# tan9zj/xnrs

Measured on AMD Instinct MI355X. Metric: impressions/sec (encode+score) on MIND-shaped batches, higher is better.
Workload: dtype f32; 1 GPU; NRMS full user+news encode + 5-candidate dot scoring (BASELINE configs[2]; token shape of config/mind_small_NRMS.yml); batch_impressions_per_gpu=512, history=50, candidates=5, d_backbone=768, n_heads=16, emb_dim=256, parallelism=impressions sharded by user over 1 GPU(s), no data-path collective

## Files before the change

### include/xnrs_hip.h

```cpp
#ifndef XNRS_HIP_H
#define XNRS_HIP_H

#include <stddef.h>
#include <stdint.h>

#ifdef __cplusplus
extern "C" {
#endif

#define XNRS_ABI_VERSION 6

#define XNRS_OK 0
#define XNRS_EINVAL (-1)
#define XNRS_EHEADS (-2)
#define XNRS_EWORKSPACE (-3)
#define XNRS_EUNSUPPORTED (-4)

#define XNRS_ACT_NONE 0
#define XNRS_ACT_RELU 1
#define XNRS_ACT_TANH 2

#define XNRS_POOL_ADDITIVE 0
#define XNRS_POOL_MEAN 1

typedef struct {
  const float *wq, *bq, *wk, *bk, *wv, *bv, *wo, *bo;
  int32_t n_heads;
  int32_t scaled;
  float dropout_p;
  uint64_t seed;
  const uint64_t *seed_dev;
} xnrs_mha_params;

typedef struct {
  const float *w1, *b1, *w2, *b2;
  int32_t hidden;
  const float *w1_folded, *b1_folded;
} xnrs_additive_params;

typedef struct {
  const float *w0, *b0, *w2, *b2;
  int32_t out_features;
  int32_t activation;
  const float *w0_folded, *b0_rowvec;
} xnrs_head_params;

int32_t xnrs_abi_version(void);
const char *xnrs_build_id(void);
const char *xnrs_error_string(int32_t code);

int32_t xnrs_linear_fwd(const float *x, const int32_t *gather_ids, int32_t gather_S, const float *w,
                        const float *bias, float *y, int64_t M, int32_t N, int32_t K, int32_t act,
                        void *stream);

size_t xnrs_mha_workspace_bytes(int64_t B, int32_t S, int32_t D);
int32_t xnrs_mha_fwd(const float *x, const float *m, const xnrs_mha_params *p, float *y, int64_t B,
                     int32_t S, int32_t D, void *ws, size_t ws_bytes, void *stream);

size_t xnrs_additive_workspace_bytes(int64_t B, int32_t N, int32_t D, int32_t A);
int32_t xnrs_additive_attention_fwd(const float *x, const float *m, const xnrs_additive_params *p,
                                    float *y, float *a_out, int64_t B, int32_t N, int32_t D, void *ws,
                                    size_t ws_bytes, void *stream);

int32_t xnrs_masked_mean_fwd(const float *x, const float *m, float *y, int64_t B, int32_t N, int32_t D,
                             void *stream);

int32_t xnrs_collapse_mask(const float *m, float *hm, int64_t n_rows, int32_t S, void *stream);

size_t xnrs_text_encoder_workspace_bytes(int64_t n_news, int32_t S, int32_t D, int32_t A, int32_t E,
                                         int32_t has_att, int32_t pool_kind, int32_t has_head,
                                         int64_t chunk);
int32_t xnrs_text_encoder_fwd(const float *x, const float *m, const int32_t *ids, int64_t n_news,
                              int32_t S, int32_t D, const xnrs_mha_params *att, int32_t pool_kind,
                              const xnrs_additive_params *pool, const xnrs_head_params *head, float *y,
                              float *hm, int64_t chunk, void *ws, size_t ws_bytes, void *stream);

size_t xnrs_fold_weights_workspace_bytes(int32_t D, int32_t A);
int32_t xnrs_fold_weights(const xnrs_mha_params *att, const xnrs_additive_params *pool, int32_t D, float *w1f, float *b1f,
                          void *ws, size_t ws_bytes, void *stream);

size_t xnrs_fold_head_weights_workspace_bytes(int32_t D, int32_t E);
int32_t xnrs_fold_head_weights(const xnrs_mha_params *att, const xnrs_head_params *head, int32_t D, float *w0f, float *b0v,
                               void *ws, size_t ws_bytes, void *stream);

size_t xnrs_text_encoder_unpadded_workspace_bytes(int64_t n_news, int64_t n_valid, int32_t S, int32_t D, int32_t A,
                                                  int32_t E, int32_t has_att, int32_t has_head);
int32_t xnrs_text_encoder_fwd_unpadded(const float *x, const int32_t *ids, int64_t n_news, int32_t S, int32_t D,
                                       const int32_t *rows, const int64_t *row_off, int64_t n_valid,
                                       const xnrs_mha_params *att, const xnrs_additive_params *pool,
                                       const xnrs_head_params *head, float *y, float *hm, void *ws, size_t ws_bytes,
                                       void *stream);

size_t xnrs_text_encoder_compact_workspace_bytes(int64_t n_news, int32_t S, int32_t D, int32_t A, int32_t E,
                                                 int32_t has_att, int32_t has_head, int64_t chunk);
int32_t xnrs_text_encoder_fwd_compact(const float *x, const float *m, const int32_t *ids, int64_t n_news, int32_t S,
                                      int32_t D, const xnrs_mha_params *att, const xnrs_additive_params *pool,
                                      const xnrs_head_params *head, float *y, float *hm, int64_t chunk, void *ws,
                                      size_t ws_bytes, void *stream);

size_t xnrs_user_encoder_workspace_bytes(int64_t B, int32_t H, int32_t E, int32_t A, int32_t has_att,
                                         int32_t pool_kind, int32_t has_head);
int32_t xnrs_user_encoder_fwd(const float *x, const float *m, int64_t B, int32_t H, int32_t E,
                              const xnrs_mha_params *att, int32_t pool_kind,
                              const xnrs_additive_params *pool, const xnrs_head_params *head, float *y,
                              float *a_out, void *ws, size_t ws_bytes, void *stream);

int32_t xnrs_dot_scoring_fwd(const float *u, const float *c, float *r, int64_t B, int32_t C, int32_t E,
                             int32_t normalize, void *stream);

#define XNRS_POOL_NONE (-1)
typedef struct {
  float *wq, *bq, *wk, *bk, *wv, *bv, *wo, *bo;
} xnrs_mha_grads;
typedef struct {
  float *w1, *b1, *w2, *b2;
} xnrs_additive_grads;
typedef struct {
  float *w0, *b0, *w2, *b2;
} xnrs_head_grads;

size_t xnrs_seq_encoder_saved_bytes(int64_t n_seq, int32_t L, int32_t D, int32_t A, int32_t E, int32_t n_heads,
                                    int32_t pool_kind, int32_t has_head);
int32_t xnrs_seq_encoder_fwd_train(const float *x, const float *m, const int32_t *ids, int64_t n_seq, int32_t L,
                                   int32_t D, const xnrs_mha_params *att, int32_t pool_kind,
                                   const xnrs_additive_params *pool, const xnrs_head_params *head, float *y,
                                   float *a_out, float *hm, void *saved, size_t saved_bytes, void *stream);
int32_t xnrs_seq_encoder_fwd_train_live(const float *x, const float *m, const int32_t *ids, int64_t n_seq, int32_t L,
                                        int32_t D, const xnrs_mha_params *att, int32_t pool_kind,
                                        const xnrs_additive_params *pool, const xnrs_head_params *head, float *y,
                                        float *a_out, float *hm, void *saved, size_t saved_bytes,
                                        const int32_t *live_rows, const int32_t *live_src_rows, int64_t n_live,
                                        void *stream);
size_t xnrs_seq_encoder_bwd_workspace_bytes(int64_t n_seq, int32_t L, int32_t D, int32_t A, int32_t E,
                                            int32_t n_heads, int32_t pool_kind, int32_t has_head);
int32_t xnrs_seq_encoder_bwd(const float *x, const float *m, const int32_t *ids, int64_t n_seq, int32_t L, int32_t D,
                             const xnrs_mha_params *att, int32_t pool_kind, const xnrs_additive_params *pool,
                             const xnrs_head_params *head, const void *saved, size_t saved_bytes, const float *dy,
                             float *dx, const xnrs_mha_grads *g_att, const xnrs_additive_grads *g_pool,
                             const xnrs_head_grads *g_head, void *ws, size_t ws_bytes, void *stream);
int32_t xnrs_seq_encoder_bwd_live(const float *x, const float *m, const int32_t *ids, int64_t n_seq, int32_t L, int32_t D,
                                  const xnrs_mha_params *att, int32_t pool_kind, const xnrs_additive_params *pool,
                                  const xnrs_head_params *head, const void *saved, size_t saved_bytes, const float *dy,
                                  float *dx, const xnrs_mha_grads *g_att, const xnrs_additive_grads *g_pool,
                                  const xnrs_head_grads *g_head, const int32_t *live_rows,
                                  const int32_t *live_src_rows, int64_t n_live, void *ws, size_t ws_bytes, void *stream);

typedef struct {
  const int32_t *live_rows, *live_src_rows;
  int64_t n_live;
  const int32_t *kv_rows, *kv_src_rows;
  int64_t n_kv;
  const float *qkv_shared;
  const int64_t *counts_dev;
  float *dqkv_image;
  int32_t dqkv_mode;
} xnrs_row_lists;
#define XNRS_DQKV_OWN 0
#define XNRS_DQKV_DEFER 1
#define XNRS_DQKV_MERGE 2

size_t xnrs_row_lists_workspace_bytes(int64_t n_seq);
int32_t xnrs_build_row_lists(const float *m, const int32_t *ids, int64_t n_seq, int32_t L, int32_t *live_rows,
                             int32_t *live_src_rows, int32_t *kv_rows, int32_t *kv_src_rows, int64_t *counts, void *ws,
                             size_t ws_bytes, void *stream);
size_t xnrs_seq_encoder_saved_qkv_offset(int64_t n_seq, int32_t L, int32_t D, int32_t A, int32_t E, int32_t n_heads,
                                         int32_t pool_kind, int32_t has_head);
int32_t xnrs_seq_encoder_fwd_train_rows(const float *x, const float *m, const int32_t *ids, int64_t n_seq, int32_t L,
                                        int32_t D, const xnrs_mha_params *att, int32_t pool_kind,
                                        const xnrs_additive_params *pool, const xnrs_head_params *head, float *y,
                                        float *a_out, float *hm, void *saved, size_t saved_bytes,
                                        const xnrs_row_lists *rows, void *stream);
int32_t xnrs_seq_encoder_bwd_rows(const float *x, const float *m, const int32_t *ids, int64_t n_seq, int32_t L, int32_t D,
                                  const xnrs_mha_params *att, int32_t pool_kind, const xnrs_additive_params *pool,
                                  const xnrs_head_params *head, const void *saved, size_t saved_bytes, const float *dy,
                                  float *dx, const xnrs_mha_grads *g_att, const xnrs_additive_grads *g_pool,
                                  const xnrs_head_grads *g_head, const xnrs_row_lists *rows, void *ws, size_t ws_bytes,
                                  void *stream);

size_t xnrs_linear_bwd_workspace_bytes(int64_t M, int32_t N, int32_t K);
int32_t xnrs_linear_bwd(const float *x, const int32_t *gather_ids, int32_t gather_S, const float *w, const float *dy,
                        float *dx, float *dw, float *db, int64_t M, int32_t N, int32_t K, void *ws, size_t ws_bytes,
                        void *stream);

size_t xnrs_embedding_linear_bwd_workspace_bytes(int64_t M, int32_t N, int32_t K);
int32_t xnrs_embedding_linear_bwd(const float *table, const int32_t *ids, const float *w, const float *dy, float *d_table,
                                  float *dw, float *db, int64_t M, int32_t N, int32_t K, int32_t n_rows, void *ws,
                                  size_t ws_bytes, void *stream);

int32_t xnrs_dot_scoring_bwd(const float *u, const float *c, const float *dr, float *du, float *dc, int64_t B,
                             int32_t C, int32_t E, void *stream);
int32_t xnrs_dot_scoring_norm_bwd(const float *u, const float *c, const float *dr, float *du, float *dc, int64_t B,
                                  int32_t C, int32_t E, void *stream);

int32_t xnrs_gather_rows(const float *table, const int32_t *ids, float *out, int64_t n, int64_t row_floats,
                         void *stream);

int32_t xnrs_dropout_rows(const float *x, const int32_t *ids, float *out, int64_t n, int64_t row_floats, float p,
                          uint64_t seed, const uint64_t *seed_dev, void *stream);

int32_t xnrs_assemble_train_batch(const int64_t *sess, int64_t B, const int64_t *hist_off, const int32_t *hist_val,
                                  const int64_t *pos_off, const int32_t *pos_val, const int64_t *neg_off,
                                  const int32_t *neg_val, int32_t l_hist, int32_t n_neg, int32_t pad_row, uint64_t seed,
                                  int32_t *hist_rows, int32_t *cand_rows, void *stream);
int32_t xnrs_assemble_eval_batch(const int64_t *sess, int64_t B, const int64_t *hist_off, const int32_t *hist_val,
                                 const int64_t *pos_off, const int32_t *pos_val, const int64_t *neg_off,
                                 const int32_t *neg_val, int32_t l_hist, int32_t pad_row, const int64_t *cand_off,
                                 int32_t *hist_rows, int32_t *cand_rows, int32_t *cand_sess, float *targets, void *stream);
int32_t xnrs_score_csr(const float *vecs, const int32_t *cand_rows, const int32_t *cand_sess, const float *u, float *r,
                       int64_t n_cand, int32_t E, int32_t relu, void *stream);
int32_t xnrs_rank_metrics(const float *scores, const float *targets, const int64_t *cand_off, float *out, int64_t B,
                          void *stream);

size_t xnrs_infonce_saved_bytes(int64_t B, int32_t E);
int32_t xnrs_infonce_fwd(const float *emb, const int64_t *labels, int64_t B, int32_t E, float temperature, float *loss,
                         void *saved, size_t saved_bytes, void *stream);
int32_t xnrs_infonce_bwd(const int64_t *labels, int64_t B, int32_t E, float temperature, const void *saved,
                         size_t saved_bytes, const float *gout, float *demb, void *stream);

#define XNRS_PROFILE_STAGES 10
int32_t xnrs_profile_enable(uint32_t stage_mask);
int32_t xnrs_profile_read(double *ms, int64_t *launches, double *flops);

int32_t xnrs_train_fold_enabled(void);

#define XNRS_STATUS_NONBINARY_MASK 1
#define XNRS_STATUS_ROW_RANGE 2
#define XNRS_STATUS_QUERY_RANGE 4
int32_t xnrs_set_status_word(int32_t *device_word);
const char *xnrs_status_string(int32_t word);

#define XNRS_GEMM_F32 0
#define XNRS_GEMM_BF16X3 1
#define XNRS_GEMM_BF16X2 2
int32_t xnrs_set_gemm_mode(int32_t mode);
int32_t xnrs_get_gemm_mode(void);

int32_t xnrs_reload_knobs(void);

size_t xnrs_bilinear_scoring_saved_bytes(int64_t B, int32_t E, int32_t normalize);
int32_t xnrs_bilinear_scoring_fwd(const float *u, const float *c, const float *w, const float *bias, float *s, int64_t B,
                                  int32_t N, int32_t E, int32_t normalize, void *saved, size_t saved_bytes, void *stream);
size_t xnrs_bilinear_scoring_bwd_workspace_bytes(int64_t B, int32_t E, int32_t normalize);
int32_t xnrs_bilinear_scoring_bwd(const float *u, const float *c, const float *w, const void *saved, size_t saved_bytes,
                                  const float *ds, float *du, float *dc, float *dw, float *dbias, int64_t B, int32_t N,
                                  int32_t E, int32_t normalize, void *ws, size_t ws_bytes, void *stream);
size_t xnrs_mlp_scoring_saved_bytes(int64_t B, int32_t N, int32_t H);
int32_t xnrs_mlp_scoring_fwd(const float *u, const float *c, const float *w1, const float *b1, const float *w2,
                             const float *b2, float *s, int64_t B, int32_t N, int32_t E, int32_t H, void *saved,
                             size_t saved_bytes, void *stream);
size_t xnrs_mlp_scoring_bwd_workspace_bytes(int64_t B, int32_t N, int32_t H);
int32_t xnrs_mlp_scoring_bwd(const float *u, const float *c, const float *w1, const float *w2, const void *saved,
                             size_t saved_bytes, const float *ds, float *du, float *dc, float *dw1, float *db1, float *dw2,
                             float *db2, int64_t B, int32_t N, int32_t E, int32_t H, void *ws, size_t ws_bytes,
                             void *stream);
int32_t xnrs_mlp_scoring_news_proj(const float *c, int64_t rows, int32_t E, const float *w1, int32_t H, float *p,
                                   void *stream);
size_t xnrs_score_csr_scorer_workspace_bytes(int64_t n_sess, int32_t width);
int32_t xnrs_score_csr_bilinear(const float *vecs, const int32_t *cand_rows, const int32_t *cand_sess, const float *u,
                                int64_t n_sess, const float *w, const float *bias, float *r, int64_t n_cand, int32_t E,
                                int32_t relu, void *ws, size_t ws_bytes, void *stream);
int32_t xnrs_score_csr_mlp(const float *P, const int32_t *cand_rows, const int32_t *cand_sess, const float *u,
                           int64_t n_sess, const float *w1, const float *b1, const float *w2, const float *b2, float *r,
                           int64_t n_cand, int32_t E, int32_t H, int32_t relu, void *ws, size_t ws_bytes, void *stream);
int32_t xnrs_l2_normalize_rows(const float *x, float *y, int64_t rows, int32_t E, void *stream);

typedef struct {
  const float *wx, *bx;
  const float *q;
  const int32_t *q_idx;
  int32_t hidden;
  int32_t q_ld;
  int32_t n_q;
} xnrs_personalized_params;

size_t xnrs_personalized_saved_bytes(int64_t n_seq, int32_t L, int32_t D, int32_t A, int32_t E, int32_t has_head);
int32_t xnrs_personalized_fwd(const float *x, const float *m, const int32_t *ids, int64_t n_seq, int32_t L, int32_t D,
                              const xnrs_personalized_params *p, const xnrs_head_params *head, float *y, float *a_out,
                              float *hm, void *ws, size_t ws_bytes, void *stream);
int32_t xnrs_personalized_fwd_train(const float *x, const float *m, const int32_t *ids, int64_t n_seq, int32_t L, int32_t D,
                                    const xnrs_personalized_params *p, const xnrs_head_params *head, float *y, float *a_out,
                                    float *hm, void *saved, size_t saved_bytes, void *stream);
size_t xnrs_personalized_bwd_workspace_bytes(int64_t n_seq, int32_t L, int32_t D, int32_t A, int32_t E, int32_t has_head);
int32_t xnrs_personalized_bwd(const float *x, const int32_t *ids, int64_t n_seq, int32_t L, int32_t D,
                              const xnrs_personalized_params *p, const xnrs_head_params *head, const void *saved,
                              size_t saved_bytes, const float *dy, float *dx, float *dwx, float *dbx, float *dq, int64_t n_q,
                              const xnrs_head_grads *g_head, void *ws, size_t ws_bytes, void *stream);

int32_t xnrs_embedding_grad_sparse(const float *d_rows, const int32_t *ids, int64_t M, int32_t K, float *d_table,
                                   int32_t n_rows, void *stream);
size_t xnrs_embedding_linear_bwd_sparse_workspace_bytes(int64_t M, int32_t N, int32_t K);
int32_t xnrs_embedding_linear_bwd_sparse(const float *table, const int32_t *ids, const float *w, const float *dy,
                                         float *d_table, float *dw, float *db, int64_t M, int32_t N, int32_t K, int32_t n_rows,
                                         void *ws, size_t ws_bytes, void *stream);

typedef struct {
  const float *w_ih, *w_hh, *b_ih, *b_hh;
  int32_t hidden;
} xnrs_gru_params;
typedef struct {
  float *w_ih, *w_hh, *b_ih, *b_hh;
} xnrs_gru_grads;
size_t xnrs_gru_workspace_bytes(int64_t B, int32_t T, int32_t E, int32_t Hd);
size_t xnrs_gru_saved_bytes(int64_t B, int32_t T, int32_t E, int32_t Hd);
int32_t xnrs_gru_fwd(const float *x, const float *m, int32_t ldm, const float *h0, const xnrs_gru_params *p, float *y,
                     int64_t B, int32_t T, int32_t E, void *ws, size_t ws_bytes, void *stream);
int32_t xnrs_gru_fwd_train(const float *x, const float *m, int32_t ldm, const float *h0, const xnrs_gru_params *p, float *y,
                           int64_t B, int32_t T, int32_t E, void *saved, size_t saved_bytes, void *stream);
size_t xnrs_gru_bwd_workspace_bytes(int64_t B, int32_t T, int32_t E, int32_t Hd);
int32_t xnrs_gru_bwd(const float *x, const xnrs_gru_params *p, const void *saved, size_t saved_bytes, const float *dy,
                     float *dx, float *dh0, const xnrs_gru_grads *g, int64_t B, int32_t T, int32_t E, void *ws,
                     size_t ws_bytes, void *stream);

size_t xnrs_attn_long_saved_bytes(int64_t L, int64_t Nb, int32_t E, int32_t n_heads);
size_t xnrs_attn_long_workspace_bytes(int64_t L, int64_t Nb, int32_t E, int32_t n_heads);
int32_t xnrs_attn_long_fwd(const float *qkv, int64_t seq_stride, int64_t batch_stride, float *o, int64_t o_seq_stride,
                           int64_t o_batch_stride, int64_t L, int64_t Nb, int32_t E, int32_t n_heads, void *stream);
int32_t xnrs_attn_long_fwd_train(const float *qkv, int64_t seq_stride, int64_t batch_stride, float *o, int64_t o_seq_stride,
                                 int64_t o_batch_stride, int64_t L, int64_t Nb, int32_t E, int32_t n_heads, void *saved,
                                 size_t saved_bytes, void *stream);
int32_t xnrs_attn_long_bwd(const float *qkv, int64_t seq_stride, int64_t batch_stride, const float *o, const float *d_o,
                           int64_t o_seq_stride, int64_t o_batch_stride, const void *saved, size_t saved_bytes, float *dqkv,
                           int64_t L, int64_t Nb, int32_t E, int32_t n_heads, void *ws, size_t ws_bytes, void *stream);

int32_t xnrs_caum_pair_fwd(const float *hp, const float *cp, int64_t ld_cp, float *h_cnn, float *z, int64_t B, int32_t C,
                           int32_t H, int32_t E, void *stream);
int32_t xnrs_caum_pair_bwd(const float *d_hcnn, const float *d_z, float *d_hp, float *d_cp, int64_t ld_dcp, int64_t B,
                           int32_t C, int32_t H, int32_t E, void *stream);

int32_t xnrs_caum_bias_tanh_fwd(const float *pre, const float *cb, int64_t ld_cb, float *t, int64_t P, int32_t H, int32_t E,
                                void *stream);
int32_t xnrs_caum_bias_tanh_bwd(const float *t, const float *dt, float *dpre, float *dcb, int64_t P, int32_t H, int32_t E,
                                void *stream);
int32_t xnrs_act_bwd(const float *y, const float *dy, float *dpre, int64_t n, int32_t act, void *stream);

int32_t xnrs_caum_pool_fwd(const float *t2, const float *w3, const float *b3, const float *h_all, float *u, float *a_out,
                           int64_t P, int32_t H, int32_t A, int32_t E, void *stream);
size_t xnrs_caum_pool_bwd_workspace_bytes(int64_t P, int32_t H, int32_t A);
int32_t xnrs_caum_pool_bwd(const float *t2, const float *w3, const float *h_all, const float *a, const float *du, float *d_t2,
                           float *d_w3, float *d_b3, float *d_hall, int64_t P, int32_t H, int32_t A, int32_t E, void *ws,
                           size_t ws_bytes, void *stream);

#ifdef __cplusplus
}
#endif
#endif
```

### xnrs_amd/csrc/api.hip

```cpp
#include <mutex>
#include <vector>

#include "host.h"

using namespace xnrs;

namespace xnrs {
uint32_t g_prof_mask = 0;
}
namespace {
std::vector<ProfRec> g_prof;
std::mutex g_prof_mu;
constexpr size_t PROF_MAX = 1 << 16;
}

bool xnrs::prof_begin(ProfRec* r, hipStream_t stream) {
  if (hipEventCreate(&r->beg) != hipSuccess || hipEventCreate(&r->end) != hipSuccess) return false;
  (void)hipEventRecord(r->beg, stream);
  return true;
}

void xnrs::prof_end(const ProfRec& r, hipStream_t stream) {
  (void)hipEventRecord(r.end, stream);
  std::lock_guard<std::mutex> lk(g_prof_mu);
  if (g_prof.size() < PROF_MAX) g_prof.push_back(r);
  else {
    (void)hipEventDestroy(r.beg);
    (void)hipEventDestroy(r.end);
  }
}

int64_t xnrs::prof_count(int stage, const int64_t* cnt, int which, int64_t host_value, hipStream_t stream) {
  if (!cnt || !prof_on(stage)) return host_value;
  int64_t v = host_value;
  if (hipStreamSynchronize(stream) != hipSuccess) return host_value;
  if (hipMemcpy(&v, cnt + which, sizeof(v), hipMemcpyDeviceToHost) != hipSuccess) return host_value;
  return v;
}

extern "C" {

int32_t xnrs_abi_version(void) { return XNRS_ABI_VERSION; }

#ifndef XNRS_BUILD_ID
#define XNRS_BUILD_ID "unknown"
#endif
const char* xnrs_build_id(void) { return XNRS_BUILD_ID; }

int32_t xnrs_set_status_word(int32_t* device_word) {
  set_status_word(device_word);
  return XNRS_OK;
}

const char* xnrs_status_string(int32_t word) {
  if (word == XNRS_STATUS_QUERY_RANGE)
    return "a query row index or user id outside its table (personalized attention: NaN outputs / clamped user ids)";
  if (word & XNRS_STATUS_QUERY_RANGE)
    return "several status bits: a query row index or user id out of range, and a bad mask value or table row id";
  switch (word & 3) {
    case 0: return "ok";
    case XNRS_STATUS_NONBINARY_MASK: return "a mask value other than 0 / 1 reached the device-compacted encoder (its outputs are NaN)";
    case XNRS_STATUS_ROW_RANGE: return "a news-table row id outside the table (clamped; the gathered rows are wrong)";
    default: return "a mask value other than 0 / 1 reached the device-compacted encoder AND a table row id was out of range";
  }
}

const char* xnrs_error_string(int32_t code) {
  switch (code) {
    case XNRS_OK: return "ok";
    case XNRS_EINVAL: return "invalid argument (shape or NULL pointer)";
    case XNRS_EHEADS: return "d_model is not divisible by n_heads";
    case XNRS_EWORKSPACE: return "workspace too small";
    case XNRS_EUNSUPPORTED:
      return "shape outside the supported range (attention S <= 128, pooling N <= 512, head width d_k <= 128, "
             "personalized attention L <= 4096, CAUM pooling H <= 8192)";
    default: return code > 0 ? hipGetErrorString((hipError_t)code) : "unknown error";
  }
}

int32_t xnrs_set_gemm_mode(int32_t mode) {
  const int prev = xnrs::gemm_mode();
  xnrs::set_gemm_mode(mode);
  return prev;
}

int32_t xnrs_get_gemm_mode(void) { return xnrs::gemm_mode(); }

int32_t xnrs_train_fold_enabled(void) { return fold_wanted(knobs().fold_train) ? 1 : 0; }

int32_t xnrs_reload_knobs(void) {
  xnrs::reload_knobs();
  return XNRS_OK;
}

int32_t xnrs_profile_enable(uint32_t stage_mask) {
  std::lock_guard<std::mutex> lk(g_prof_mu);
  for (auto& r : g_prof) {
    (void)hipEventDestroy(r.beg);
    (void)hipEventDestroy(r.end);
  }
  g_prof.clear();
  g_prof_mask = stage_mask;
  return XNRS_OK;
}

int32_t xnrs_profile_read(double* ms, int64_t* launches, double* flops) {
  if (!ms || !launches || !flops) return XNRS_EINVAL;
  for (int i = 0; i < XNRS_PROFILE_STAGES; ++i) {
    ms[i] = 0.0;
    launches[i] = 0;
    flops[i] = 0.0;
  }
  int32_t rc = XNRS_OK;
  std::lock_guard<std::mutex> lk(g_prof_mu);
  for (auto& r : g_prof) {
    float t = 0.f;
    hipError_t e = hipEventSynchronize(r.end);
    if (e == hipSuccess) e = hipEventElapsedTime(&t, r.beg, r.end);
    if (e != hipSuccess) rc = (int32_t)e;
    else {
      ms[r.stage] += t;
      launches[r.stage] += 1;
      flops[r.stage] += r.flops;
    }
    (void)hipEventDestroy(r.beg);
    (void)hipEventDestroy(r.end);
  }
  g_prof.clear();
  return rc;
}

}
```

### xnrs_amd/csrc/encoder_fwd.hip

```cpp
#include <vector>

#include "host.h"

using namespace xnrs;

namespace xnrs {

Plan make_plan(int64_t n_seq, int L, int D, int A, int E, bool att, bool additive, bool head, bool pooled, int64_t chunk,
               bool train, int n_heads) {
  Plan p{};
  if (train) chunk = n_seq > 0 ? n_seq : 1;
  if (chunk <= 0) chunk = 65536 / L;
  if (chunk > n_seq) chunk = n_seq;
  if (chunk < 1) chunk = 1;
  p.chunk = chunk;
  const size_t rows = (size_t)chunk * L;
  Carver c;
  p.off_qkv = c.take_if(att, rows * 3 * (size_t)D * F32);
  p.off_o = c.take_if(att, rows * (size_t)D * F32);
  p.off_y = c.take_if(att && pooled, rows * (size_t)D * F32);
  p.off_t = c.take_if(pooled && additive, rows * (size_t)A * F32);
  p.off_p = c.take_if(pooled && head, (size_t)n_seq * D * F32);
  p.off_h = c.take_if(pooled && head, (size_t)n_seq * E * F32);
  p.off_stats = c.take_if(train && att, (size_t)chunk * n_heads * L * 2 * F32);
  p.off_a = c.take_if(train && additive, rows * F32);
  size_t pl = 0;
  if (att) pl += 4 * align_up(split_planes_bytes(D, D));
  if (pooled && additive) pl += align_up(split_planes_bytes(A, D));
  p.off_planes = c.take(pl);
  NewsFusedPlan nf{};
  size_t nfb = 0;
  if (att && additive && !train) {
    if (n_heads <= 0) nfb = news_fused_img_bound_bytes(L, D, A);
    else if (news_fused_plan(L, D, n_heads, A, &nf)) nfb = nf.img_bytes;
  }
  p.off_nf = c.take_if(nfb != 0, nfb);
  p.off_nfo = c.take_if(nfb != 0, news_fused_scratch_bytes(L, D));
  const bool lt = att && pooled && !train;
  const size_t passes = (size_t)(((n_seq > 0 ? n_seq : 1) + chunk - 1) / chunk);
  p.off_lt_alive = c.take_if(lt, (size_t)(n_seq > 0 ? n_seq : 1));
  p.off_lt_n = c.take_if(lt, passes * sizeof(int64_t));
  p.off_lt_tiles = c.take_if(lt, passes * (size_t)live_tiles_cap(chunk, L, LIVE_TILE_BM) * sizeof(int32_t));
  const bool lr = lt && L <= 64;
  p.off_lr_loc = c.take_if(lr, passes * rows * sizeof(int32_t));
  p.off_lr_src = c.take_if(lr, passes * rows * sizeof(int32_t));
  p.off_lr_cnt = c.take_if(lr, passes * 3 * sizeof(int64_t));
  p.fold = carve_fold(c, att && additive, n_seq, D, A);
  p.total = c.total();
  return p;
}

bool device_counts_ok(const float* x, int D, int A, const xnrs_mha_params* att, const xnrs_additive_params* pool) {
  auto al16 = [](const void* p) { return p == nullptr || (reinterpret_cast<uintptr_t>(p) & 15) == 0; };
  if (!knobs().gemm_buf || gemm_mode() != 0 || D % 4 != 0 || D < 4 || (A > 0 && A % 4 != 0)) return false;
  if (!al16(x) || (pool && !al16(pool->w1))) return false;
  if (att && !(al16(att->wq) && al16(att->wk) && al16(att->wv) && al16(att->wo))) return false;
  return (int64_t)D * D * 4 <= (1ll << 30) && (int64_t)A * D * 4 <= (1ll << 30);
}

}

namespace {


hipError_t fold_product(const float* X, int M, const float* wo, int D, float* C, float* slabs, hipStream_t stream) {
  GemmArgs g = gemm_kmajor_b(X, D, wo, D, C, D, M, D, D);
  if (D >= 64 * FOLD_SPLITS) {
    g.slabs = slabs;
    g.nsplit = FOLD_SPLITS;
  }
  return launch_gemm_f32(g, stream);
}

const float* fold_out_projection(const xnrs_mha_params* att, const xnrs_additive_params* pool, int D, int A, float* wf,
                                 float* bf, float* slabs, hipStream_t stream, hipError_t* err) {
  *err = fold_product(pool->w1, A, att->wo, D, wf, slabs, stream);
  if (*err != hipSuccess || !att->bo) return pool->b1;
  *err = launch_fold_bias(pool->w1, att->bo, pool->b1, bf, A, D, stream);
  return bf;
}

struct Fc1 {
  const float* w;
  const float* b;
};
int32_t fc1_pair(bool fold, const xnrs_mha_params* att, const xnrs_additive_params* pool, int D, void* ws, const FoldRegions& fr,
                 hipStream_t stream, Fc1* fc1) {
  *fc1 = Fc1{pool ? pool->w1 : nullptr, pool ? pool->b1 : nullptr};
  if (!fold) return XNRS_OK;
  if (pool->w1_folded) {
    if (att->bo && !pool->b1_folded) return XNRS_EINVAL;
    *fc1 = Fc1{pool->w1_folded, att->bo ? pool->b1_folded : pool->b1};
    return XNRS_OK;
  }
  hipError_t fe = hipSuccess;
  fc1->w = at(ws, fr.fw);
  fc1->b = fold_out_projection(att, pool, D, pool->hidden, at(ws, fr.fw), at(ws, fr.fb), at(ws, fr.fsl), stream, &fe);
  return hip_rc(fe);
}

bool fc1_rowdot_ok(const float* x, bool att, const xnrs_additive_params* pool, int D) {
  auto al16 = [](const void* p) { return (reinterpret_cast<uintptr_t>(p) & 15) == 0; };
  return knobs().fc1_rowdot && knobs().gemm_buf && gemm_mode() == 0 && pool && pool->w2 && D % 4 == 0 && D >= 4 &&
         al16(pool->w1) && (att || al16(x)) && (int64_t)pool->hidden * D * 4 <= (1ll << 30);
}
inline int n_epart(int A) { return (A + 31) / 32; }

int32_t compact_attention_rc(const xnrs_mha_params* att, int S, int D) {
  if (att->n_heads <= 0 || D % att->n_heads != 0) return XNRS_EHEADS;
  if (S > 64 || D / att->n_heads > 64 || (D / att->n_heads) % 4 != 0 || D % 4 != 0) return XNRS_EUNSUPPORTED;
  return XNRS_OK;
}

GemmArgs qkv_projection(const float* x, RowIds rows, const xnrs_mha_params* att, int first, float* C, int64_t ldc, int64_t M,
                        int D, const unsigned short* const* planes = nullptr) {
  const float* W[3] = {att->wq, att->wk, att->wv};
  const float* b[3] = {att->bq, att->bk, att->bv};
  GemmArgs g = gemm_base(x, D, nullptr, D, C, ldc, M, D, D);
  g.gather_ids = rows.ids;
  g.gather_S = rows.S;
  for (int s = first; s < 3; ++s) {
    g.W[s - first] = W[s];
    g.bias[s - first] = b[s];
    g.Wp[s - first] = planes ? planes[s] : nullptr;
  }
  g.ldp = split_plane_ld(D);
  g.nseg = 3 - first;
  return g;
}

MhaCoreArgs mha_core_args(const float* k, int64_t ld, const xnrs_mha_params* att, float* out, int64_t n_seq, int S, int D) {
  MhaCoreArgs ma{};
  ma.k = k;
  ma.v = k + D;
  ma.ld = ld;
  ma.seq_stride = (int64_t)S * ld;
  ma.head_stride = D / att->n_heads;
  ma.out = out;
  ma.ldo = D;
  ma.n_seq = n_seq;
  ma.S = S;
  ma.n_heads = att->n_heads;
  ma.d_k = D / att->n_heads;
  ma.scaled = att->scaled;
  return ma;
}

GemmArgs fc1_product(const float* seq, RowIds rows, Fc1 fc1, float* t, int64_t M, int D, int A, bool rowdot,
                     const xnrs_additive_params* pool, const unsigned short* planes = nullptr) {
  GemmArgs g = gemm_linear(seq, rows, D, fc1.w, fc1.b, t, A, M, A, D, XNRS_ACT_TANH, planes);
  if (rowdot) {
    g.rowdot_w = pool->w2;
    g.rowdot_out = t;
    g.ldrd = n_epart(A);
  }
  return g;
}

AdditivePoolArgs additive_pool_args(const float* t, bool rowdot, const xnrs_additive_params* pool, const float* x, int64_t n_seq,
                                    int N, int D, int A) {
  AdditivePoolArgs pa{};
  pa.t = rowdot ? nullptr : t;
  pa.epart = rowdot ? t : nullptr;
  pa.n_epart = n_epart(A);
  pa.w2 = pool->w2;
  pa.b2 = pool->b2;
  pa.x = x;
  pa.ldx = D;
  pa.n_seq = n_seq;
  pa.N = N;
  pa.D = D;
  pa.A = A;
  return pa;
}

hipError_t pooled_out_projection(const float* po, const float* s, const xnrs_mha_params* att, float* dst, int64_t n, int D,
                                 const unsigned short* planes, hipStream_t stream) {
  GemmArgs g = gemm_linear(po, {}, D, att->wo, nullptr, dst, D, n, D, D, XNRS_ACT_NONE, planes);
  const bool in_epilogue = att->bo && gemm_mode() == 0;
  if (in_epilogue) {
    g.rowscale = s;
    g.rowscale_vec = att->bo;
  }
  hipError_t e = launch_gemm_f32(g, stream);
  if (e != hipSuccess || !att->bo || in_epilogue) return e;
  return launch_add_rowscaled_bias(dst, D, s, att->bo, n, D, stream);
}

int32_t pooled_tail(bool fold, const float* pob, const float* asum, const xnrs_mha_params* att, const xnrs_head_params* head,
                    float* pb, float* hb, float* y, int64_t n, int D, int E, const unsigned short* wo_planes, bool train,
                    hipStream_t stream) {
  const bool fold_head = fold && head && !train && head->w0_folded && gemm_mode() == 0 && (!att->bo || head->b0_rowvec);
  if (fold && !fold_head) {
    ProfScope ps(2, 2.0 * n * (double)D * D, stream);
    XNRS_TRY(pooled_out_projection(pob, asum, att, head ? pb : y, n, D, wo_planes, stream));
  }
  if (head) {
    ProfScope ps(5, 2.0 * n * ((double)D * E + (double)E * E), stream);
    GemmArgs g1 = gemm_linear(fold_head ? pob : pb, {}, D, fold_head ? head->w0_folded : head->w0, head->b0, hb, E, n, E, D,
                              head->activation);
    if (fold_head && att->bo) {
      g1.rowscale = asum;
      g1.rowscale_vec = head->b0_rowvec;
    }
    XNRS_TRY(launch_gemm_f32(g1, stream));
    XNRS_TRY(launch_gemm_f32(gemm_linear(hb, {}, E, head->w2, head->b2, y, E, n, E, E), stream));
  }
  return XNRS_OK;
}

}

int32_t xnrs::seq_encode(const SeqEncode& r, hipStream_t stream) {
  const float *x = r.x, *m = r.m;
  const int32_t* ids = r.ids;
  const int64_t n_seq = r.n_seq;
  const int L = r.L, D = r.D, pool_kind = r.pool_kind;
  const xnrs_mha_params* att = r.att;
  const xnrs_additive_params* pool = r.pool;
  const xnrs_head_params* head = r.head;
  const bool pooled = r.pooled, train = r.train;
  float *y = r.y, *a_out = r.a_out, *hm = r.hm;
  const xnrs_row_lists no_lists{};
  const xnrs_row_lists* rl = r.rl ? r.rl : &no_lists;
  const int32_t *live_rows = rl->live_rows, *live_src_rows = rl->live_src_rows, *kv_rows = rl->kv_rows,
                *kv_src_rows = rl->kv_src_rows;
  const float* qkv_shared = rl->qkv_shared;
  const int64_t* cnt = rl->counts_dev;
  const int64_t n_live = cnt ? n_seq * L : rl->n_live, n_kv = cnt ? n_seq * L : rl->n_kv;
  if (n_seq == 0) return XNRS_OK;
  if (n_seq < 0 || L <= 0 || D <= 0 || !x || !y) return XNRS_EINVAL;
  if (att) {
    if (att->n_heads <= 0 || !att->wq || !att->wk || !att->wv || !att->wo) return XNRS_EINVAL;
    if (D % att->n_heads != 0) return XNRS_EHEADS;
    if (L > 128) return XNRS_EUNSUPPORTED;
    if (train && D / att->n_heads > 128) return XNRS_EUNSUPPORTED;
  }
  const bool additive = pooled && pool_kind == XNRS_POOL_ADDITIVE;
  if (pooled) {
    if (pool_kind != XNRS_POOL_ADDITIVE && pool_kind != XNRS_POOL_MEAN) return XNRS_EINVAL;
    if (additive && (!pool || !pool->w1 || !pool->w2 || pool->hidden <= 0)) return XNRS_EINVAL;
    if (pool_kind == XNRS_POOL_MEAN && !m) return XNRS_EINVAL;
    if (L > 512) return XNRS_EUNSUPPORTED;
    if (head && (!head->w0 || !head->w2 || head->out_features <= 0 || head->activation < 0 || head->activation > 2))
      return XNRS_EINVAL;
  }
  if (ids && !m && pooled && pool_kind == XNRS_POOL_MEAN) return XNRS_EINVAL;
  const int A = additive ? pool->hidden : 0;
  const int E = (pooled && head) ? head->out_features : D;
  const Plan p = make_plan(n_seq, L, D, A, E, att != nullptr, additive, pooled && head, pooled, r.chunk, train,
                           att ? att->n_heads : 0);
  if (p.total > r.ws_bytes || (p.total > 0 && !r.ws)) return XNRS_EWORKSPACE;
  void* w = r.ws;
  float* stats = (train && att) ? at(w, p.off_stats) : nullptr;
  float* a_save = (train && additive) ? at(w, p.off_a) : nullptr;
  const bool qkv_given = train && att && qkv_shared;
  float* qkv = qkv_given ? const_cast<float*>(qkv_shared) : at(w, p.off_qkv);
  float *o = at(w, p.off_o), *yb = at(w, p.off_y), *t = at(w, p.off_t), *pb = at(w, p.off_p), *hb = at(w, p.off_h);

  const bool live = train && additive && m && live_rows && (cnt || (n_live >= 0 && n_live < n_seq * L)) &&
                    !(ids && !live_src_rows);
  if (cnt && live && !device_counts_ok(x, D, A, att, pool)) return XNRS_EUNSUPPORTED;
  const int32_t* lvx = live ? (ids ? live_src_rows : live_rows) : nullptr;
  const bool kvl = live && kv_rows && (cnt || (n_kv >= 0 && n_kv < n_seq * L)) && !(ids && !kv_src_rows);
  const int32_t* kvx = kvl ? (ids ? kv_src_rows : kv_rows) : nullptr;

  NewsFusedArgs f{};
  bool fused = att && additive && !train && !a_out && att->dropout_p == 0.f && gemm_mode() == 0 &&
               knobs().news_fused && news_fused_plan(L, D, att->n_heads, A, nullptr) &&
               (D / att->n_heads) * att->n_heads == D &&
               (knobs().news_fused == 2 || (L >= 26 && n_seq >= 192));
  if (fused) {
    f.x = x; f.ids = ids; f.mask = m;
    f.wq = att->wq; f.bq = att->bq; f.wk = att->wk; f.bk = att->bk; f.wv = att->wv; f.bv = att->bv;
    f.wo = att->wo; f.bo = att->bo;
    f.w1 = pool->w1; f.b1 = pool->b1; f.w2 = pool->w2; f.b2 = pool->b2;
    f.img = at(w, p.off_nf);
    f.p = head ? pb : y;
    f.ldp = D;
    f.hm = m ? hm : nullptr;
    f.n_seq = n_seq;
    f.S = L; f.D = D; f.n_heads = att->n_heads; f.d_k = D / att->n_heads; f.A = A; f.scaled = att->scaled;
    f.npw = knobs().news_fused_npw ? knobs().news_fused_npw : (n_seq < 512 ? 1 : 2);
    if (fold_wanted(knobs().fold_out)) {
      f.fold = 1;
      f.o_scratch = at(w, p.off_nfo);
      f.asum = at(w, p.fold.as);
      f.p = at(w, p.fold.po);
    }
    fused = p.off_nf != 0 && news_fused_ready(f);
  }
  const bool fold = att && additive && fold_wanted(train ? knobs().fold_train : knobs().fold_out);
  float *pob = at(w, p.fold.po), *asum = at(w, p.fold.as);
  const bool rowdot = additive && !train && !fused && fc1_rowdot_ok(x, att != nullptr, pool, D);
  Fc1 fc1{};
  XNRS_TRY_RC(fc1_pair(fold, att, additive ? pool : nullptr, D, w, p.fold, stream, &fc1));
  if (fold && fused) {
    f.w1 = fc1.w;
    f.b1 = fc1.b;
  }

  bool afused = !att && additive && !train && !a_out && gemm_mode() == 0 && knobs().additive_fused &&
                additive_fused_plan(L, D, A, nullptr, nullptr) && rowdot &&
                (knobs().additive_fused == 2 || additive_fused_tiles(n_seq, L) >= 512);
  if (afused) {
    AdditiveFusedArgs af{};
    af.x = x; af.ids = ids; af.mask = m;
    af.w1 = pool->w1; af.b1 = pool->b1; af.w2 = pool->w2; af.b2 = pool->b2;
    af.y = head ? pb : y;
    af.ldy = D;
    af.hm = m ? hm : nullptr;
    af.n_seq = n_seq;
    af.S = L; af.D = D; af.A = A;
    afused = additive_fused_ready(af);
    if (afused) {
      const double fl = (double)n_seq * (2.0 * L * D * A + 2.0 * L * (A + D));
      ProfScope ps(3, fl, stream);
      XNRS_TRY(launch_additive_fused(af, stream));
    }
  }

  const unsigned short* pqkv[3] = {nullptr, nullptr, nullptr};
  const unsigned short *po = nullptr, *p1 = nullptr;
  if (gemm_mode() != 0) {
    char* pw = at<char>(w, p.off_planes);
    auto prep = [&](const float* W, int N, int K) -> const unsigned short* {
      unsigned short* dst = reinterpret_cast<unsigned short*>(pw);
      pw += align_up(split_planes_bytes(N, K));
      return launch_split_weights(W, N, K, dst, stream) == hipSuccess ? dst : nullptr;
    };
    if (att) {
      pqkv[0] = prep(att->wq, D, D);
      pqkv[1] = prep(att->wk, D, D);
      pqkv[2] = prep(att->wv, D, D);
      po = prep(att->wo, D, D);
    }
    if (pooled && additive) p1 = prep(fc1.w, A, D);
  }

  if (fused) {
    const double fl = (double)n_seq * ((f.fold ? 6.0 : 8.0) * L * D * D + 4.0 * L * L * D + 2.0 * L * D * A + 2.0 * L * (A + D));
    ProfScope ps(6, fl, stream);
    XNRS_TRY(launch_news_fused(f, stream));
  }
  const bool lt = r.live_tiles && knobs().gemm_live_tiles && !train && pooled && m && att && !fused && !afused &&
                  n_seq * (int64_t)L >= knobs().gemm_live_tiles_min_rows &&
                  device_counts_ok(x, D, A, att, additive ? pool : nullptr);
  bool lt_qkv = false;
  if (lt && knobs().mha_skip_masked) {
    MhaCoreArgs probe = mha_core_args(qkv + D, 3 * (int64_t)D, att, o, p.chunk, L, D);
    probe.q = qkv;
    probe.mask = m;
    probe.skip_dead = 1;
    lt_qkv = mha_core_skips_dead(probe);
  }
  const bool lt_fc1 = lt && additive && rowdot;
  const int64_t lt_cap = live_tiles_cap(p.chunk, L, LIVE_TILE_BM);
  const int64_t* lt_n = at<int64_t>(w, p.off_lt_n);
  const int32_t* lt_tiles = at<int32_t>(w, p.off_lt_tiles);
  const bool lr = lt && knobs().gemm_live_rows && p.off_lr_cnt != 0 && L <= 64 && n_seq * (int64_t)L <= 0x7fffffffLL &&
                  n_seq * (int64_t)L >= knobs().gemm_live_rows_min_rows;
  const bool lr_qkv = lr && lt_qkv, lr_fc1 = lr && lt_fc1;
  const int32_t *lr_loc = at<int32_t>(w, p.off_lr_loc), *lr_src = at<int32_t>(w, p.off_lr_src);
  const int64_t* lr_cnt = at<int64_t>(w, p.off_lr_cnt);
  constexpr float LR_FILL = 0.3f;
  if (lr_qkv || lr_fc1)
    XNRS_TRY(launch_dense_row_lists(m, ids, n_seq, p.chunk, L, LIVE_TILE_BM, at<int32_t>(w, p.off_lr_loc), at<int32_t>(w, p.off_lr_src),
                                    at<int64_t>(w, p.off_lr_cnt), at<uint8_t>(w, p.off_lt_alive), at<int64_t>(w, p.off_lt_n),
                                    at<int32_t>(w, p.off_lt_tiles), stream));
  else if (lt_qkv || lt_fc1)
    XNRS_TRY(launch_live_tiles(m, ids, n_seq, p.chunk, L, LIVE_TILE_BM, at<uint8_t>(w, p.off_lt_alive), at<int64_t>(w, p.off_lt_n),
                               at<int32_t>(w, p.off_lt_tiles), stream));
  std::vector<int64_t> lt_host, lr_host;
  if ((lt_qkv && prof_on(0)) || (lt_fc1 && prof_on(3))) {
    lt_host.resize((size_t)((n_seq + p.chunk - 1) / p.chunk));
    if (hipStreamSynchronize(stream) != hipSuccess ||
        hipMemcpy(lt_host.data(), lt_n, lt_host.size() * sizeof(int64_t), hipMemcpyDeviceToHost) != hipSuccess)
      lt_host.clear();
    if (lr_qkv || lr_fc1) {
      lr_host.resize(3 * lt_host.size());
      if (lt_host.empty() || hipMemcpy(lr_host.data(), lr_cnt, lr_host.size() * sizeof(int64_t), hipMemcpyDeviceToHost) != hipSuccess)
        lr_host.clear();
    }
  }
  for (int64_t c0 = 0; !fused && !afused && c0 < n_seq; c0 += p.chunk) {
    const int64_t nc = (n_seq - c0 < p.chunk) ? (n_seq - c0) : p.chunk;
    const int64_t rows = nc * L;
    const int64_t* ltn = lt_n + c0 / p.chunk;
    const int32_t* ltl = lt_tiles + (c0 / p.chunk) * lt_cap;
    const double lt_rows = (double)LIVE_TILE_BM *
                           (double)(lt_host.empty() ? (rows + LIVE_TILE_BM - 1) / LIVE_TILE_BM : lt_host[(size_t)(c0 / p.chunk)]);
    const int32_t* lrl = lr_loc + (c0 / p.chunk) * p.chunk * L;
    const int32_t* lrs = lr_src + (c0 / p.chunk) * p.chunk * L;
    const int64_t* lrn = lr_cnt + 3 * (c0 / p.chunk);
    const double lr_rows = lr_host.empty() ? (double)rows : (double)lr_host[(size_t)(3 * (c0 / p.chunk))];
    const int32_t* cids = ids ? ids + c0 : nullptr;
    const float* cx = ids ? x : x + c0 * (int64_t)L * D;
    const float* cm = m ? (ids ? m : m + c0 * (int64_t)L) : nullptr;

    const float* seq = cx;
    const int32_t* seq_ids = cids;
    if (att) {
      const int64_t ld3 = 3 * (int64_t)D;
      if (qkv_given) {
      } else if (live) {
        const double nl = (double)prof_count(0, cnt, 0, n_live, stream), nkv = (double)prof_count(0, cnt, 1, n_kv, stream);
        ProfScope ps(0, 2.0 * (kvl ? nkv : rows) * 2.0 * D * D + 2.0 * nl * (double)D * D, stream);
        GemmArgs g = qkv_projection(cx, {cids, L}, att, 1, qkv + D, ld3, rows, D, pqkv);
        if (kvl) {
          XNRS_TRY(launch_zero_dead_qkv(qkv, cm, cids, nc, L, D, stream));
          g.gather_ids = kvx;
          g.gather_S = 1;
          g.c_scatter = 1;
          g.c_scatter_ids = kv_rows;
          g.M = n_kv;
          g.m_dev = cnt ? cnt + 1 : nullptr;
          g.m_fill_hint = 0.6f;
          if (n_kv > 0) XNRS_TRY(launch_gemm_f32(g, stream));
        } else {
          XNRS_TRY(launch_gemm_f32(g, stream));
          XNRS_TRY(launch_zero_cols(qkv, ld3, D, rows, stream));
        }
        if (n_live > 0) {
          GemmArgs q = gemm_linear(cx, {lvx, 1}, D, att->wq, att->bq, qkv, ld3, n_live, D, D, XNRS_ACT_NONE, pqkv[0]);
          q.c_scatter = 1;
          q.c_scatter_ids = live_rows;
          q.m_dev = cnt;
          q.m_fill_hint = 0.4f;
          XNRS_TRY(launch_gemm_f32(q, stream));
        }
      } else if (lr_qkv) {
        ProfScope ps(0, 2.0 * lt_rows * 2.0 * D * D + 2.0 * lr_rows * (double)D * D, stream);
        GemmArgs g = qkv_projection(cx, {cids, L}, att, 1, qkv + D, ld3, rows, D, pqkv);
        g.live_n = ltn;
        g.live_tiles = ltl;
        XNRS_TRY(launch_gemm_f32(g, stream));
        GemmArgs q = gemm_linear(cx, {ids ? lrs : lrl, 1}, D, att->wq, att->bq, qkv, ld3, rows, D, D);
        q.c_scatter = 1;
        q.c_scatter_ids = lrl;
        q.m_dev = lrn;
        q.m_fill_hint = LR_FILL;
        XNRS_TRY(launch_gemm_f32(q, stream));
      } else {
        GemmArgs g = qkv_projection(cx, {cids, L}, att, 0, qkv, ld3, rows, D, pqkv);
        if (lt_qkv) {
          g.live_n = ltn;
          g.live_tiles = ltl;
        }
        ProfScope ps(0, 2.0 * (lt_qkv ? lt_rows : (double)rows) * 3.0 * D * D, stream);
        XNRS_TRY(launch_gemm_f32(g, stream));
      }

      MhaCoreArgs ma = mha_core_args(qkv + D, ld3, att, o, nc, L, D);
      ma.q = qkv;
      ma.mask = cm;
      ma.mask_gather_ids = cids;
      ma.dropout_p = att->dropout_p;
      ma.seed = att->seed + (uint64_t)c0 * (uint64_t)att->n_heads * 0x9E3779B97F4A7C15ull;
      ma.seed_dev = att->seed_dev;
      ma.stats = stats;
      ma.skip_dead = (live || (pooled && cm && knobs().mha_skip_masked)) ? 1 : 0;
      if (lt_qkv && !mha_core_skips_dead(ma)) return XNRS_EUNSUPPORTED;
      {
        ProfScope ps(1, 4.0 * rows * (double)L * D, stream);
        XNRS_TRY(launch_mha_core(ma, stream));
      }

      float* dst = pooled ? yb : y + c0 * (int64_t)L * D;
      if (fold) {
        dst = o;
      } else if (live) {
        ProfScope ps(2, 2.0 * (double)prof_count(2, cnt, 0, n_live, stream) * (double)D * D, stream);
        XNRS_TRY(hipMemsetAsync(dst, 0, (size_t)rows * D * sizeof(float), stream));
        if (n_live > 0) {
          GemmArgs og = gemm_linear(o, {live_rows, 1}, D, att->wo, att->bo, dst, D, n_live, D, D, XNRS_ACT_NONE, po);
          og.c_scatter = 1;
          og.m_dev = cnt;
          og.m_fill_hint = 0.4f;
          XNRS_TRY(launch_gemm_f32(og, stream));
        }
      } else {
        ProfScope ps(2, 2.0 * rows * (double)D * D, stream);
        XNRS_TRY(launch_gemm_f32(gemm_linear(o, {}, D, att->wo, att->bo, dst, D, rows, D, D, XNRS_ACT_NONE, po), stream));
      }
      seq = dst;
      seq_ids = nullptr;
    }
    if (!pooled) continue;

    float* pooled_dst = (head ? pb : y) + c0 * (int64_t)D;
    float* hm_dst = hm ? hm + c0 : nullptr;
    if (additive) {
      if (live) {
        ProfScope ps(3, 2.0 * (double)prof_count(3, cnt, 0, n_live, stream) * (double)D * A, stream);
        XNRS_TRY(hipMemsetAsync(t, 0, (size_t)rows * A * sizeof(float), stream));
        if (n_live > 0) {
          GemmArgs fg = fc1_product(seq, {att ? live_rows : lvx, 1}, fc1, t, n_live, D, A, false, pool, p1);
          fg.c_scatter = 1;
          fg.c_scatter_ids = live_rows;
          fg.m_dev = cnt;
          fg.m_fill_hint = 0.4f;
          XNRS_TRY(launch_gemm_f32(fg, stream));
        }
      } else if (lr_fc1) {
        GemmArgs fg = fc1_product(seq, {seq_ids ? lrs : lrl, 1}, fc1, t, rows, D, A, true, pool, p1);
        fg.c_scatter = 1;
        fg.c_scatter_ids = lrl;
        fg.m_dev = lrn;
        fg.m_fill_hint = LR_FILL;
        ProfScope ps(3, 2.0 * lr_rows * (double)D * A, stream);
        XNRS_TRY(launch_gemm_f32(fg, stream));
      } else {
        GemmArgs fg = fc1_product(seq, {seq_ids, L}, fc1, t, rows, D, A, rowdot, pool, p1);
        if (lt_fc1) {
          fg.live_n = ltn;
          fg.live_tiles = ltl;
        }
        ProfScope ps(3, 2.0 * (lt_fc1 ? lt_rows : (double)rows) * (double)D * A, stream);
        XNRS_TRY(launch_gemm_f32(fg, stream));
      }
      AdditivePoolArgs pa = additive_pool_args(t, rowdot, pool, seq, nc, L, D, A);
      pa.skip_dead = lt_fc1 ? 1 : 0;
      pa.skip_masked = lr_fc1 ? 1 : 0;
      pa.mask = cm;
      pa.mask_gather_ids = cids;
      pa.x_gather_ids = seq_ids;
      pa.y = fold ? pob + c0 * (int64_t)D : pooled_dst;
      pa.asum_out = fold ? asum + c0 : nullptr;
      pa.a_out = a_save ? a_save : (a_out ? a_out + c0 * (int64_t)L : nullptr);
      pa.hm_out = cm ? hm_dst : nullptr;
      {
        ProfScope ps(4, 2.0 * rows * (double)(A + D), stream);
        XNRS_TRY(launch_additive_pool(pa, stream));
      }
      if (a_save && a_out)
        XNRS_TRY(hipMemcpyAsync(a_out, a_save, (size_t)rows * sizeof(float), hipMemcpyDeviceToDevice, stream));
    } else {
      MeanPoolArgs mp{};
      mp.x = seq;
      mp.ldx = D;
      mp.mask = cm;
      mp.mask_gather_ids = cids;
      mp.x_gather_ids = seq_ids;
      mp.y = pooled_dst;
      mp.hm_out = hm_dst;
      mp.n_seq = nc;
      mp.N = L;
      mp.D = D;
      {
        ProfScope ps(4, 2.0 * rows * (double)D, stream);
        XNRS_TRY(launch_mean_pool(mp, stream));
      }
    }
  }
  return pooled_tail(fold, pob, asum, att, pooled ? head : nullptr, pb, hb, y, n_seq, D, E, po, train, stream);
}

namespace {

struct UnpadPlan {
  size_t off_kv, off_q, off_o, off_y, off_t, off_p, off_h;
  FoldRegions fold;
  size_t total;
};
UnpadPlan make_unpad_plan(int64_t n_news, int64_t n_valid, int S, int D, int A, int E, bool att, bool head) {
  UnpadPlan p{};
  Carver c;
  const size_t nv = (size_t)(n_valid > 0 ? n_valid : 1);
  p.off_kv = c.take_if(att, (size_t)n_news * S * 2 * D * F32);
  p.off_q = c.take_if(att, nv * D * F32);
  p.off_o = c.take_if(att, nv * D * F32);
  p.off_y = c.take_if(att, nv * D * F32);
  p.off_t = c.take(nv * A * F32);
  p.off_p = c.take_if(head, (size_t)n_news * D * F32);
  p.off_h = c.take_if(head, (size_t)n_news * E * F32);
  p.fold = carve_fold(c, att, n_news, D, A);
  p.total = c.total();
  return p;
}

struct CompactPlan {
  int64_t chunk;
  size_t off_kv, off_q, off_o, off_t, off_roff, off_live, off_kvs, off_kvb, off_cnt, off_p, off_h;
  FoldRegions fold;
  size_t total;
};
CompactPlan make_compact_plan(int64_t n_news, int S, int D, int A, int E, bool att, bool head, int64_t chunk) {
  CompactPlan p{};
  if (chunk <= 0) chunk = 262144 / S;
  if (chunk > n_news) chunk = n_news;
  if (chunk < 1) chunk = 1;
  p.chunk = chunk;
  Carver c;
  const size_t rows = (size_t)chunk * S;
  p.off_kv = c.take_if(att, rows * 2 * D * F32);
  p.off_q = c.take_if(att, rows * D * F32);
  p.off_o = c.take_if(att, rows * D * F32);
  p.off_t = c.take(rows * (size_t)n_epart(A) * F32);
  const size_t passes = (size_t)((n_news + chunk - 1) / chunk);
  p.off_roff = c.take(passes * ((size_t)chunk + 1) * 8);
  p.off_live = c.take(passes * rows * 4);
  p.off_kvs = c.take(passes * rows * 4);
  p.off_kvb = c.take(passes * (size_t)chunk * 4);
  p.off_cnt = c.take(passes * 3 * 8);
  p.off_p = c.take_if(head, (size_t)n_news * D * F32);
  p.off_h = c.take_if(head, (size_t)n_news * E * F32);
  p.fold = carve_fold(c, att, n_news, D, A);
  p.total = c.total();
  return p;
}

SeqEncode padded_call(const float* x, const float* m, int64_t n_seq, int L, int D, float* y, void* ws, size_t ws_bytes) {
  SeqEncode r{};
  r.x = x; r.m = m; r.n_seq = n_seq; r.L = L; r.D = D; r.y = y; r.ws = ws; r.ws_bytes = ws_bytes;
  return r;
}

}

extern "C" {

int32_t xnrs_linear_fwd(const float* x, const int32_t* gather_ids, int32_t gather_S, const float* w, const float* bias,
                        float* y, int64_t M, int32_t N, int32_t K, int32_t act, void* stream) {
  if (!x || !w || !y || M < 0 || N <= 0 || K <= 0 || act < 0 || act > 2) return XNRS_EINVAL;
  if (gather_ids && gather_S <= 0) return XNRS_EINVAL;
  return hip_rc(launch_gemm_f32(gemm_linear(x, {gather_ids, gather_S}, K, w, bias, y, N, M, N, K, act), (hipStream_t)stream));
}

size_t xnrs_mha_workspace_bytes(int64_t B, int32_t S, int32_t D) {
  return make_plan(B, S, D, 0, D, true, false, false, false, 0).total;
}

int32_t xnrs_mha_fwd(const float* x, const float* m, const xnrs_mha_params* p, float* y, int64_t B, int32_t S, int32_t D,
                     void* ws, size_t ws_bytes, void* stream) {
  if (!p) return XNRS_EINVAL;
  SeqEncode r = padded_call(x, m, B, S, D, y, ws, ws_bytes);
  r.att = p;
  return seq_encode(r, (hipStream_t)stream);
}

size_t xnrs_additive_workspace_bytes(int64_t B, int32_t N, int32_t D, int32_t A) {
  return make_plan(B, N, D, A, D, false, true, false, true, 0).total;
}

int32_t xnrs_additive_attention_fwd(const float* x, const float* m, const xnrs_additive_params* p, float* y, float* a_out,
                                    int64_t B, int32_t N, int32_t D, void* ws, size_t ws_bytes, void* stream) {
  if (!p) return XNRS_EINVAL;
  SeqEncode r = padded_call(x, m, B, N, D, y, ws, ws_bytes);
  r.pooled = true; r.pool_kind = XNRS_POOL_ADDITIVE; r.pool = p; r.a_out = a_out;
  return seq_encode(r, (hipStream_t)stream);
}

int32_t xnrs_masked_mean_fwd(const float* x, const float* m, float* y, int64_t B, int32_t N, int32_t D, void* stream) {
  SeqEncode r = padded_call(x, m, B, N, D, y, nullptr, 0);
  r.pooled = true; r.pool_kind = XNRS_POOL_MEAN;
  return seq_encode(r, (hipStream_t)stream);
}

size_t xnrs_text_encoder_workspace_bytes(int64_t n_news, int32_t S, int32_t D, int32_t A, int32_t E, int32_t has_att,
                                         int32_t pool_kind, int32_t has_head, int64_t chunk) {
  return make_plan(n_news, S, D, A, E, has_att != 0, pool_kind == XNRS_POOL_ADDITIVE, has_head != 0, true, chunk).total;
}

int32_t xnrs_text_encoder_fwd(const float* x, const float* m, const int32_t* ids, int64_t n_news, int32_t S, int32_t D,
                              const xnrs_mha_params* att, int32_t pool_kind, const xnrs_additive_params* pool,
                              const xnrs_head_params* head, float* y, float* hm, int64_t chunk, void* ws, size_t ws_bytes,
                              void* stream) {
  if (n_news == 0) return XNRS_OK;
  if (!m) return XNRS_EINVAL;
  SeqEncode r = padded_call(x, m, n_news, S, D, y, ws, ws_bytes);
  r.ids = ids; r.att = att; r.pooled = true; r.pool_kind = pool_kind; r.pool = pool; r.head = head; r.hm = hm; r.chunk = chunk;
  r.live_tiles = true;
  return seq_encode(r, (hipStream_t)stream);
}

size_t xnrs_user_encoder_workspace_bytes(int64_t B, int32_t H, int32_t E, int32_t A, int32_t has_att, int32_t pool_kind,
                                         int32_t has_head) {
  return make_plan(B, H, E, A, E, has_att != 0, pool_kind == XNRS_POOL_ADDITIVE, has_head != 0, true, 0).total;
}

int32_t xnrs_user_encoder_fwd(const float* x, const float* m, int64_t B, int32_t H, int32_t E, const xnrs_mha_params* att,
                              int32_t pool_kind, const xnrs_additive_params* pool, const xnrs_head_params* head, float* y,
                              float* a_out, void* ws, size_t ws_bytes, void* stream) {
  SeqEncode r = padded_call(x, m, B, H, E, y, ws, ws_bytes);
  r.att = att; r.pooled = true; r.pool_kind = pool_kind; r.pool = pool; r.head = head; r.a_out = a_out;
  return seq_encode(r, (hipStream_t)stream);
}

size_t xnrs_text_encoder_unpadded_workspace_bytes(int64_t n_news, int64_t n_valid, int32_t S, int32_t D, int32_t A,
                                                  int32_t E, int32_t has_att, int32_t has_head) {
  return make_unpad_plan(n_news, n_valid, S, D, A, E, has_att != 0, has_head != 0).total;
}

int32_t xnrs_text_encoder_fwd_unpadded(const float* x, const int32_t* ids, int64_t n_news, int32_t S, int32_t D,
                                       const int32_t* rows, const int64_t* row_off, int64_t n_valid,
                                       const xnrs_mha_params* att, const xnrs_additive_params* pool,
                                       const xnrs_head_params* head, float* y, float* hm, void* ws, size_t ws_bytes,
                                       void* stream_) {
  hipStream_t stream = (hipStream_t)stream_;
  if (n_news == 0) return XNRS_OK;
  if (!x || !row_off || !pool || !y || n_news < 0 || n_valid < 0 || S <= 0 || D <= 0 || (n_valid > 0 && !rows))
    return XNRS_EINVAL;
  if (S > 512) return XNRS_EUNSUPPORTED;
  const int A = pool->hidden, E = head ? head->out_features : D;
  if (att) XNRS_TRY_RC(compact_attention_rc(att, S, D));
  const UnpadPlan p = make_unpad_plan(n_news, n_valid, S, D, A, E, att != nullptr, head != nullptr);
  if (p.total > 0 && (!ws || ws_bytes < p.total)) return XNRS_EWORKSPACE;
  float *kv = at(ws, p.off_kv), *qc = at(ws, p.off_q), *oc = at(ws, p.off_o), *yc = at(ws, p.off_y), *tc = at(ws, p.off_t);
  float *pb = at(ws, p.off_p), *hb = at(ws, p.off_h), *pob = at(ws, p.fold.po), *asum = at(ws, p.fold.as);
  const int64_t rows_all = n_news * (int64_t)S;

  const float* vals = x;
  const int32_t* val_ids = rows;
  const bool fold = att && fold_wanted(knobs().fold_out);
  Fc1 fc1{};
  XNRS_TRY_RC(fc1_pair(fold, att, pool, D, ws, p.fold, stream, &fc1));
  if (att) {
    {
      ProfScope ps(0, 2.0 * rows_all * 2.0 * D * D + 2.0 * n_valid * (double)D * D, stream);
      XNRS_TRY(launch_gemm_f32(qkv_projection(x, {ids, S}, att, 1, kv, 2 * (int64_t)D, rows_all, D), stream));
      if (n_valid > 0) XNRS_TRY(launch_gemm_f32(gemm_linear(x, {rows, 1}, D, att->wq, att->bq, qc, D, n_valid, D, D), stream));
    }
    if (n_valid > 0) {
      MhaCoreArgs ma = mha_core_args(kv, 2 * (int64_t)D, att, oc, n_news, S, D);
      ma.q = qc;
      ma.q_off = row_off;
      ma.ldq = D;
      {
        ProfScope ps(1, 4.0 * n_valid * (double)S * D, stream);
        XNRS_TRY(launch_mha_core(ma, stream));
      }
      if (!fold) {
        ProfScope ps(2, 2.0 * n_valid * (double)D * D, stream);
        XNRS_TRY(launch_gemm_f32(gemm_linear(oc, {}, D, att->wo, att->bo, yc, D, n_valid, D, D), stream));
      }
    }
    vals = fold ? oc : yc;
    val_ids = nullptr;
  }
  const bool rowdot = fc1_rowdot_ok(x, att != nullptr, pool, D);
  if (n_valid > 0) {
    ProfScope ps(3, 2.0 * n_valid * (double)D * A, stream);
    XNRS_TRY(launch_gemm_f32(fc1_product(vals, {val_ids, 1}, fc1, tc, n_valid, D, A, rowdot, pool), stream));
  }
  AdditivePoolArgs pa = additive_pool_args(tc, rowdot, pool, vals, n_news, S, D, A);
  pa.row_off = row_off;
  pa.row_ids = val_ids;
  pa.y = fold ? pob : (head ? pb : y);
  pa.asum_out = fold ? asum : nullptr;
  pa.hm_out = hm;
  {
    ProfScope ps(4, 2.0 * n_valid * (double)(A + D), stream);
    XNRS_TRY(launch_additive_pool(pa, stream));
  }
  return pooled_tail(fold, pob, asum, att, head, pb, hb, y, n_news, D, E, nullptr, false, stream);
}

size_t xnrs_text_encoder_compact_workspace_bytes(int64_t n_news, int32_t S, int32_t D, int32_t A, int32_t E, int32_t has_att,
                                                 int32_t has_head, int64_t chunk) {
  return make_compact_plan(n_news, S, D, A, E, has_att != 0, has_head != 0, chunk).total;
}

int32_t xnrs_text_encoder_fwd_compact(const float* x, const float* m, const int32_t* ids, int64_t n_news, int32_t S, int32_t D,
                                      const xnrs_mha_params* att, const xnrs_additive_params* pool, const xnrs_head_params* head,
                                      float* y, float* hm, int64_t chunk, void* ws, size_t ws_bytes, void* stream_) {
  hipStream_t stream = (hipStream_t)stream_;
  if (n_news == 0) return XNRS_OK;
  if (!x || !m || !pool || !pool->w1 || !pool->w2 || !y || n_news < 0 || S <= 0 || D <= 0 || pool->hidden <= 0) return XNRS_EINVAL;
  if (S > 512) return XNRS_EUNSUPPORTED;
  const int A = pool->hidden, E = head ? head->out_features : D;
  if (att) {
    XNRS_TRY_RC(compact_attention_rc(att, S, D));
    if (att->dropout_p != 0.f) return XNRS_EUNSUPPORTED;
  }
  if (gemm_mode() != 0 || !fc1_rowdot_ok(x, att != nullptr, pool, D)) return XNRS_EUNSUPPORTED;
  const CompactPlan p = make_compact_plan(n_news, S, D, A, E, att != nullptr, head != nullptr, chunk);
  if (!ws || ws_bytes < p.total) return XNRS_EWORKSPACE;
  float *kv = at(ws, p.off_kv), *qc = at(ws, p.off_q), *oc = at(ws, p.off_o), *tc = at(ws, p.off_t);
  int64_t *roff0 = at<int64_t>(ws, p.off_roff), *cnt0 = at<int64_t>(ws, p.off_cnt);
  int32_t *live0 = at<int32_t>(ws, p.off_live), *kvs0 = at<int32_t>(ws, p.off_kvs), *kvb0 = at<int32_t>(ws, p.off_kvb);
  float *pb = at(ws, p.off_p), *hb = at(ws, p.off_h), *pob = at(ws, p.fold.po), *asum = at(ws, p.fold.as);
  const bool fold = att && fold_wanted(knobs().fold_out);
  Fc1 fc1{};
  XNRS_TRY_RC(fc1_pair(fold, att, pool, D, ws, p.fold, stream, &fc1));
  if (att && !fold) return XNRS_EUNSUPPORTED;
  XNRS_TRY(launch_compact_rows(m, ids, n_news, p.chunk, S, roff0, live0, kvs0, kvb0, cnt0, stream));
  for (int64_t c0 = 0; c0 < n_news; c0 += p.chunk) {
    const int64_t nc = (n_news - c0 < p.chunk) ? (n_news - c0) : p.chunk;
    const int64_t rows = nc * S;
    const int64_t pass = c0 / p.chunk;
    const int64_t* cnt = cnt0 + 3 * pass;
    const int64_t* roff = roff0 + pass * (p.chunk + 1);
    const int32_t* live = live0 + pass * p.chunk * S;
    const int32_t* kvs = kvs0 + pass * p.chunk * S;
    const int32_t* kvb = kvb0 + pass * p.chunk;
    const float* vals = x;
    const int32_t* val_ids = live;
    if (att) {
      {
        GemmArgs g = qkv_projection(x, {kvs, 1}, att, 1, kv, 2 * (int64_t)D, rows, D);
        g.m_dev = cnt + 1;
        ProfScope ps(0, 2.0 * rows * 3.0 * D * D, stream);
        XNRS_TRY(launch_gemm_f32(g, stream));
        GemmArgs q = gemm_linear(x, {live, 1}, D, att->wq, att->bq, qc, D, rows, D, D);
        q.m_dev = cnt;
        XNRS_TRY(launch_gemm_f32(q, stream));
      }
      MhaCoreArgs ma = mha_core_args(kv, 2 * (int64_t)D, att, oc, nc, S, D);
      ma.q = qc;
      ma.q_off = roff;
      ma.ldq = D;
      ma.kv_block = kvb;
      {
        ProfScope ps(1, 4.0 * rows * (double)S * D, stream);
        XNRS_TRY(launch_mha_core(ma, stream));
      }
      vals = oc;
      val_ids = nullptr;
    }
    {
      ProfScope ps(3, 2.0 * rows * (double)D * A, stream);
      GemmArgs fg = fc1_product(vals, {val_ids, 1}, fc1, tc, rows, D, A, true, pool);
      fg.m_dev = cnt;
      XNRS_TRY(launch_gemm_f32(fg, stream));
    }
    AdditivePoolArgs pa = additive_pool_args(tc, true, pool, vals, nc, S, D, A);
    pa.row_off = roff;
    pa.row_ids = val_ids;
    pa.poison = cnt + 2;
    pa.y = (fold ? pob : (head ? pb : y)) + c0 * (int64_t)D;
    pa.asum_out = fold ? asum + c0 : nullptr;
    pa.hm_out = hm ? hm + c0 : nullptr;
    {
      ProfScope ps(4, 2.0 * rows * (double)(A + D), stream);
      XNRS_TRY(launch_additive_pool(pa, stream));
    }
  }
  XNRS_TRY_RC(pooled_tail(fold, pob, asum, att, head, pb, hb, y, n_news, D, E, nullptr, false, stream));
  const int n_pass = (int)((n_news + p.chunk - 1) / p.chunk);
  XNRS_TRY(launch_poison(y, n_news * (int64_t)E, cnt0 + 2, n_pass, 3, stream));
  if (hm) XNRS_TRY(launch_poison(hm, n_news, cnt0 + 2, n_pass, 3, stream));
  return XNRS_OK;
}

size_t xnrs_fold_weights_workspace_bytes(int32_t D, int32_t A) {
  return D > 0 && A > 0 ? align_up((size_t)FOLD_SPLITS * A * D * sizeof(float)) : 0;
}

int32_t xnrs_fold_weights(const xnrs_mha_params* att, const xnrs_additive_params* pool, int32_t D, float* w1f, float* b1f,
                          void* ws, size_t ws_bytes, void* stream) {
  if (!att || !pool || !att->wo || !pool->w1 || pool->hidden <= 0 || D <= 0 || !w1f || !b1f) return XNRS_EINVAL;
  if (ws_bytes < xnrs_fold_weights_workspace_bytes(D, pool->hidden) || !ws) return XNRS_EWORKSPACE;
  hipError_t fe = hipSuccess;
  const float* b = fold_out_projection(att, pool, D, pool->hidden, w1f, b1f, static_cast<float*>(ws), (hipStream_t)stream, &fe);
  XNRS_TRY(fe);
  if (b != b1f) {
    if (pool->b1) XNRS_TRY(hipMemcpyAsync(b1f, pool->b1, (size_t)pool->hidden * sizeof(float), hipMemcpyDeviceToDevice, (hipStream_t)stream));
    else XNRS_TRY(hipMemsetAsync(b1f, 0, (size_t)pool->hidden * sizeof(float), (hipStream_t)stream));
  }
  return XNRS_OK;
}

size_t xnrs_fold_head_weights_workspace_bytes(int32_t D, int32_t E) {
  return (D > 0 && E > 0) ? (size_t)FOLD_SPLITS * (size_t)E * (size_t)D * sizeof(float) : 0;
}

int32_t xnrs_fold_head_weights(const xnrs_mha_params* att, const xnrs_head_params* head, int32_t D, float* w0f, float* b0v,
                               void* ws, size_t ws_bytes, void* stream_) {
  hipStream_t stream = (hipStream_t)stream_;
  if (!att || !head || !att->wo || !head->w0 || !w0f || D <= 0 || head->out_features <= 0) return XNRS_EINVAL;
  if (att->bo && !b0v) return XNRS_EINVAL;
  const int E = head->out_features;
  if (ws_bytes < xnrs_fold_head_weights_workspace_bytes(D, E) || !ws) return XNRS_EWORKSPACE;
  XNRS_TRY(fold_product(head->w0, E, att->wo, D, w0f, static_cast<float*>(ws), stream));
  if (att->bo) XNRS_TRY(launch_fold_bias(head->w0, att->bo, nullptr, b0v, E, D, stream));
  return XNRS_OK;
}

}
```

### xnrs_amd/csrc/gemm_f32.hip

```cpp
#include <atomic>
#include <cstdlib>
#include <type_traits>

#include "kernels.h"

namespace xnrs {

constexpr int KALIGN = 32;

__device__ __attribute__((aligned(16))) float g_zero_line[4] = {0.f, 0.f, 0.f, 0.f};

typedef unsigned u32x4 __attribute__((ext_vector_type(4)));
constexpr unsigned BUF_OOB = 0x40000000u;

template <int TM, int TN, bool A_COL, bool B_KN, bool VEC, int PIPE, int BK, bool BUF = false, int MINW = 2, bool GATH = false,
          int KG = 2, bool RDOT = false, bool MDEV = false, bool LIVE = false>
__global__ __launch_bounds__(256, MINW) void gemm_f32_kernel(const GemmArgs a, int m_tiles, int n_tiles_seg, int gn) {
  static_assert(!MDEV || (!A_COL && !B_KN), "device row counts: forward layout only");
  static_assert(!LIVE || (BUF && !MDEV), "live row tiles: buffer-load forward kernels, host row count");
  static_assert(!BUF || (!A_COL && !B_KN && VEC), "buffer loads are implemented for the forward layout");
  static_assert(!RDOT || PIPE == 5, "the fused row dots ride on the interleaved pipeline (its MFMA call is the swapped one)");
  static_assert(!GATH || BUF, "the gathered-A variant keeps buffer loads for B");
  constexpr int BM = 64 * TM, BN = 64 * TN;
  constexpr bool SWZ = BK == 16;
  constexpr int LDK = SWZ ? BK : BK + 4;
  constexpr int CHK = BK / 4;
  constexpr int RPP = 256 / CHK;
  constexpr int AR = BM / RPP, BR = BN / RPP;
  constexpr int LDA = A_COL ? (BM + 4) : LDK;
  constexpr int LDB = B_KN ? (BN + 4) : LDK;
  constexpr int A_SZ = A_COL ? BK * LDA : BM * LDA;
  constexpr int B_SZ = B_KN ? BK * LDB : BN * LDB;
  constexpr int NBUF = 2;
  __shared__ __attribute__((aligned(16))) float As[NBUF][A_SZ];
  __shared__ __attribute__((aligned(16))) float Bs[NBUF][B_SZ];

  int64_t Mrun = a.M;
  int nwg = gridDim.x;
  if constexpr (MDEV) {
    const int64_t md = load_dev_scalar(a.m_dev);
    Mrun = ((int64_t)__builtin_amdgcn_readfirstlane((int)(md >> 32)) << 32) | (uint32_t)__builtin_amdgcn_readfirstlane((int)md);
    if (Mrun > a.M) Mrun = a.M;
    m_tiles = (int)((Mrun + BM - 1) / BM);
    nwg = m_tiles * n_tiles_seg * a.nseg;
    if ((int)blockIdx.x >= nwg) return;
  }
  if constexpr (LIVE) {
    const int nl = __builtin_amdgcn_readfirstlane((int)load_dev_scalar(a.live_n));
    m_tiles = nl < m_tiles ? (nl > 0 ? nl : 0) : m_tiles;
    nwg = m_tiles * n_tiles_seg * a.nseg;
    if ((int)blockIdx.x >= nwg) return;
  }
  const int bid = blockIdx.x;
  const int xcd = bid & 7;
  const int q = nwg >> 3, r = nwg & 7;
  const int wgid = (xcd < r ? xcd * (q + 1) : r * (q + 1) + (xcd - r) * q) + (bid >> 3);
  const int n_tiles = n_tiles_seg * a.nseg;
  const int grp = wgid / (gn * m_tiles);
  const int rem = wgid - grp * gn * m_tiles;
  const int gw = (n_tiles - grp * gn < gn) ? n_tiles - grp * gn : gn;
  const int mt = rem / gw;
  const int nt = grp * gn + (rem - mt * gw);
  const int seg = nt / n_tiles_seg;
  const int nts = nt - seg * n_tiles_seg;
  int64_t m0 = (int64_t)mt * BM;
  if constexpr (LIVE) m0 = (int64_t)__builtin_amdgcn_readfirstlane(a.live_tiles[mt]) * BM;
  const int n0 = nts * BN;

  int64_t kps = a.k_per_split;
  int Ktot = (int)a.K;
  if constexpr (A_COL && B_KN) {
    if (a.k_dev) {
      const int kd = __builtin_amdgcn_readfirstlane((int)load_dev_scalar(a.k_dev));
      Ktot = kd < Ktot ? (kd > 0 ? kd : 0) : Ktot;
      kps = (((int64_t)Ktot + gridDim.y - 1) / gridDim.y + KALIGN - 1) / KALIGN * KALIGN;
      if (kps < KALIGN) kps = KALIGN;
    }
  }
  const int kbeg = (int)((int64_t)blockIdx.y * kps);
  const int kend = (int)((kbeg + kps < Ktot) ? kbeg + kps : Ktot);

  const float* __restrict__ W = a.W[seg];
  const float* __restrict__ bias = a.bias[seg];

  const int tid = threadIdx.x;
  const int lane = tid & 63;
  const int wave = tid >> 6;
  const int wm = wave >> 1, wn = wave & 1;

  const int lc = tid % CHK, lr = tid / CHK;
  constexpr int CHA = BM / 4, KRA = 256 / CHA;
  constexpr int CHB = BN / 4, KRB = 256 / CHB;
  const int cA = tid % CHA, kA = tid / CHA;
  const int cB = tid % CHB, kB = tid / CHB;

  const float* pa[AR];
  const float* pb[BR];
  unsigned a_ok = 0, b_ok = 0;
  unsigned offA0 = 0, offB0 = 0;
  unsigned offBv[BR];
  int dA = 0, dB = 0;
  __amdgpu_buffer_rsrc_t rsA, rsB;
  if constexpr (BUF) {
    if constexpr (!GATH) rsA = __builtin_amdgcn_make_buffer_rsrc(const_cast<float*>(a.A), 0, (int)(Mrun * a.lda * 4), 0x00020000);
    rsB = __builtin_amdgcn_make_buffer_rsrc(const_cast<float*>(W), 0, (int)((int64_t)a.Nseg * a.ldw * 4), 0x00020000);
    if constexpr (GATH) {
#pragma unroll
      for (int i = 0; i < AR; ++i) {
        const int64_t gr = m0 + lr + RPP * i;
        int64_t src = gr < Mrun ? gr : Mrun - 1;
        if (a.gather_ids) {
          const int64_t n = src / a.gather_S;
          src = (int64_t)a.gather_ids[n] * a.gather_S + (src - n * a.gather_S);
        }
        pa[i] = a.A + src * a.lda + 4 * lc;
      }
    } else {
      const int64_t gr = m0 + lr;
      offA0 = gr < Mrun ? (unsigned)((gr * a.lda + 4 * lc) * 4) : BUF_OOB;
      dA = (int)(RPP * a.lda * 4);
    }
    const int col = n0 + lr;
    offB0 = col < a.Nseg ? (unsigned)(((int64_t)col * a.ldw + 4 * lc) * 4) : BUF_OOB;
    dB = (int)(RPP * a.ldw * 4);
    if constexpr (GATH) {
#pragma unroll
      for (int i = 0; i < BR; ++i) offBv[i] = offB0 + (unsigned)(i * dB);
    }
  } else if (!A_COL) {
#pragma unroll
    for (int i = 0; i < AR; ++i) {
      int64_t gr = m0 + lr + RPP * i;
      if (gr < Mrun) a_ok |= 1u << i;
      else gr = Mrun - 1;
      int64_t src = gr;
      if (a.gather_ids) {
        const int64_t n = gr / a.gather_S;
        src = (int64_t)a.gather_ids[n] * a.gather_S + (gr - n * a.gather_S);
      }
      pa[i] = a.A + src * a.lda;
    }
  } else {
    if (m0 + 4 * cA < Mrun) a_ok = 1;
  }
  if (!B_KN) {
#pragma unroll
    for (int i = 0; i < BR; ++i) {
      int col = n0 + lr + RPP * i;
      if (col < a.Nseg) b_ok |= 1u << i;
      else col = a.Nseg - 1;
      pb[i] = W + (int64_t)col * a.ldw;
    }
  } else {
    if (n0 + 4 * cB < a.Nseg) b_ok = 1;
  }

  f32x4 ra[1][AR], rb[1][BR];
  const f32x4 zero4 = {0.f, 0.f, 0.f, 0.f};
  auto gload = [&](auto P, int k0, int only = -1) {
    constexpr int p = decltype(P)::value;
    if constexpr (BUF) {
      const unsigned sel = (k0 + 4 * lc < kend) ? 0u : BUF_OOB;
      const int soff = (int)(k0 * 4);
      int ka = k0;
      if constexpr (GATH) {
        const int klim = kend - 4 - 4 * lc;
        ka = ka < klim ? ka : klim;
      }
#pragma unroll
      for (int i = 0; i < AR; ++i)
        if (only < 0 || only == i) {
          if constexpr (GATH) ra[p][i] = *reinterpret_cast<const f32x4*>(pa[i] + ka);
          else ra[p][i] = __builtin_bit_cast(f32x4, __builtin_amdgcn_raw_buffer_load_b128(rsA, (int)(offA0 | sel), soff + i * dA, 0));
        }
#pragma unroll
      for (int i = 0; i < BR; ++i)
        if (only < 0 || only == AR + i) {
          if constexpr (GATH) rb[p][i] = __builtin_bit_cast(f32x4, __builtin_amdgcn_raw_buffer_load_b128(rsB, (int)(offBv[i] | sel), soff, 0));
          else rb[p][i] = __builtin_bit_cast(f32x4, __builtin_amdgcn_raw_buffer_load_b128(rsB, (int)(offB0 | sel), soff + i * dB, 0));
        }
      return;
    }
    if (!A_COL) {
      const int64_t k = k0 + 4 * lc;
      const bool kok = k < kend;
#pragma unroll
      for (int i = 0; i < AR; ++i) {
        if (only >= 0 && only != i) continue;
        if (VEC) {
          ra[p][i] = *reinterpret_cast<const f32x4*>((kok && ((a_ok >> i) & 1u)) ? pa[i] + k : g_zero_line);
        } else {
          f32x4 v = zero4;
          if ((a_ok >> i) & 1u) {
#pragma unroll
            for (int e = 0; e < 4; ++e)
              if (k + e < kend) v[e] = pa[i][k + e];
          }
          ra[p][i] = v;
        }
      }
    } else {
      const int64_t mi = m0 + 4 * cA;
#pragma unroll
      for (int i = 0; i < AR; ++i) {
        if (only >= 0 && only != i) continue;
        const int k = k0 + kA + KRA * i;
        const bool kok = k < kend;
        int srck = kok ? k : kbeg;
        if constexpr (KG == 1) {
          srck = a.gather_ids[srck];
        } else if constexpr (KG == 2) {
          if (a.gather_ids) {
            if (a.gather_S == 1) srck = a.gather_ids[srck];
            else {
              const int n = srck / a.gather_S;
              srck = a.gather_ids[n] * a.gather_S + (srck - n * a.gather_S);
            }
          }
        }
        const float* ptr = a.A + (int64_t)srck * a.lda;
        if (VEC) {
          ra[p][i] = *reinterpret_cast<const f32x4*>((kok && a_ok) ? ptr + mi : g_zero_line);
        } else {
          f32x4 v = zero4;
          if (kok) {
#pragma unroll
            for (int e = 0; e < 4; ++e)
              if (mi + e < Mrun) v[e] = ptr[mi + e];
          }
          ra[p][i] = v;
        }
      }
    }
    if (!B_KN) {
      const int64_t k = k0 + 4 * lc;
      const bool kok = k < kend;
#pragma unroll
      for (int i = 0; i < BR; ++i) {
        if (only >= 0 && only != AR + i) continue;
        if (VEC) {
          rb[p][i] = *reinterpret_cast<const f32x4*>((kok && ((b_ok >> i) & 1u)) ? pb[i] + k : g_zero_line);
        } else {
          f32x4 v = zero4;
          if ((b_ok >> i) & 1u) {
#pragma unroll
            for (int e = 0; e < 4; ++e)
              if (k + e < kend) v[e] = pb[i][k + e];
          }
          rb[p][i] = v;
        }
      }
    } else {
      const int ni = n0 + 4 * cB;
#pragma unroll
      for (int i = 0; i < BR; ++i) {
        if (only >= 0 && only != AR + i) continue;
        const int k = k0 + kB + KRB * i;
        const bool kok = k < kend;
        int src = kok ? k : kbeg;
        if constexpr (KG == 1) {
          src = a.b_gather_ids[src];
        } else if constexpr (KG == 2) {
          if (a.b_gather_ids) {
            if (a.b_gather_S == 1) src = a.b_gather_ids[src];
            else {
              const int n = src / a.b_gather_S;
              src = a.b_gather_ids[n] * a.b_gather_S + (src - n * a.b_gather_S);
            }
          }
        }
        const float* ptr = W + (int64_t)src * a.ldw;
        if (VEC) {
          rb[p][i] = *reinterpret_cast<const f32x4*>((kok && b_ok) ? ptr + ni : g_zero_line);
        } else {
          f32x4 v = zero4;
          if (kok) {
#pragma unroll
            for (int e = 0; e < 4; ++e)
              if (ni + e < a.Nseg) v[e] = ptr[ni + e];
          }
          rb[p][i] = v;
        }
      }
    }
  };
  auto kswz = [](int row, int c) { return SWZ ? (c ^ ((row >> 2) & 3)) : c; };
  const bool do_cs = A_COL && a.colsum != nullptr && nt == 0;
  f32x4 cs = {0.f, 0.f, 0.f, 0.f};
  auto sstore = [&](auto P, int buf, int only = -1, bool fresh = true) {
    constexpr int p = decltype(P)::value;
#pragma unroll
    for (int i = 0; i < AR; ++i) {
      if (only >= 0 && only != i) continue;
      if (!A_COL) *reinterpret_cast<f32x4*>(&As[buf][(lr + RPP * i) * LDA + 4 * kswz(lr + RPP * i, lc)]) = ra[p][i];
      else {
        *reinterpret_cast<f32x4*>(&As[buf][(kA + KRA * i) * LDA + 4 * cA]) = ra[p][i];
        if (do_cs && fresh) cs += ra[p][i];
      }
    }
#pragma unroll
    for (int i = 0; i < BR; ++i) {
      if (only >= 0 && only != AR + i) continue;
      if (!B_KN) *reinterpret_cast<f32x4*>(&Bs[buf][(lr + RPP * i) * LDB + 4 * kswz(lr + RPP * i, lc)]) = rb[p][i];
      else *reinterpret_cast<f32x4*>(&Bs[buf][(kB + KRB * i) * LDB + 4 * cB]) = rb[p][i];
    }
  };

  f32x16 acc[TM][TN];
#pragma unroll
  for (int i = 0; i < TM; ++i)
#pragma unroll
    for (int j = 0; j < TN; ++j)
#pragma unroll
      for (int e = 0; e < 16; ++e) acc[i][j][e] = 0.f;

  const int frow = lane & 31;
  const int fk = (lane >> 5) * 4;
  const int a_row0 = wm * 32 * TM + frow;
  const int b_row0 = wn * 32 * TN + frow;

  auto compute = [&](int buf, auto KQ0, auto KQ1) {
#pragma unroll
    for (int kq = decltype(KQ0)::value; kq < decltype(KQ1)::value; ++kq) {
      f32x4 fa[TM], fb[TN];
#pragma unroll
      for (int i = 0; i < TM; ++i) {
        if (!A_COL) {
          fa[i] = *reinterpret_cast<const f32x4*>(&As[buf][(a_row0 + 32 * i) * LDA + 4 * kswz(a_row0 + 32 * i, kq * 2 + (fk >> 2))]);
        } else {
#pragma unroll
          for (int e = 0; e < 4; ++e) fa[i][e] = As[buf][(kq * 8 + fk + e) * LDA + a_row0 + 32 * i];
        }
      }
#pragma unroll
      for (int j = 0; j < TN; ++j) {
        if (!B_KN) {
          fb[j] = *reinterpret_cast<const f32x4*>(&Bs[buf][(b_row0 + 32 * j) * LDB + 4 * kswz(b_row0 + 32 * j, kq * 2 + (fk >> 2))]);
        } else {
#pragma unroll
          for (int e = 0; e < 4; ++e) fb[j][e] = Bs[buf][(kq * 8 + fk + e) * LDB + b_row0 + 32 * j];
        }
      }
#pragma unroll
      for (int e = 0; e < 4; ++e)
#pragma unroll
        for (int i = 0; i < TM; ++i)
#pragma unroll
          for (int j = 0; j < TN; ++j)
            acc[i][j] = __builtin_amdgcn_mfma_f32_32x32x2f32(fa[i][e], fb[j][e], acc[i][j], 0, 0, 0);
    }
  };
  using I0 = std::integral_constant<int, 0>;
  using I4 = std::integral_constant<int, BK / 8>;

  const int nk = (kend - kbeg + BK - 1) / BK;
  auto ktile = [&](int t) { return kbeg + t * BK; };
  if constexpr (PIPE == 1) {
    if (nk > 0) {
      gload(I0{}, ktile(0));
      sstore(I0{}, 0);
    }
    __syncthreads();
    for (int t = 0; t < nk; ++t) {
      const int buf = t & 1;
      if (t + 1 < nk) gload(I0{}, ktile(t + 1));
      compute(buf, I0{}, I4{});
      if (t + 1 < nk) sstore(I0{}, buf ^ 1);
      __syncthreads();
    }
  } else if constexpr (PIPE == 5) {
    constexpr int NKQ = BK / 8;
    constexpr int NSLOT = NKQ * 4;
    constexpr int NCH = AR + BR;
    static_assert(NCH + 2 <= NSLOT, "not enough slots for the tile stores/loads");
    f32x4 fa[2][TM], fb[2][TN];
    auto ldfrag = [&](int st, int buf, int kq) {
#pragma unroll
      for (int i = 0; i < TM; ++i) {
        if (!A_COL) {
          fa[st][i] = *reinterpret_cast<const f32x4*>(&As[buf][(a_row0 + 32 * i) * LDA + 4 * kswz(a_row0 + 32 * i, kq * 2 + (fk >> 2))]);
        } else {
#pragma unroll
          for (int e = 0; e < 4; ++e) fa[st][i][e] = As[buf][(kq * 8 + fk + e) * LDA + a_row0 + 32 * i];
        }
      }
#pragma unroll
      for (int j = 0; j < TN; ++j) {
        if (!B_KN) {
          fb[st][j] = *reinterpret_cast<const f32x4*>(&Bs[buf][(b_row0 + 32 * j) * LDB + 4 * kswz(b_row0 + 32 * j, kq * 2 + (fk >> 2))]);
        } else {
#pragma unroll
          for (int e = 0; e < 4; ++e) fb[st][j][e] = Bs[buf][(kq * 8 + fk + e) * LDB + b_row0 + 32 * j];
        }
      }
    };
    const int last = nk - 1;
    if (nk > 0) {
      gload(I0{}, ktile(0));
      sstore(I0{}, 0);
      gload(I0{}, ktile(1 < last ? 1 : last));
    }
    __syncthreads();
    for (int t = 0; t < nk; ++t) {
      const int buf = t & 1;
      const int kn = ktile(t + 2 < last ? t + 2 : last);
      ldfrag(0, buf, 0);
#pragma unroll
      for (int kq = 0; kq < NKQ; ++kq) {
#pragma unroll
        for (int e = 0; e < 4; ++e) {
          const int slot = kq * 4 + e;
#pragma unroll
          for (int i = 0; i < TM; ++i)
#pragma unroll
            for (int j = 0; j < TN; ++j)
              if constexpr (RDOT)
                acc[i][j] = __builtin_amdgcn_mfma_f32_32x32x2f32(fb[kq & 1][j][e], fa[kq & 1][i][e], acc[i][j], 0, 0, 0);
              else
                acc[i][j] = __builtin_amdgcn_mfma_f32_32x32x2f32(fa[kq & 1][i][e], fb[kq & 1][j][e], acc[i][j], 0, 0, 0);
          if (e == 1 && kq + 1 < NKQ) ldfrag((kq + 1) & 1, buf, kq + 1);
          if (slot >= 1 && slot < 1 + NCH) sstore(I0{}, buf ^ 1, slot - 1, t < last);
          if (slot >= 2 && slot < 2 + NCH) gload(I0{}, kn, slot - 2);
          __builtin_amdgcn_sched_barrier(0);
        }
      }
      __syncthreads();
    }
  }

  if constexpr (A_COL) {
    if (a.colsum != nullptr && nt == 0) {
      f32x4* red = reinterpret_cast<f32x4*>(&As[0][0]);
      red[kA * CHA + cA] = cs;
      __syncthreads();
      if (kA == 0) {
        f32x4 v = red[cA];
#pragma unroll
        for (int r = 1; r < KRA; ++r) v += red[r * CHA + cA];
        float* dst = a.colsum + (int64_t)blockIdx.y * Mrun + m0 + 4 * cA;
#pragma unroll
        for (int e = 0; e < 4; ++e)
          if (m0 + 4 * cA + e < Mrun) dst[e] = v[e];
      }
    }
  }

  const int ccol = lane & 31;
  const int crow = 4 * (lane >> 5);
  const bool split = gridDim.y > 1;
  float* Cout = split ? a.slabs + (int64_t)blockIdx.y * a.slab_stride : a.C;
  if constexpr (RDOT) {
    float2* s_bw = reinterpret_cast<float2*>(&As[0][0]);
    static_assert(sizeof(float2) * BN <= sizeof(float) * A_SZ * NBUF, "bias / weight staging fits the A tile buffers");
    for (int c = tid; c < BN; c += 256) {
      const int col = n0 + c;
      const bool cok = col < a.Nseg;
      s_bw[c] = make_float2((bias && cok) ? bias[col] : 0.f, cok ? a.rowdot_w[col] : 0.f);
    }
    __syncthreads();
    const int half = lane >> 5;
    auto dots = [&](auto FAST) {
#pragma unroll
      for (int j = 0; j < TN; ++j) {
        const int cb = wn * 32 * TN + 32 * j;
#pragma unroll
        for (int i = 0; i < TM; ++i) {
          const float sc = rowdot_block_t_lds<decltype(FAST)::value>(acc[i][j], s_bw + cb, half);
          int64_t row = m0 + wm * 32 * TM + 32 * i + (lane & 31);
          if (lane < 32 && row < Mrun && n0 + cb < a.Nseg) {
            if constexpr (GATH && MDEV) {
              if (a.c_scatter) row = (a.c_scatter_ids ? a.c_scatter_ids : a.gather_ids)[row];
            }
            a.rowdot_out[row * a.ldrd + ((n0 + cb) >> 5)] = sc;
          }
        }
      }
    };
    if (a.act == ACT_TANH_FAST) dots(std::true_type{});
    else dots(std::false_type{});
    return;
  }
  if constexpr (!A_COL) {
    if (a.c_scatter) {
      const int32_t* __restrict__ sids = a.c_scatter_ids ? a.c_scatter_ids : a.gather_ids;
      const bool one = a.gather_S == 1;
      float bvj[TN];
      int colj[TN];
#pragma unroll
      for (int j = 0; j < TN; ++j) {
        colj[j] = n0 + wn * 32 * TN + 32 * j + ccol;
        bvj[j] = (bias && !split && colj[j] < a.Nseg) ? bias[colj[j]] : 0.f;
      }
#pragma unroll
      for (int i = 0; i < TM; ++i) {
#pragma unroll
        for (int e = 0; e < 16; ++e) {
          int64_t row = m0 + wm * 32 * TM + 32 * i + (e & 3) + 8 * (e >> 2) + crow;
          if (row >= Mrun) continue;
          if (one) row = sids[row];
          else {
            const int64_t n = row / a.gather_S;
            row = (int64_t)sids[n] * a.gather_S + (row - n * a.gather_S);
          }
#pragma unroll
          for (int j = 0; j < TN; ++j) {
            if (colj[j] >= a.Nseg) continue;
            const int64_t coff = (int64_t)seg * a.Nseg + colj[j];
            float v = acc[i][j][e];
            if (!split) {
              if (a.rowscale) v = fmaf(a.rowscale[row], a.rowscale_vec[colj[j]], v);
              v = apply_act(v + bvj[j], a.act);
              if (a.aux_mode) {
                const float x = a.aux[row * a.ldaux + coff];
                v *= (a.aux_mode == 1) ? (1.f - x * x) : (x > 0.f ? 1.f : 0.f);
              }
              if (a.accumulate) v += Cout[row * a.ldc + coff];
            }
            Cout[row * a.ldc + coff] = v;
          }
        }
      }
      return;
    }
  }
#pragma unroll
  for (int j = 0; j < TN; ++j) {
    const int col = n0 + wn * 32 * TN + 32 * j + ccol;
    if (col >= a.Nseg) continue;
    const float bv = (bias && !split) ? bias[col] : 0.f;
    const int64_t coff = (int64_t)seg * a.Nseg + col;
#pragma unroll
    for (int i = 0; i < TM; ++i) {
#pragma unroll
      for (int e = 0; e < 16; ++e) {
        int64_t row = m0 + wm * 32 * TM + 32 * i + (e & 3) + 8 * (e >> 2) + crow;
        if (row < Mrun) {
          float v = acc[i][j][e];
          if (!split) {
            if (a.rowscale) v = fmaf(a.rowscale[row], a.rowscale_vec[col], v);
            v = apply_act(v + bv, a.act);
            if (a.aux_mode) {
              const float x = a.aux[row * a.ldaux + coff];
              v *= (a.aux_mode == 1) ? (1.f - x * x) : (x > 0.f ? 1.f : 0.f);
            }
            if (a.accumulate) v += Cout[row * a.ldc + coff];
          }
          if (BUF && a.nt_store) __builtin_nontemporal_store(v, &Cout[row * a.ldc + coff]);
          else Cout[row * a.ldc + coff] = v;
        }
      }
    }
  }
}

__global__ __launch_bounds__(256) void transpose_kernel(const float* W, float* Wt, int rows, int cols) {
  __shared__ float tile[32][33];
  const int tx = threadIdx.x & 31, ty = threadIdx.x >> 5;
  const int c0 = blockIdx.x * 32, r0 = blockIdx.y * 32;
#pragma unroll
  for (int i = 0; i < 4; ++i) {
    const int r = r0 + ty + 8 * i, c = c0 + tx;
    if (r < rows && c < cols) tile[ty + 8 * i][tx] = W[(int64_t)r * cols + c];
  }
  __syncthreads();
#pragma unroll
  for (int i = 0; i < 4; ++i) {
    const int c = c0 + ty + 8 * i, r = r0 + tx;
    if (r < rows && c < cols) Wt[(int64_t)c * rows + r] = tile[tx][ty + 8 * i];
  }
}

__global__ __launch_bounds__(256) void zero_cols_kernel(float* p, int64_t ld, int w4, int64_t n4) {
  const int64_t i = (int64_t)blockIdx.x * 256 + threadIdx.x;
  if (i >= n4) return;
  const int64_t r = i / w4;
  const int c = (int)(i - r * w4);
  __builtin_nontemporal_store(f32x4{0.f, 0.f, 0.f, 0.f}, reinterpret_cast<f32x4*>(p + r * ld) + c);
}

hipError_t launch_zero_cols(float* p, int64_t ld, int width, int64_t rows, hipStream_t stream) {
  if (rows <= 0 || width <= 0) return hipSuccess;
  if (width % 4 != 0 || ld % 4 != 0 || (reinterpret_cast<uintptr_t>(p) & 15) != 0)
    return hipMemset2DAsync(p, (size_t)ld * sizeof(float), 0, (size_t)width * sizeof(float), (size_t)rows, stream);
  const int64_t n4 = rows * (width / 4);
  hipLaunchKernelGGL(zero_cols_kernel, dim3((unsigned)((n4 + 255) / 256)), dim3(256), 0, stream, p, ld, width / 4, n4);
  return hipGetLastError();
}

__global__ __launch_bounds__(256) void zero_dead_qkv_kernel(float* qkv, const float* __restrict__ mask,
                                                            const int32_t* __restrict__ ids, int L, int D4) {
  const int64_t seq = blockIdx.x;
  const float* mp = mask + (ids ? (int64_t)ids[seq] : seq) * L;
  int any = 0;
  for (int s = threadIdx.x; s < L; s += 256) any |= mp[s] != 0.f ? 1 : 0;
  const bool empty = !__syncthreads_or(any);
  const int w4 = empty ? 3 * D4 : D4;
  f32x4* base = reinterpret_cast<f32x4*>(qkv) + seq * L * (int64_t)(3 * D4);
  for (int s = 0; s < L; ++s) {
    if (!empty && mp[s] != 0.f) continue;
    f32x4* row = base + (int64_t)s * (3 * D4);
    for (int c = threadIdx.x; c < w4; c += 256) __builtin_nontemporal_store(f32x4{0.f, 0.f, 0.f, 0.f}, row + c);
  }
}

hipError_t launch_zero_dead_qkv(float* qkv, const float* mask, const int32_t* ids, int64_t n_seq, int L, int D, hipStream_t stream) {
  if (n_seq <= 0) return hipSuccess;
  if (D % 4 != 0 || (reinterpret_cast<uintptr_t>(qkv) & 15) != 0 || n_seq > 0x7fffffffLL || !mask)
    return launch_zero_cols(qkv, 3 * (int64_t)D, 3 * D, n_seq * L, stream);
  hipLaunchKernelGGL(zero_dead_qkv_kernel, dim3((unsigned)n_seq), dim3(256), 0, stream, qkv, mask, ids, L, D / 4);
  return hipGetLastError();
}

hipError_t launch_transpose(const float* W, float* Wt, int rows, int cols, hipStream_t stream) {
  if (rows <= 0 || cols <= 0) return hipSuccess;
  hipLaunchKernelGGL(transpose_kernel, dim3((unsigned)((cols + 31) / 32), (unsigned)((rows + 31) / 32)), dim3(256), 0, stream, W,
                     Wt, rows, cols);
  return hipGetLastError();
}

__global__ __launch_bounds__(256) void splitk_reduce_kernel(const float* slabs, int64_t slab_stride, int nsplit, float* C,
                                                             int64_t n, int accumulate, const float* cs_partial, float* cs_out,
                                                             int cs_n, float* C2, int64_t n1, float* cs_out2, int cs_n1) {
  const int64_t i = (int64_t)blockIdx.x * 256 + threadIdx.x;
  if (i >= n) {
    const int64_t c = i - n;
    if (c < cs_n) {
      float v = 0.f;
      for (int s = 0; s < nsplit; ++s) v += cs_partial[(int64_t)s * cs_n + c];
      if (cs_out2 && c >= cs_n1) cs_out2[c - cs_n1] = v;
      else cs_out[c] = v;
    }
    return;
  }
  float* dst = (C2 && i >= n1) ? C2 + (i - n1) : C + i;
  float v = accumulate ? *dst : 0.f;
  for (int s = 0; s < nsplit; ++s) v += slabs[(int64_t)s * slab_stride + i];
  *dst = v;
}

int gemm_group_tiles(int n_tiles, int bn, int64_t K, bool plain) {
  int64_t gn = (int64_t)(2.5 * 1024 * 1024) / ((int64_t)bn * (K > 0 ? K : 1) * 4);
  if (knobs().gemm_group >= 0) gn = knobs().gemm_group;
  if (plain || gn <= 0 || gn >= n_tiles) return n_tiles;
  const int groups = (int)((n_tiles + gn - 1) / gn);
  return (n_tiles + groups - 1) / groups;
}

template <int TM, int TN, bool A_COL, bool B_KN>
static hipError_t launch_cfg(const GemmArgs& a, bool vec, int nsplit, hipStream_t stream) {
  constexpr int BM = 64 * TM, BN = 64 * TN;
  const int64_t m_tiles = (a.M + BM - 1) / BM;
  const int n_tiles_seg = (a.Nseg + BN - 1) / BN;
  const int64_t grid = m_tiles * n_tiles_seg * a.nseg;
  if (grid <= 0 || grid > 0x7fffffffLL) return hipErrorInvalidValue;
  const dim3 g((unsigned)grid, (unsigned)nsplit);
  const int gn = gemm_group_tiles(n_tiles_seg * a.nseg, BN, a.K, A_COL || B_KN);
  const int pipe = knobs().gemm_pipe;
  const int bk = knobs().gemm_bk;
  const bool bufB = knobs().gemm_buf && vec && (int64_t)a.Nseg * a.ldw * 4 <= (int64_t)BUF_OOB;
  const bool buf = bufB && !a.gather_ids && a.M * a.lda * 4 <= (int64_t)BUF_OOB;
  const bool gath = bufB && !buf && a.K >= 4;
#define XNRS_LAUNCH(VECV, PIPEV, BKV, BUFV, MINWV)                                                                  \
  hipLaunchKernelGGL((gemm_f32_kernel<TM, TN, A_COL, B_KN, VECV, PIPEV, BKV, BUFV, MINWV>), g, dim3(256), 0, stream, a, \
                     (int)m_tiles, n_tiles_seg, gn)
#define XNRS_LAUNCH_GATH(MINWV)                                                                                       \
  hipLaunchKernelGGL((gemm_f32_kernel<TM, TN, A_COL, B_KN, true, 5, 16, true, MINWV, true>), g, dim3(256), 0, stream, a, \
                     (int)m_tiles, n_tiles_seg, gn)
  if constexpr (TM == 2 && TN == 2 && !A_COL && !B_KN) {
    if (a.live_tiles) {
      if (!vec || !(buf || gath) || a.m_dev || !a.live_n || nsplit != 1 || a.c_scatter) return hipErrorInvalidValue;
#define XNRS_LAUNCH_LIVE(GATHV, RDOTV)                                                                                            \
  hipLaunchKernelGGL((gemm_f32_kernel<2, 2, false, false, true, 5, 16, true, 4, GATHV, 2, RDOTV, false, true>), g, dim3(256), 0, \
                     stream, a, (int)m_tiles, n_tiles_seg, gn)
      if (a.rowdot_out) {
        if (buf) XNRS_LAUNCH_LIVE(false, true);
        else XNRS_LAUNCH_LIVE(true, true);
      } else if (buf) XNRS_LAUNCH_LIVE(false, false);
      else XNRS_LAUNCH_LIVE(true, false);
#undef XNRS_LAUNCH_LIVE
      return hipGetLastError();
    }
  }
  if constexpr (!A_COL && !B_KN) {
    if (a.live_tiles && !(TM == 2 && TN == 2)) return hipErrorInvalidValue;
    if (a.m_dev) {
      if (!vec || !(buf || gath)) return hipErrorInvalidValue;
      if (a.rowdot_out) {
        if (buf)
          hipLaunchKernelGGL((gemm_f32_kernel<TM, TN, false, false, true, 5, 16, true, 4, false, 2, true, true>), g, dim3(256), 0,
                             stream, a, (int)m_tiles, n_tiles_seg, gn);
        else
          hipLaunchKernelGGL((gemm_f32_kernel<TM, TN, false, false, true, 5, 16, true, 4, true, 2, true, true>), g, dim3(256), 0,
                             stream, a, (int)m_tiles, n_tiles_seg, gn);
      } else if (buf) {
        hipLaunchKernelGGL((gemm_f32_kernel<TM, TN, false, false, true, 5, 16, true, 4, false, 2, false, true>), g, dim3(256), 0,
                           stream, a, (int)m_tiles, n_tiles_seg, gn);
      } else {
        hipLaunchKernelGGL((gemm_f32_kernel<TM, TN, false, false, true, 5, 16, true, 4, true, 2, false, true>), g, dim3(256), 0,
                           stream, a, (int)m_tiles, n_tiles_seg, gn);
      }
      return hipGetLastError();
    }
    if (a.rowdot_out) {
      if (!vec || !(buf || gath)) return hipErrorInvalidValue;
      if (buf)
        hipLaunchKernelGGL((gemm_f32_kernel<TM, TN, false, false, true, 5, 16, true, 4, false, 2, true>), g, dim3(256), 0, stream,
                           a, (int)m_tiles, n_tiles_seg, gn);
      else
        hipLaunchKernelGGL((gemm_f32_kernel<TM, TN, false, false, true, 5, 16, true, 4, true, 2, true>), g, dim3(256), 0, stream,
                           a, (int)m_tiles, n_tiles_seg, gn);
      return hipGetLastError();
    }
  }
  if (!vec) XNRS_LAUNCH(false, 1, 32, false, 2);
  else if constexpr (TM == 2 && TN == 2 && !A_COL && !B_KN) {
    if (pipe == 1 && buf) XNRS_LAUNCH(true, 1, 32, true, 2);
    else if (pipe == 1) XNRS_LAUNCH(true, 1, 32, false, 2);
    else if (pipe == 5 && bk == 16 && buf) XNRS_LAUNCH(true, 5, 16, true, 2);
    else if (pipe == 5 && buf) XNRS_LAUNCH(true, 5, 32, true, 2);
    else if (pipe == 5) XNRS_LAUNCH(true, 5, 32, false, 2);
    else if (buf) XNRS_LAUNCH(true, 5, 16, true, 4);
    else if (gath) XNRS_LAUNCH_GATH(4);
    else XNRS_LAUNCH(true, 5, 16, false, 3);
  } else if constexpr (!A_COL && !B_KN) {
    if (buf) XNRS_LAUNCH(true, 5, 16, true, 4);
    else if (gath) XNRS_LAUNCH_GATH(4);
    else XNRS_LAUNCH(true, 5, 16, false, 4);
  } else if constexpr (A_COL && B_KN) {
    const bool g_none = !a.gather_ids && !a.b_gather_ids;
    const bool g_live = a.gather_ids && a.b_gather_ids && a.gather_S == 1 && a.b_gather_S == 1;
#define XNRS_LAUNCH_KG(KGV)                                                                                              \
  hipLaunchKernelGGL((gemm_f32_kernel<TM, TN, A_COL, B_KN, true, 5, 32, false, 2, false, KGV>), g, dim3(256), 0, stream, a, \
                     (int)m_tiles, n_tiles_seg, gn)
    if (g_none) XNRS_LAUNCH_KG(0);
    else if (g_live) XNRS_LAUNCH_KG(1);
    else XNRS_LAUNCH_KG(2);
#undef XNRS_LAUNCH_KG
  } else {
    XNRS_LAUNCH(true, 5, 32, false, 2);
  }
#undef XNRS_LAUNCH
#undef XNRS_LAUNCH_GATH
  return hipGetLastError();
}

template <bool A_COL, bool B_KN>
static hipError_t launch_layout(const GemmArgs& a, bool vec, int nsplit, hipStream_t stream) {
  const int cand[4][2] = {{2, 2}, {2, 1}, {1, 2}, {1, 1}};
  const double eff[4] = {1.0, 0.94, 0.94, 0.86};
  int best = 0;
  double best_t = 1e300;
  for (int c = 0; c < 4; ++c) {
    const int64_t bm = 64 * cand[c][0], bn = 64 * cand[c][1];
    const int64_t m_exp = (a.m_dev && a.m_fill_hint > 0.f && a.m_fill_hint < 1.f) ? (int64_t)(a.M * (double)a.m_fill_hint) + 1 : a.M;
    const int64_t wgs = ((m_exp + bm - 1) / bm) * ((a.Nseg + bn - 1) / bn) * a.nseg * nsplit;
    const double slots = (A_COL || B_KN) ? 512.0 : 1024.0;
    const double rounds = (double)wgs / slots > 1.0 ? (double)wgs / slots : 1.0;
    const double t = rounds * (double)(bm * bn) / eff[c];
    if (t < best_t * 0.999) {
      best_t = t;
      best = c;
    }
  }
  if (knobs().gemm_tile >= 0 && knobs().gemm_tile <= 3) best = knobs().gemm_tile;
  if (a.live_tiles) best = 0;
  switch (best) {
    case 0: return launch_cfg<2, 2, A_COL, B_KN>(a, vec, nsplit, stream);
    case 1: return launch_cfg<2, 1, A_COL, B_KN>(a, vec, nsplit, stream);
    case 2: return launch_cfg<1, 2, A_COL, B_KN>(a, vec, nsplit, stream);
    default: return launch_cfg<1, 1, A_COL, B_KN>(a, vec, nsplit, stream);
  }
}

size_t gemm_splitk_workspace_bytes(int64_t M, int64_t N, int64_t K) {
  const int ns0 = gemm_pick_splits(M, N, K, false), ns1 = gemm_pick_splits(M, N, K, true);
  const int ns = ns0 > ns1 ? ns0 : ns1;
  return ns > 1 ? (size_t)ns * (size_t)M * (size_t)N * sizeof(float) : 0;
}

int gemm_pick_splits(int64_t M, int64_t N, int64_t K, bool dw_kernel) {
  int64_t tiles = ((M + 127) / 128) * ((N + 127) / 128);
  int64_t slots = dw_kernel ? 768 : 512;
  if (dw_kernel && knobs().gemm_dw_tile != 128 && M >= 384 && N >= 384) {
    tiles = ((M + 255) / 256) * ((N + 255) / 256);
    slots = 256;
  }
  int64_t ns = slots / tiles;
  const int64_t max_by_k = K / 256;
  if (ns > max_by_k) ns = max_by_k;
  if (ns > 64) ns = 64;
  if (ns < 1) ns = 1;
  return (int)ns;
}

static Knobs read_knobs() {
  Knobs k;
  auto num = [](const char* name, long long dflt) {
    const char* e = getenv(name);
    return (e && *e) ? atoll(e) : dflt;
  };
  k.gemm_pipe = (int)num("XNRS_GEMM_PIPE", 6);
  k.gemm_bk = num("XNRS_GEMM_BK", 32) == 16 ? 16 : 32;
  k.gemm_buf = num("XNRS_GEMM_BUF", 1) != 0;
  k.gemm_group = num("XNRS_GEMM_GROUP", -1);
  k.gemm_tile = (int)num("XNRS_GEMM_TILE", -1);
  k.split_min_tiles = num("XNRS_GEMM_SPLIT_MIN_TILES", 512);
  k.mha_lds = (int)num("XNRS_MHA_LDS", -1);
  k.mha_headwave = num("XNRS_MHA_HEADWAVE", 1) != 0;
  k.mha_pair = num("XNRS_MHA_PAIR", 1) != 0;
  k.mha_bwd_fused = num("XNRS_MHA_BWD_FUSED", 1) != 0;
  k.gemm_dw = (int)num("XNRS_GEMM_DW", 2);
  k.gemm_dw_tile = (int)num("XNRS_GEMM_DW_TILE", 256);
  k.fold_out = (int)num("XNRS_FOLD_OUT", 1);
  k.fc1_rowdot = num("XNRS_FC1_ROWDOT", 1) != 0;
  k.fold_train = (int)num("XNRS_FOLD_TRAIN", 1);
  k.news_fused = (int)num("XNRS_NEWS_FUSED", 1);
  k.news_fused_npw = (int)num("XNRS_NEWS_FUSED_NPW", 0);
  k.fast_tanh = num("XNRS_FAST_TANH", 1) != 0;
  k.additive_fused = (int)num("XNRS_ADDITIVE_FUSED", 1);
  k.af_fbuf = num("XNRS_AF_FBUF", 1) == 2 ? 2 : 1;
  k.mha_skip_masked = num("XNRS_MHA_SKIP_MASKED", 1) != 0;
  k.gemm_live_tiles = num("XNRS_GEMM_LIVE_TILES", 1) != 0;
  k.gemm_live_tiles_min_rows = num("XNRS_GEMM_LIVE_TILES_MIN_ROWS", 16384);
  k.gemm_live_rows = num("XNRS_GEMM_LIVE_ROWS", 1) != 0;
  k.gemm_live_rows_min_rows = num("XNRS_GEMM_LIVE_ROWS_MIN_ROWS", 16384);
  k.bwd_side_stream = num("XNRS_BWD_SIDE_STREAM", 1) != 0;
  k.bwd_side_min_rows = num("XNRS_BWD_SIDE_MIN_ROWS", 0);
  k.gru_layout = num("XNRS_GRU_LAYOUT", 0) == 1 ? 1 : 0;
  const long long m = num("XNRS_GEMM_MODE", 0);
  k.gemm_mode_init = (m >= 0 && m <= 2) ? (int)m : 0;
  return k;
}
static Knobs g_knobs = read_knobs();
static std::atomic<int> g_gemm_mode{g_knobs.gemm_mode_init};
const Knobs& knobs() { return g_knobs; }
void reload_knobs() { g_knobs = read_knobs(); }
int gemm_mode() { return g_gemm_mode.load(std::memory_order_relaxed); }
void set_gemm_mode(int mode) { g_gemm_mode.store((mode >= 0 && mode <= 2) ? mode : 0, std::memory_order_relaxed); }

hipError_t launch_gemm_f32(const GemmArgs& a_in, hipStream_t stream, int* nsplit_used) {
  GemmArgs a = a_in;
  if (a.M <= 0 || a.Nseg <= 0) return hipSuccess;
  if (a.act == 2 && knobs().fast_tanh) a.act = ACT_TANH_FAST;
  if (a.K >= (1ll << 31)) return hipErrorInvalidValue;
  auto al16 = [](const void* p) { return (reinterpret_cast<uintptr_t>(p) & 15) == 0; };
  bool vec = (a.lda % 4 == 0) && (a.ldw % 4 == 0) && al16(a.A);
  vec = vec && (a.a_col ? (a.M % 4 == 0) : (a.K % 4 == 0));
  vec = vec && (a.b_kn ? (a.Nseg % 4 == 0) : (a.K % 4 == 0));
  for (int s = 0; s < a.nseg; ++s) vec = vec && al16(a.W[s]);

  int nsplit = 1;
  if (a.slabs && a.nsplit > 1) {
    nsplit = a.nsplit;
    const int64_t per = ((a.K + nsplit - 1) / nsplit + KALIGN - 1) / KALIGN * KALIGN;
    a.k_per_split = per;
    nsplit = (int)((a.K + per - 1) / per);
    a.slab_stride = a.M * a.ldc;
    if (a.nseg != 1 || a.ldc != a.Nseg) return hipErrorInvalidValue;
  }
  if (nsplit <= 1) {
    nsplit = 1;
    a.k_per_split = a.K > 0 ? a.K : 1;
  }
  if (nsplit_used) *nsplit_used = nsplit;
  a.nt_store = (!a.accumulate && !a.c_scatter && a.M * a.ldc * 4 >= (64ll << 20)) ? 1 : 0;
  if (a.colsum && !(a.a_col && a.b_kn)) return hipErrorInvalidValue;
  if (a.k_dev && !(a.a_col && a.b_kn)) return hipErrorInvalidValue;
  if (a.colsum_out && !a.colsum) return hipErrorInvalidValue;
  if (a.C2 && (nsplit <= 1 || !(a.a_col && a.b_kn) || a.c2_row0 <= 0 || a.c2_row0 >= a.M)) return hipErrorInvalidValue;
  bool cs_copy = false;
  if (a.colsum && a.colsum_out && nsplit == 1) {
    if (al16(a.colsum_out)) a.colsum = a.colsum_out;
    else cs_copy = true;
  }
  if (a.rowdot_out && (a.a_col || a.b_kn || a.nseg != 1 || nsplit != 1 || !a.rowdot_w || a.accumulate || a.aux_mode ||
                       (a.act != 2 && a.act != ACT_TANH_FAST)))
    return hipErrorInvalidValue;
  if (a.rowdot_out && a.c_scatter && !(a.gather_ids && a.gather_S == 1 && a.m_dev)) return hipErrorInvalidValue;
  hipError_t e;
  const int mode = gemm_mode();
  const int64_t min_tiles = knobs().split_min_tiles;
  if (a.m_dev && (a.a_col || a.b_kn || nsplit != 1 || mode != 0)) return hipErrorInvalidValue;
  if (a.live_tiles && (a.a_col || a.b_kn || nsplit != 1 || mode != 0 || a.m_dev)) return hipErrorInvalidValue;
  if (a.rowscale && (a.a_col || a.b_kn || a.nseg != 1 || nsplit != 1 || !a.rowscale_vec || a.c_scatter || a.rowdot_out))
    return hipErrorInvalidValue;
  if (mode && !a.rowdot_out && !a.rowscale && !a.a_col && !a.b_kn && vec && nsplit == 1 &&
      ((a.M + 127) / 128) * ((a.Nseg + 127) / 128) * a.nseg >= min_tiles)
    return launch_gemm_split(a, mode == 1 ? 3 : 2, stream);
  if (!a.a_col && !a.b_kn) e = launch_layout<false, false>(a, vec, nsplit, stream);
  else if (!a.a_col && a.b_kn) e = launch_layout<false, true>(a, vec, nsplit, stream);
  else if (a.a_col && a.b_kn) {
    if (knobs().gemm_dw && gemm_dw_eligible(a)) e = launch_gemm_dw(a, nsplit, stream);
    else e = launch_layout<true, true>(a, vec, nsplit, stream);
  }
  else return hipErrorInvalidValue;
  if (e != hipSuccess) return e;
  if (nsplit > 1) {
    const int64_t n = a.M * a.ldc;
    const int cs_n = (a.colsum && a.colsum_out) ? (int)a.M : 0;
    hipLaunchKernelGGL(splitk_reduce_kernel, dim3((unsigned)((n + cs_n + 255) / 256)), dim3(256), 0, stream, a.slabs,
                       a.slab_stride, nsplit, a.C, n, a.accumulate, a.colsum, a.colsum_out, cs_n, a.C2, a.c2_row0 * a.ldc,
                       a.C2 ? a.colsum_out2 : nullptr, (int)a.c2_row0);
    e = hipGetLastError();
  } else if (cs_copy) {
    e = launch_colsum_final(a.colsum, 1, (int)a.M, a.colsum_out, stream);
  }
  return e;
}

}
```

### xnrs_amd/csrc/kernels.h

```cpp
#pragma once
#include <hip/hip_runtime.h>
#include <stdint.h>

namespace xnrs {

typedef float f32x4 __attribute__((ext_vector_type(4)));
typedef float f32x16 __attribute__((ext_vector_type(16)));

struct Knobs {
  int gemm_pipe = 6;
  int gemm_bk = 32;
  int gemm_buf = 1;
  long long gemm_group = -1;
  int gemm_tile = -1;
  long long split_min_tiles = 512;
  bool fc1_rowdot = true;
  int fold_train = 1;
  int fold_out = 1;
  int gemm_dw = 2;
  int gemm_dw_tile = 256;
  int mha_lds = -1;
  bool mha_pair = true;
  int mha_headwave = 1;
  int mha_bwd_fused = 1;
  int news_fused = 1;
  int news_fused_npw = 0;
  int gemm_mode_init = 0;
  bool fast_tanh = true;
  int additive_fused = 1;
  int af_fbuf = 1;
  bool bwd_side_stream = true;
  long long bwd_side_min_rows = 0;
  bool gemm_live_tiles = true;
  long long gemm_live_tiles_min_rows = 16384;
  bool gemm_live_rows = true;
  long long gemm_live_rows_min_rows = 16384;
  bool mha_skip_masked = true;
  int gru_layout = 0;
};
const Knobs& knobs();
void reload_knobs();

__device__ __forceinline__ int64_t load_dev_scalar(const int64_t* p) { return *p; }

struct GemmArgs {
  const float* A;
  int32_t a_col;
  const int32_t* gather_ids;
  int32_t gather_S;
  int32_t c_scatter;
  const int32_t* c_scatter_ids;
  int64_t lda;
  const float* W[3];
  const float* bias[3];
  int32_t b_kn;
  const int32_t* b_gather_ids;
  int32_t b_gather_S;
  int32_t nseg;
  int32_t Nseg;
  int64_t ldw;
  float* C;
  int64_t ldc;
  int64_t M;
  int64_t K;
  int32_t act;
  const float* aux;
  int64_t ldaux;
  int32_t aux_mode;
  int32_t accumulate;
  int32_t nt_store;
  const unsigned short* Wp[3];
  int64_t ldp;
  float* colsum;
  const float* rowdot_w;
  float* rowdot_out;
  int64_t ldrd;
  const float* rowscale;
  const float* rowscale_vec;
  const int64_t* m_dev;
  const int64_t* k_dev;
  float* colsum_out;
  float* C2;
  int64_t c2_row0;
  float* colsum_out2;
  float m_fill_hint;
  const int64_t* live_n;
  const int32_t* live_tiles;
  float* slabs;
  int32_t nsplit;
  int64_t k_per_split;
  int64_t slab_stride;
};
hipError_t launch_zero_cols(float* p, int64_t ld, int width, int64_t rows, hipStream_t stream);
hipError_t launch_zero_dead_qkv(float* qkv, const float* mask, const int32_t* ids, int64_t n_seq, int L, int D, hipStream_t stream);
hipError_t launch_transpose(const float* W, float* Wt, int rows, int cols, hipStream_t stream);
int gemm_pick_splits(int64_t M, int64_t N, int64_t K, bool dw_kernel = false);
int gemm_group_tiles(int n_tiles, int bn, int64_t K, bool plain);
size_t gemm_splitk_workspace_bytes(int64_t M, int64_t N, int64_t K);
hipError_t launch_gemm_f32(const GemmArgs& a, hipStream_t stream, int* nsplit_used = nullptr);
bool gemm_dw_eligible(const GemmArgs& a);
bool gemm_dw_big_tile(const GemmArgs& a);
hipError_t launch_gemm_dw(const GemmArgs& a, int nsplit, hipStream_t stream);
hipError_t launch_gemm_split(const GemmArgs& a, int npl, hipStream_t stream);
inline int64_t split_plane_ld(int64_t K) { return (K + 15) / 16 * 16; }
inline size_t split_planes_bytes(int64_t N, int64_t K) { return (size_t)3 * (size_t)N * (size_t)split_plane_ld(K) * 2; }
hipError_t launch_split_weights(const float* W, int64_t N, int64_t K, unsigned short* planes, hipStream_t stream);
int gemm_mode();
void set_gemm_mode(int mode);

struct MhaCoreArgs {
  const float* q;
  const float* k;
  const float* v;
  int64_t ld;
  int64_t seq_stride;
  int64_t head_stride;
  const float* mask;
  const int32_t* mask_gather_ids;
  float* out;
  int64_t ldo;
  int64_t n_seq;
  int32_t S, n_heads, d_k;
  int32_t scaled;
  float dropout_p;
  uint64_t seed;
  const uint64_t* seed_dev;
  float* stats;
  const int64_t* q_off;
  int64_t ldq;
  const int32_t* kv_block;
  int32_t skip_dead;
};
hipError_t launch_mha_core(const MhaCoreArgs& a, hipStream_t stream);
bool mha_core_skips_dead(const MhaCoreArgs& a);

struct MhaBwdArgs {
  const float* q;
  const float* k;
  const float* v;
  int64_t ld;
  const float* mask;
  const int32_t* mask_gather_ids;
  const float* o;
  int64_t ldo;
  const float* d_o;
  int64_t lddo;
  const float* stats;
  float* delta;
  float* dq;
  float* dk;
  float* dv;
  int64_t ldd;
  int64_t n_seq;
  int32_t S, n_heads, d_k;
  int32_t scaled;
  float dropout_p;
  uint64_t seed;
  const uint64_t* seed_dev;
  int32_t masked_do_is_zero;
  int32_t dead_seq_mode;
  int32_t accumulate;
};
hipError_t launch_mha_bwd(const MhaBwdArgs& a, hipStream_t stream);

__device__ __forceinline__ int64_t xcd_pair(int64_t L, int64_t W, int n_heads) {
  const int64_t n_seq = W / n_heads;
  const int64_t full = (n_seq >> 3) << 3;
  const int64_t per = (full >> 3) * n_heads;
  const int64_t x = L & 7, q = L >> 3;
  if (q < per) return ((q / n_heads) * 8 + x) * n_heads + (q % n_heads);
  return full * n_heads + (q - per) * 8 + x;
}

__device__ __forceinline__ float attn_exp(float x) { return __expf(x); }

__device__ __forceinline__ float fast_tanh(float x) {
  const float e = __builtin_amdgcn_exp2f(x * 2.8853900817779268f);
  return fmaf(-2.f, __builtin_amdgcn_rcpf(e + 1.f), 1.f);
}
template <bool FAST>
__device__ __forceinline__ float rowdot_block_t(const f32x16& acc, const float2 (&bw)[16]) {
  float s = 0.f;
#pragma unroll
  for (int e = 0; e < 16; ++e) {
    const float pre = acc[e] + bw[e].x;
    s = fmaf(FAST ? fast_tanh(pre) : tanhf(pre), bw[e].y, s);
  }
  return s + __shfl_xor(s, 32);
}
template <bool FAST>
__device__ __forceinline__ float rowdot_block_t_lds(const f32x16& acc, const float2* __restrict__ src, int half) {
  float s = 0.f;
#pragma unroll
  for (int g = 0; g < 4; ++g) {
    float2 c[4];
#pragma unroll
    for (int r = 0; r < 4; ++r) c[r] = src[8 * g + 4 * half + r];
#pragma unroll
    for (int r = 0; r < 4; ++r) {
      const float pre = acc[4 * g + r] + c[r].x;
      s = fmaf(FAST ? fast_tanh(pre) : tanhf(pre), c[r].y, s);
    }
  }
  return s + __shfl_xor(s, 32);
}
__device__ __forceinline__ void rowdot_load_bw(float2 (&bw)[16], const float2* __restrict__ src, int half) {
#pragma unroll
  for (int g = 0; g < 4; ++g)
#pragma unroll
    for (int r = 0; r < 4; ++r) bw[4 * g + r] = src[8 * g + 4 * half + r];
}

constexpr int ACT_TANH_FAST = 3;
__device__ __forceinline__ float apply_act(float v, int act) {
  if (act == 1) return fmaxf(v, 0.f);
  if (act == 3) return fast_tanh(v);
  if (act == 2) return tanhf(v);
  return v;
}

template <class Args>
__device__ __forceinline__ uint64_t drop_seed(const Args& a) {
  return a.seed + (a.seed_dev ? *a.seed_dev : 0ull);
}
template <class Args>
__device__ __forceinline__ float drop_uniform(const Args& a, int64_t seq, int hd, int S, int query, int key) {
  uint64_t z = drop_seed(a) + 0x9E3779B97F4A7C15ull * ((uint64_t)(seq * a.n_heads + hd) + 1);
  z = (z ^ (z >> 30)) * 0xBF58476D1CE4E5B9ull;
  z = (z ^ (z >> 27)) * 0x94D049BB133111EBull;
  z = z ^ (z >> 31);
  uint32_t x = (uint32_t)z ^ ((uint32_t)(query * S + key) * 0x9E3779B9u);
  x ^= x >> 16;
  x *= 0x85EBCA6Bu;
  x ^= x >> 13;
  x *= 0xC2B2AE35u;
  x ^= x >> 16;
  x ^= (uint32_t)(z >> 32);
  return (float)(x >> 8) * (1.0f / 16777216.0f);
}
struct DropRowsArgs {
  uint64_t seed;
  const uint64_t* seed_dev;
  int n_heads;
};
__device__ __forceinline__ float drop_uniform(const DropRowsArgs& a, int64_t row, uint32_t j) {
  return drop_uniform(a, row, 0, 0, 0, (int)j);
}

struct NewsFusedArgs {
  const float* x;
  const int32_t* ids;
  const float* mask;
  const float *wq, *bq, *wk, *bk, *wv, *bv, *wo, *bo;
  const float *w1, *b1, *w2, *b2;
  float* img;
  float* p;
  int64_t ldp;
  float* hm;
  int64_t n_seq;
  int32_t S, D, n_heads, d_k, A, scaled;
  int32_t npw;
  int32_t tanh_act;
  int32_t fold;
  float* o_scratch;
  float* asum;
};
struct NewsFusedPlan {
  int npw, hg, lq, ly;
  int n_groups, nk, nkc;
  size_t lds_bytes;
  size_t img_bytes;
};
bool news_fused_plan(int S, int D, int n_heads, int A, NewsFusedPlan* plan, int npw = 2);
size_t news_fused_img_bound_bytes(int S, int D, int A);
size_t news_fused_scratch_bytes(int S, int D);
bool news_fused_ready(const NewsFusedArgs& a);
hipError_t launch_news_fused(const NewsFusedArgs& a, hipStream_t stream);

struct AdditiveFusedArgs {
  const float* x;
  const int32_t* ids;
  const float* mask;
  const float *w1, *b1, *w2, *b2;
  float* y;
  int64_t ldy;
  float* hm;
  int64_t n_seq;
  int32_t S, D, A;
  int32_t tanh_act;
};
bool additive_fused_plan(int S, int D, int A, int* nn_out, int* pp_out);
bool additive_fused_ready(const AdditiveFusedArgs& a);
int64_t additive_fused_tiles(int64_t n_seq, int S);
hipError_t launch_additive_fused(const AdditiveFusedArgs& a, hipStream_t stream);

struct AdditivePoolArgs {
  const float* t;
  const float* epart;
  int32_t n_epart;
  const float* w2;
  const float* b2;
  const float* mask;
  const int32_t* mask_gather_ids;
  const int32_t* x_gather_ids;
  const float* x;
  int64_t ldx;
  float* y;
  float* a_out;
  float* hm_out;
  float* asum_out;
  int64_t n_seq;
  int32_t N, D, A;
  const int64_t* row_off;
  const int32_t* row_ids;
  int32_t skip_dead;
  int32_t skip_masked;
  const int64_t* poison;
};
hipError_t launch_additive_pool(const AdditivePoolArgs& a, hipStream_t stream);
hipError_t launch_fold_bias(const float* w1, const float* bo, const float* b1, float* bf, int A, int D, hipStream_t stream);
hipError_t launch_add_rowscaled_bias(float* p, int64_t ld, const float* s, const float* b, int64_t n, int D, hipStream_t stream);

struct MeanPoolArgs {
  const float* x;
  int64_t ldx;
  const float* mask;
  const int32_t* mask_gather_ids;
  const int32_t* x_gather_ids;
  float* y;
  float* hm_out;
  int64_t n_seq;
  int32_t N, D;
};
hipError_t launch_mean_pool(const MeanPoolArgs& a, hipStream_t stream);

struct AdditivePoolBwdArgs {
  const float* dp;
  const float* x;
  int64_t ldx;
  const int32_t* x_gather_ids;
  const float* a;
  const float* t;
  const float* w2;
  float* dx;
  int64_t lddx;
  float* dpre;
  float* de;
  const float* da_shift;
  const float* shift_u;
  const float* shift_v;
  int64_t n_seq;
  int32_t N, D, A;
};
hipError_t launch_additive_pool_bwd(const AdditivePoolBwdArgs& a, hipStream_t stream);
hipError_t launch_mean_pool_bwd(const float* dy, const float* mask, const int32_t* mask_ids, float* dx, int64_t lddx,
                                int64_t n_seq, int32_t N, int32_t D, hipStream_t stream);
size_t colsum_workspace_bytes(int N);
hipError_t launch_colsum(const float* X, int64_t ldx, const float* w, int64_t M, int N, float* out, float* partial,
                         hipStream_t stream);
hipError_t launch_colsum2(const float* X, int64_t ldx, const float* w, int64_t M, const float* X2, int64_t ldx2, const float* w2,
                          int64_t M2, int N, float* out, float* partial, hipStream_t stream);
hipError_t launch_colsum_wsum(const float* X, int64_t ldx, const float* w, int64_t M, int N, float* out, float* wsum_out,
                              float* partial, hipStream_t stream);
hipError_t launch_colsum_final(const float* partial, int nsplit, int N, float* out, hipStream_t stream);
hipError_t launch_dot_scoring_bwd(const float* u, const float* c, const float* dr, float* du, float* dc, int64_t B, int32_t C,
                                  int32_t E, hipStream_t stream);
hipError_t launch_dot_scoring_norm_bwd(const float* u, const float* c, const float* dr, float* du, float* dc, int64_t B,
                                       int32_t C, int32_t E, hipStream_t stream);

hipError_t launch_embedding_grad(const float* d_rows, const int32_t* ids, int64_t M, int K, float* d_table, int n_rows,
                                 hipStream_t stream);

hipError_t launch_collapse_mask(const float* m, const int32_t* gather_ids, float* hm, int64_t n_rows, int32_t S,
                                hipStream_t stream);
hipError_t launch_dot_scoring(const float* u, const float* c, float* r, int64_t B, int32_t C, int32_t E,
                              int32_t normalize, hipStream_t stream);

struct BatchArgs {
  const int64_t* sess;
  const int64_t* hist_off;
  const int32_t* hist_val;
  const int64_t* pos_off;
  const int32_t* pos_val;
  const int64_t* neg_off;
  const int32_t* neg_val;
  int64_t B;
  int32_t l_hist, n_neg;
  int32_t pad_row;
  uint64_t seed;
  int32_t* hist_out;
  int32_t* cand_out;
  const int64_t* cand_off_out;
  int32_t* cand_sess_out;
  float* targets_out;
};
hipError_t launch_gather_rows(const float* table, const int32_t* ids, float* out, int64_t n, int64_t row_floats,
                              hipStream_t stream);
hipError_t launch_poison(float* y, int64_t n, const int64_t* flags, int n_flags, int flag_stride, hipStream_t stream);
int32_t* status_word();
void set_status_word(int32_t* w);
hipError_t launch_compact_rows(const float* mask, const int32_t* ids, int64_t n_news, int64_t chunk, int S, int64_t* row_off,
                               int32_t* live_src, int32_t* kv_src, int32_t* kv_block, int64_t* counts, hipStream_t stream);
hipError_t launch_build_row_lists(const float* mask, const int32_t* ids, int64_t n_seq, int L, int32_t* live, int32_t* live_src,
                                  int32_t* kv, int32_t* kv_src, int64_t* counts, int32_t* cnt_scratch, hipStream_t stream);
constexpr int LIVE_TILE_BM = 128;
inline int64_t live_tiles_cap(int64_t chunk, int L, int BM) { return (chunk * L + BM - 1) / BM; }
hipError_t launch_live_tiles(const float* mask, const int32_t* ids, int64_t n_seq, int64_t chunk, int L, int BM, uint8_t* alive,
                             int64_t* n_tiles, int32_t* tiles, hipStream_t stream);
hipError_t launch_dense_row_lists(const float* mask, const int32_t* ids, int64_t n_seq, int64_t chunk, int L, int BM,
                                  int32_t* live_loc, int32_t* live_src, int64_t* counts, uint8_t* alive, int64_t* n_tiles,
                                  int32_t* tiles, hipStream_t stream);
hipError_t launch_assemble_train(const BatchArgs& a, hipStream_t stream);
hipError_t launch_assemble_eval(const BatchArgs& a, hipStream_t stream);
hipError_t launch_score_csr(const float* vecs, const int32_t* rows, const int32_t* sess, const float* u, float* r, int64_t n,
                            int E, int relu, hipStream_t stream);
hipError_t launch_rank_metrics(const float* score, const float* target, const int64_t* off, float* out, int64_t B,
                               hipStream_t stream);

struct ColSumSeg {
  const float* X;
  int64_t ld;
  int64_t rows;
  int ncol;
  float* out;
};
hipError_t launch_colsum_segments(const ColSumSeg* segs, int n_segs, hipStream_t stream);
hipError_t launch_l2_normalize_rows(const float* x, float* y, int64_t rows, int E, hipStream_t stream);
hipError_t launch_l2_normalize_bwd(const float* u, const float* uh, const float* duh, float* du, int64_t rows, int E,
                                   hipStream_t stream);
hipError_t launch_bilinear_pair_fwd(const float* v, const float* c, const float* bias, float* s, int64_t B, int N, int E,
                                    int normalize, hipStream_t stream);
hipError_t launch_bilinear_pair_bwd(const float* v, const float* c, const float* g, float* dc, float* G, int64_t B, int N, int E,
                                    int normalize, hipStream_t stream);
hipError_t launch_mlp_pair_fwd(const float* q, const float* p, const float* w2, const float* b2, float* s, int64_t B, int N, int H,
                               hipStream_t stream);
hipError_t launch_mlp_pair_bwd(const float* q, const float* p, const float* w2, const float* g, float* delta, float* Delta,
                               float* dw2_part, int64_t B, int N, int H, hipStream_t stream);
hipError_t launch_score_csr_bilinear(const float* vecs, const int32_t* rows, const int32_t* sess, const float* v, const float* bias,
                                     float* r, int64_t n, int E, int relu, hipStream_t stream);
hipError_t launch_score_csr_mlp(const float* P, const int32_t* rows, const int32_t* sess, const float* q, const float* w2,
                                const float* b2, float* r, int64_t n, int H, int relu, hipStream_t stream);

hipError_t launch_infonce_fwd(const float* x, const int64_t* lab, int64_t B, int E, float temperature, float* loss, float* ws,
                              hipStream_t stream);
hipError_t launch_infonce_bwd(const int64_t* lab, int64_t B, int E, float temperature, const float* ws, const float* gout,
                              float* dx, hipStream_t stream);

struct GruFwdArgs {
  float* g;
  const float* whh;
  const float* bhh;
  const float* h0;
  const int32_t* len;
  float* y;
  float* hs;
  float* q;
  int32_t B, T, Hd;
  int32_t vec;
};
hipError_t launch_gru_lengths(const float* m, int64_t ldm, int32_t* len, int64_t B, int T, hipStream_t stream);
hipError_t launch_gru_fwd(const GruFwdArgs& a, hipStream_t stream);
struct GruBwdArgs {
  const float* g;
  const float* q;
  const float* hs;
  const float* whh_t;
  const float* dy;
  float* dh;
  float* dgi;
  float* dgh;
  int32_t B, T, Hd;
  int32_t vec;
};
hipError_t launch_gru_bwd(const GruBwdArgs& a, hipStream_t stream);

}
```

Before: 20620 impressions/s.

## Fuse K/V and query projection GEMMs into a single launch

Merges the live-tile K/V projection GEMM and the scattered query-row projection GEMM into one kernel launch. Blocks are split into two sections by a map function, with the K/V section padded to a multiple of eight for XCD alignment. Device-side counts decide which blocks do work. It also adds a launch counter and an ABI query for testing. The aim is to cut one launch plus the tail idle time between the two dependent-free GEMMs, at the cost of a more complex kernel and possible idle padded blocks.

```diff
diff --git a/include/xnrs_hip.h b/include/xnrs_hip.h
--- a/include/xnrs_hip.h
+++ b/include/xnrs_hip.h
@@ -220,6 +220,11 @@
 #define XNRS_PROFILE_STAGES 10
 int32_t xnrs_profile_enable(uint32_t stage_mask);
 int32_t xnrs_profile_read(double *ms, int64_t *launches, double *flops);
+
+int32_t xnrs_qkv_launch_count(int32_t reset);
+int32_t xnrs_qkv_one_launch_map(int64_t block, int64_t live_tiles, int64_t live_rows, int32_t kv_row_tiles,
+                                int32_t kv_col_tiles, int64_t q_rows, int32_t q_tile_rows, int32_t q_col_tiles,
+                                int32_t *section, int32_t *index);
 
 int32_t xnrs_train_fold_enabled(void);
 
diff --git a/xnrs_amd/csrc/api.hip b/xnrs_amd/csrc/api.hip
--- a/xnrs_amd/csrc/api.hip
+++ b/xnrs_amd/csrc/api.hip
@@ -93,6 +93,25 @@
   return XNRS_OK;
 }
 
+int32_t xnrs_qkv_launch_count(int32_t reset) {
+  const int64_t n = xnrs::qkv_launches_read(reset != 0);
+  return n > 0x7fffffffLL ? 0x7fffffff : (int32_t)n;
+}
+
+int32_t xnrs_qkv_one_launch_map(int64_t block, int64_t live_tiles, int64_t live_rows, int32_t kv_row_tiles, int32_t kv_col_tiles,
+                                int64_t q_rows, int32_t q_tile_rows, int32_t q_col_tiles, int32_t* section, int32_t* index) {
+  if (kv_row_tiles < 0 || kv_col_tiles < 1 || q_rows < 0 || q_tile_rows < 1 || q_col_tiles < 1) return XNRS_EINVAL;
+  const int64_t grid = xnrs::qkv_one_launch_grid(kv_row_tiles, kv_col_tiles, q_rows, q_tile_rows, q_col_tiles);
+  if (grid > 0x7fffffffLL) return XNRS_EINVAL;
+  if (section && index) {
+    const xnrs::QkvOneLaunchWork w =
+        xnrs::qkv_one_launch_map(block, live_tiles, live_rows, kv_row_tiles, kv_col_tiles, q_rows, q_tile_rows, q_col_tiles);
+    *section = w.section;
+    *index = w.index;
+  }
+  return (int32_t)grid;
+}
+
 int32_t xnrs_profile_enable(uint32_t stage_mask) {
   std::lock_guard<std::mutex> lk(g_prof_mu);
   for (auto& r : g_prof) {
diff --git a/xnrs_amd/csrc/encoder_fwd.hip b/xnrs_amd/csrc/encoder_fwd.hip
--- a/xnrs_amd/csrc/encoder_fwd.hip
+++ b/xnrs_amd/csrc/encoder_fwd.hip
@@ -434,13 +434,19 @@
         GemmArgs g = qkv_projection(cx, {cids, L}, att, 1, qkv + D, ld3, rows, D, pqkv);
         g.live_n = ltn;
         g.live_tiles = ltl;
-        XNRS_TRY(launch_gemm_f32(g, stream));
         GemmArgs q = gemm_linear(cx, {ids ? lrs : lrl, 1}, D, att->wq, att->bq, qkv, ld3, rows, D, D);
         q.c_scatter = 1;
         q.c_scatter_ids = lrl;
         q.m_dev = lrn;
         q.m_fill_hint = LR_FILL;
-        XNRS_TRY(launch_gemm_f32(q, stream));
+        if (gemm_qkv_one_launch_ok(g, q)) {
+          XNRS_TRY(launch_gemm_qkv_one(g, q, stream));
+          qkv_launches_add(1);
+        } else {
+          XNRS_TRY(launch_gemm_f32(g, stream));
+          XNRS_TRY(launch_gemm_f32(q, stream));
+          qkv_launches_add(2);
+        }
       } else {
         GemmArgs g = qkv_projection(cx, {cids, L}, att, 0, qkv, ld3, rows, D, pqkv);
         if (lt_qkv) {
diff --git a/xnrs_amd/csrc/gemm_f32.hip b/xnrs_amd/csrc/gemm_f32.hip
--- a/xnrs_amd/csrc/gemm_f32.hip
+++ b/xnrs_amd/csrc/gemm_f32.hip
@@ -16,541 +16,55 @@
 template <int TM, int TN, bool A_COL, bool B_KN, bool VEC, int PIPE, int BK, bool BUF = false, int MINW = 2, bool GATH = false,
           int KG = 2, bool RDOT = false, bool MDEV = false, bool LIVE = false>
 __global__ __launch_bounds__(256, MINW) void gemm_f32_kernel(const GemmArgs a, int m_tiles, int n_tiles_seg, int gn) {
-  static_assert(!MDEV || (!A_COL && !B_KN), "device row counts: forward layout only");
-  static_assert(!LIVE || (BUF && !MDEV), "live row tiles: buffer-load forward kernels, host row count");
-  static_assert(!BUF || (!A_COL && !B_KN && VEC), "buffer loads are implemented for the forward layout");
-  static_assert(!RDOT || PIPE == 5, "the fused row dots ride on the interleaved pipeline (its MFMA call is the swapped one)");
-  static_assert(!GATH || BUF, "the gathered-A variant keeps buffer loads for B");
-  constexpr int BM = 64 * TM, BN = 64 * TN;
-  constexpr bool SWZ = BK == 16;
-  constexpr int LDK = SWZ ? BK : BK + 4;
-  constexpr int CHK = BK / 4;
-  constexpr int RPP = 256 / CHK;
-  constexpr int AR = BM / RPP, BR = BN / RPP;
-  constexpr int LDA = A_COL ? (BM + 4) : LDK;
-  constexpr int LDB = B_KN ? (BN + 4) : LDK;
-  constexpr int A_SZ = A_COL ? BK * LDA : BM * LDA;
-  constexpr int B_SZ = B_KN ? BK * LDB : BN * LDB;
-  constexpr int NBUF = 2;
-  __shared__ __attribute__((aligned(16))) float As[NBUF][A_SZ];
-  __shared__ __attribute__((aligned(16))) float Bs[NBUF][B_SZ];
-
-  int64_t Mrun = a.M;
-  int nwg = gridDim.x;
-  if constexpr (MDEV) {
-    const int64_t md = load_dev_scalar(a.m_dev);
-    Mrun = ((int64_t)__builtin_amdgcn_readfirstlane((int)(md >> 32)) << 32) | (uint32_t)__builtin_amdgcn_readfirstlane((int)md);
-    if (Mrun > a.M) Mrun = a.M;
-    m_tiles = (int)((Mrun + BM - 1) / BM);
-    nwg = m_tiles * n_tiles_seg * a.nseg;
-    if ((int)blockIdx.x >= nwg) return;
-  }
-  if constexpr (LIVE) {
-    const int nl = __builtin_amdgcn_readfirstlane((int)load_dev_scalar(a.live_n));
-    m_tiles = nl < m_tiles ? (nl > 0 ? nl : 0) : m_tiles;
-    nwg = m_tiles * n_tiles_seg * a.nseg;
-    if ((int)blockIdx.x >= nwg) return;
-  }
-  const int bid = blockIdx.x;
-  const int xcd = bid & 7;
-  const int q = nwg >> 3, r = nwg & 7;
-  const int wgid = (xcd < r ? xcd * (q + 1) : r * (q + 1) + (xcd - r) * q) + (bid >> 3);
-  const int n_tiles = n_tiles_seg * a.nseg;
-  const int grp = wgid / (gn * m_tiles);
-  const int rem = wgid - grp * gn * m_tiles;
-  const int gw = (n_tiles - grp * gn < gn) ? n_tiles - grp * gn : gn;
-  const int mt = rem / gw;
-  const int nt = grp * gn + (rem - mt * gw);
-  const int seg = nt / n_tiles_seg;
-  const int nts = nt - seg * n_tiles_seg;
-  int64_t m0 = (int64_t)mt * BM;
-  if constexpr (LIVE) m0 = (int64_t)__builtin_amdgcn_readfirstlane(a.live_tiles[mt]) * BM;
-  const int n0 = nts * BN;
-
-  int64_t kps = a.k_per_split;
-  int Ktot = (int)a.K;
-  if constexpr (A_COL && B_KN) {
-    if (a.k_dev) {
-      const int kd = __builtin_amdgcn_readfirstlane((int)load_dev_scalar(a.k_dev));
-      Ktot = kd < Ktot ? (kd > 0 ? kd : 0) : Ktot;
-      kps = (((int64_t)Ktot + gridDim.y - 1) / gridDim.y + KALIGN - 1) / KALIGN * KALIGN;
-      if (kps < KALIGN) kps = KALIGN;
-    }
-  }
-  const int kbeg = (int)((int64_t)blockIdx.y * kps);
-  const int kend = (int)((kbeg + kps < Ktot) ? kbeg + kps : Ktot);
-
-  const float* __restrict__ W = a.W[seg];
-  const float* __restrict__ bias = a.bias[seg];
-
-  const int tid = threadIdx.x;
-  const int lane = tid & 63;
-  const int wave = tid >> 6;
-  const int wm = wave >> 1, wn = wave & 1;
-
-  const int lc = tid % CHK, lr = tid / CHK;
-  constexpr int CHA = BM / 4, KRA = 256 / CHA;
-  constexpr int CHB = BN / 4, KRB = 256 / CHB;
-  const int cA = tid % CHA, kA = tid / CHA;
-  const int cB = tid % CHB, kB = tid / CHB;
-
-  const float* pa[AR];
-  const float* pb[BR];
-  unsigned a_ok = 0, b_ok = 0;
-  unsigned offA0 = 0, offB0 = 0;
-  unsigned offBv[BR];
-  int dA = 0, dB = 0;
-  __amdgpu_buffer_rsrc_t rsA, rsB;
-  if constexpr (BUF) {
-    if constexpr (!GATH) rsA = __builtin_amdgcn_make_buffer_rsrc(const_cast<float*>(a.A), 0, (int)(Mrun * a.lda * 4), 0x00020000);
-    rsB = __builtin_amdgcn_make_buffer_rsrc(const_cast<float*>(W), 0, (int)((int64_t)a.Nseg * a.ldw * 4), 0x00020000);
-    if constexpr (GATH) {
-#pragma unroll
-      for (int i = 0; i < AR; ++i) {
-        const int64_t gr = m0 + lr + RPP * i;
-        int64_t src = gr < Mrun ? gr : Mrun - 1;
-        if (a.gather_ids) {
-          const int64_t n = src / a.gather_S;
-          src = (int64_t)a.gather_ids[n] * a.gather_S + (src - n * a.gather_S);
-        }
-        pa[i] = a.A + src * a.lda + 4 * lc;
-      }
-    } else {
-      const int64_t gr = m0 + lr;
-      offA0 = gr < Mrun ? (unsigned)((gr * a.lda + 4 * lc) * 4) : BUF_OOB;
-      dA = (int)(RPP * a.lda * 4);
-    }
-    const int col = n0 + lr;
-    offB0 = col < a.Nseg ? (unsigned)(((int64_t)col * a.ldw + 4 * lc) * 4) : BUF_OOB;
-    dB = (int)(RPP * a.ldw * 4);
-    if constexpr (GATH) {
-#pragma unroll
-      for (int i = 0; i < BR; ++i) offBv[i] = offB0 + (unsigned)(i * dB);
-    }
-  } else if (!A_COL) {
-#pragma unroll
-    for (int i = 0; i < AR; ++i) {
-      int64_t gr = m0 + lr + RPP * i;
-      if (gr < Mrun) a_ok |= 1u << i;
-      else gr = Mrun - 1;
-      int64_t src = gr;
-      if (a.gather_ids) {
-        const int64_t n = gr / a.gather_S;
-        src = (int64_t)a.gather_ids[n] * a.gather_S + (gr - n * a.gather_S);
-      }
-      pa[i] = a.A + src * a.lda;
-    }
-  } else {
-    if (m0 + 4 * cA < Mrun) a_ok = 1;
-  }
-  if (!B_KN) {
-#pragma unroll
-    for (int i = 0; i < BR; ++i) {
-      int col = n0 + lr + RPP * i;
-      if (col < a.Nseg) b_ok |= 1u << i;
-      else col = a.Nseg - 1;
-      pb[i] = W + (int64_t)col * a.ldw;
-    }
-  } else {
-    if (n0 + 4 * cB < a.Nseg) b_ok = 1;
-  }
-
-  f32x4 ra[1][AR], rb[1][BR];
-  const f32x4 zero4 = {0.f, 0.f, 0.f, 0.f};
-  auto gload = [&](auto P, int k0, int only = -1) {
-    constexpr int p = decltype(P)::value;
-    if constexpr (BUF) {
-      const unsigned sel = (k0 + 4 * lc < kend) ? 0u : BUF_OOB;
-      const int soff = (int)(k0 * 4);
-      int ka = k0;
-      if constexpr (GATH) {
-        const int klim = kend - 4 - 4 * lc;
-        ka = ka < klim ? ka : klim;
-      }
-#pragma unroll
-      for (int i = 0; i < AR; ++i)
-        if (only < 0 || only == i) {
-          if constexpr (GATH) ra[p][i] = *reinterpret_cast<const f32x4*>(pa[i] + ka);
-          else ra[p][i] = __builtin_bit_cast(f32x4, __builtin_amdgcn_raw_buffer_load_b128(rsA, (int)(offA0 | sel), soff + i * dA, 0));
-        }
-#pragma unroll
-      for (int i = 0; i < BR; ++i)
-        if (only < 0 || only == AR + i) {
-          if constexpr (GATH) rb[p][i] = __builtin_bit_cast(f32x4, __builtin_amdgcn_raw_buffer_load_b128(rsB, (int)(offBv[i] | sel), soff, 0));
-          else rb[p][i] = __builtin_bit_cast(f32x4, __builtin_amdgcn_raw_buffer_load_b128(rsB, (int)(offB0 | sel), soff + i * dB, 0));
-        }
-      return;
-    }
-    if (!A_COL) {
-      const int64_t k = k0 + 4 * lc;
-      const bool kok = k < kend;
-#pragma unroll
-      for (int i = 0; i < AR; ++i) {
-        if (only >= 0 && only != i) continue;
-        if (VEC) {
-          ra[p][i] = *reinterpret_cast<const f32x4*>((kok && ((a_ok >> i) & 1u)) ? pa[i] + k : g_zero_line);
-        } else {
-          f32x4 v = zero4;
-          if ((a_ok >> i) & 1u) {
-#pragma unroll
-            for (int e = 0; e < 4; ++e)
-              if (k + e < kend) v[e] = pa[i][k + e];
-          }
-          ra[p][i] = v;
-        }
-      }
-    } else {
-      const int64_t mi = m0 + 4 * cA;
-#pragma unroll
-      for (int i = 0; i < AR; ++i) {
-        if (only >= 0 && only != i) continue;
-        const int k = k0 + kA + KRA * i;
-        const bool kok = k < kend;
-        int srck = kok ? k : kbeg;
-        if constexpr (KG == 1) {
-          srck = a.gather_ids[srck];
-        } else if constexpr (KG == 2) {
-          if (a.gather_ids) {
-            if (a.gather_S == 1) srck = a.gather_ids[srck];
-            else {
-              const int n = srck / a.gather_S;
-              srck = a.gather_ids[n] * a.gather_S + (srck - n * a.gather_S);
-            }
-          }
-        }
-        const float* ptr = a.A + (int64_t)srck * a.lda;
-        if (VEC) {
-          ra[p][i] = *reinterpret_cast<const f32x4*>((kok && a_ok) ? ptr + mi : g_zero_line);
-        } else {
-          f32x4 v = zero4;
-          if (kok) {
-#pragma unroll
-            for (int e = 0; e < 4; ++e)
-              if (mi + e < Mrun) v[e] = ptr[mi + e];
-          }
-          ra[p][i] = v;
-        }
-      }
-    }
-    if (!B_KN) {
-      const int64_t k = k0 + 4 * lc;
-      const bool kok = k < kend;
-#pragma unroll
-      for (int i = 0; i < BR; ++i) {
-        if (only >= 0 && only != AR + i) continue;
-        if (VEC) {
-          rb[p][i] = *reinterpret_cast<const f32x4*>((kok && ((b_ok >> i) & 1u)) ? pb[i] + k : g_zero_line);
-        } else {
-          f32x4 v = zero4;
-          if ((b_ok >> i) & 1u) {
-#pragma unroll
-            for (int e = 0; e < 4; ++e)
-              if (k + e < kend) v[e] = pb[i][k + e];
-          }
-          rb[p][i] = v;
-        }
-      }
-    } else {
-      const int ni = n0 + 4 * cB;
-#pragma unroll
-      for (int i = 0; i < BR; ++i) {
-        if (only >= 0 && only != AR + i) continue;
-        const int k = k0 + kB + KRB * i;
-        const bool kok = k < kend;
-        int src = kok ? k : kbeg;
-        if constexpr (KG == 1) {
-          src = a.b_gather_ids[src];
-        } else if constexpr (KG == 2) {
-          if (a.b_gather_ids) {
-            if (a.b_gather_S == 1) src = a.b_gather_ids[src];
-            else {
-              const int n = src / a.b_gather_S;
-              src = a.b_gather_ids[n] * a.b_gather_S + (src - n * a.b_gather_S);
-            }
-          }
-        }
-        const float* ptr = W + (int64_t)src * a.ldw;
-        if (VEC) {
-          rb[p][i] = *reinterpret_cast<const f32x4*>((kok && b_ok) ? ptr + ni : g_zero_line);
-        } else {
-          f32x4 v = zero4;
-          if (kok) {
-#pragma unroll
-            for (int e = 0; e < 4; ++e)
-              if (ni + e < a.Nseg) v[e] = ptr[ni + e];
-          }
-          rb[p][i] = v;
-        }
-      }
-    }
-  };
-  auto kswz = [](int row, int c) { return SWZ ? (c ^ ((row >> 2) & 3)) : c; };
-  const bool do_cs = A_COL && a.colsum != nullptr && nt == 0;
-  f32x4 cs = {0.f, 0.f, 0.f, 0.f};
-  auto sstore = [&](auto P, int buf, int only = -1, bool fresh = true) {
-    constexpr int p = decltype(P)::value;
-#pragma unroll
-    for (int i = 0; i < AR; ++i) {
-      if (only >= 0 && only != i) continue;
-      if (!A_COL) *reinterpret_cast<f32x4*>(&As[buf][(lr + RPP * i) * LDA + 4 * kswz(lr + RPP * i, lc)]) = ra[p][i];
-      else {
-        *reinterpret_cast<f32x4*>(&As[buf][(kA + KRA * i) * LDA + 4 * cA]) = ra[p][i];
-        if (do_cs && fresh) cs += ra[p][i];
-      }
-    }
-#pragma unroll
-    for (int i = 0; i < BR; ++i) {
-      if (only >= 0 && only != AR + i) continue;
-      if (!B_KN) *reinterpret_cast<f32x4*>(&Bs[buf][(lr + RPP * i) * LDB + 4 * kswz(lr + RPP * i, lc)]) = rb[p][i];
-      else *reinterpret_cast<f32x4*>(&Bs[buf][(kB + KRB * i) * LDB + 4 * cB]) = rb[p][i];
-    }
-  };
-
-  f32x16 acc[TM][TN];
-#pragma unroll
-  for (int i = 0; i < TM; ++i)
-#pragma unroll
-    for (int j = 0; j < TN; ++j)
-#pragma unroll
-      for (int e = 0; e < 16; ++e) acc[i][j][e] = 0.f;
-
-  const int frow = lane & 31;
-  const int fk = (lane >> 5) * 4;
-  const int a_row0 = wm * 32 * TM + frow;
-  const int b_row0 = wn * 32 * TN + frow;
-
-  auto compute = [&](int buf, auto KQ0, auto KQ1) {
-#pragma unroll
-    for (int kq = decltype(KQ0)::value; kq < decltype(KQ1)::value; ++kq) {
-      f32x4 fa[TM], fb[TN];
-#pragma unroll
-      for (int i = 0; i < TM; ++i) {
-        if (!A_COL) {
-          fa[i] = *reinterpret_cast<const f32x4*>(&As[buf][(a_row0 + 32 * i) * LDA + 4 * kswz(a_row0 + 32 * i, kq * 2 + (fk >> 2))]);
-        } else {
-#pragma unroll
-          for (int e = 0; e < 4; ++e) fa[i][e] = As[buf][(kq * 8 + fk + e) * LDA + a_row0 + 32 * i];
-        }
-      }
-#pragma unroll
-      for (int j = 0; j < TN; ++j) {
-        if (!B_KN) {
-          fb[j] = *reinterpret_cast<const f32x4*>(&Bs[buf][(b_row0 + 32 * j) * LDB + 4 * kswz(b_row0 + 32 * j, kq * 2 + (fk >> 2))]);
-        } else {
-#pragma unroll
-          for (int e = 0; e < 4; ++e) fb[j][e] = Bs[buf][(kq * 8 + fk + e) * LDB + b_row0 + 32 * j];
-        }
-      }
-#pragma unroll
-      for (int e = 0; e < 4; ++e)
-#pragma unroll
-        for (int i = 0; i < TM; ++i)
-#pragma unroll
-          for (int j = 0; j < TN; ++j)
-            acc[i][j] = __builtin_amdgcn_mfma_f32_32x32x2f32(fa[i][e], fb[j][e], acc[i][j], 0, 0, 0);
-    }
-  };
-  using I0 = std::integral_constant<int, 0>;
-  using I4 = std::integral_constant<int, BK / 8>;
-
-  const int nk = (kend - kbeg + BK - 1) / BK;
-  auto ktile = [&](int t) { return kbeg + t * BK; };
-  if constexpr (PIPE == 1) {
-    if (nk > 0) {
-      gload(I0{}, ktile(0));
-      sstore(I0{}, 0);
-    }
-    __syncthreads();
-    for (int t = 0; t < nk; ++t) {
-      const int buf = t & 1;
-      if (t + 1 < nk) gload(I0{}, ktile(t + 1));
-      compute(buf, I0{}, I4{});
-      if (t + 1 < nk) sstore(I0{}, buf ^ 1);
-      __syncthreads();
-    }
-  } else if constexpr (PIPE == 5) {
-    constexpr int NKQ = BK / 8;
-    constexpr int NSLOT = NKQ * 4;
-    constexpr int NCH = AR + BR;
-    static_assert(NCH + 2 <= NSLOT, "not enough slots for the tile stores/loads");
-    f32x4 fa[2][TM], fb[2][TN];
-    auto ldfrag = [&](int st, int buf, int kq) {
-#pragma unroll
-      for (int i = 0; i < TM; ++i) {
-        if (!A_COL) {
-          fa[st][i] = *reinterpret_cast<const f32x4*>(&As[buf][(a_row0 + 32 * i) * LDA + 4 * kswz(a_row0 + 32 * i, kq * 2 + (fk >> 2))]);
-        } else {
-#pragma unroll
-          for (int e = 0; e < 4; ++e) fa[st][i][e] = As[buf][(kq * 8 + fk + e) * LDA + a_row0 + 32 * i];
-        }
-      }
-#pragma unroll
-      for (int j = 0; j < TN; ++j) {
-        if (!B_KN) {
-          fb[st][j] = *reinterpret_cast<const f32x4*>(&Bs[buf][(b_row0 + 32 * j) * LDB + 4 * kswz(b_row0 + 32 * j, kq * 2 + (fk >> 2))]);
-        } else {
-#pragma unroll
-          for (int e = 0; e < 4; ++e) fb[st][j][e] = Bs[buf][(kq * 8 + fk + e) * LDB + b_row0 + 32 * j];
-        }
-      }
-    };
-    const int last = nk - 1;
-    if (nk > 0) {
-      gload(I0{}, ktile(0));
-      sstore(I0{}, 0);
-      gload(I0{}, ktile(1 < last ? 1 : last));
-    }
-    __syncthreads();
-    for (int t = 0; t < nk; ++t) {
-      const int buf = t & 1;
-      const int kn = ktile(t + 2 < last ? t + 2 : last);
-      ldfrag(0, buf, 0);
-#pragma unroll
-      for (int kq = 0; kq < NKQ; ++kq) {
-#pragma unroll
-        for (int e = 0; e < 4; ++e) {
-          const int slot = kq * 4 + e;
-#pragma unroll
-          for (int i = 0; i < TM; ++i)
-#pragma unroll
-            for (int j = 0; j < TN; ++j)
-              if constexpr (RDOT)
-                acc[i][j] = __builtin_amdgcn_mfma_f32_32x32x2f32(fb[kq & 1][j][e], fa[kq & 1][i][e], acc[i][j], 0, 0, 0);
-              else
-                acc[i][j] = __builtin_amdgcn_mfma_f32_32x32x2f32(fa[kq & 1][i][e], fb[kq & 1][j][e], acc[i][j], 0, 0, 0);
-          if (e == 1 && kq + 1 < NKQ) ldfrag((kq + 1) & 1, buf, kq + 1);
-          if (slot >= 1 && slot < 1 + NCH) sstore(I0{}, buf ^ 1, slot - 1, t < last);
-          if (slot >= 2 && slot < 2 + NCH) gload(I0{}, kn, slot - 2);
-          __builtin_amdgcn_sched_barrier(0);
-        }
-      }
-      __syncthreads();
-    }
-  }
-
-  if constexpr (A_COL) {
-    if (a.colsum != nullptr && nt == 0) {
-      f32x4* red = reinterpret_cast<f32x4*>(&As[0][0]);
-      red[kA * CHA + cA] = cs;
-      __syncthreads();
-      if (kA == 0) {
-        f32x4 v = red[cA];
-#pragma unroll
-        for (int r = 1; r < KRA; ++r) v += red[r * CHA + cA];
-        float* dst = a.colsum + (int64_t)blockIdx.y * Mrun + m0 + 4 * cA;
-#pragma unroll
-        for (int e = 0; e < 4; ++e)
-          if (m0 + 4 * cA + e < Mrun) dst[e] = v[e];
-      }
-    }
-  }
-
-  const int ccol = lane & 31;
-  const int crow = 4 * (lane >> 5);
-  const bool split = gridDim.y > 1;
-  float* Cout = split ? a.slabs + (int64_t)blockIdx.y * a.slab_stride : a.C;
-  if constexpr (RDOT) {
-    float2* s_bw = reinterpret_cast<float2*>(&As[0][0]);
-    static_assert(sizeof(float2) * BN <= sizeof(float) * A_SZ * NBUF, "bias / weight staging fits the A tile buffers");
-    for (int c = tid; c < BN; c += 256) {
-      const int col = n0 + c;
-      const bool cok = col < a.Nseg;
-      s_bw[c] = make_float2((bias && cok) ? bias[col] : 0.f, cok ? a.rowdot_w[col] : 0.f);
-    }
-    __syncthreads();
-    const int half = lane >> 5;
-    auto dots = [&](auto FAST) {
-#pragma unroll
-      for (int j = 0; j < TN; ++j) {
-        const int cb = wn * 32 * TN + 32 * j;
-#pragma unroll
-        for (int i = 0; i < TM; ++i) {
-          const float sc = rowdot_block_t_lds<decltype(FAST)::value>(acc[i][j], s_bw + cb, half);
-          int64_t row = m0 + wm * 32 * TM + 32 * i + (lane & 31);
-          if (lane < 32 && row < Mrun && n0 + cb < a.Nseg) {
-            if constexpr (GATH && MDEV) {
-              if (a.c_scatter) row = (a.c_scatter_ids ? a.c_scatter_ids : a.gather_ids)[row];
-            }
-            a.rowdot_out[row * a.ldrd + ((n0 + cb) >> 5)] = sc;
-          }
-        }
-      }
-    };
-    if (a.act == ACT_TANH_FAST) dots(std::true_type{});
-    else dots(std::false_type{});
-    return;
-  }
-  if constexpr (!A_COL) {
-    if (a.c_scatter) {
-      const int32_t* __restrict__ sids = a.c_scatter_ids ? a.c_scatter_ids : a.gather_ids;
-      const bool one = a.gather_S == 1;
-      float bvj[TN];
-      int colj[TN];
-#pragma unroll
-      for (int j = 0; j < TN; ++j) {
-        colj[j] = n0 + wn * 32 * TN + 32 * j + ccol;
-        bvj[j] = (bias && !split && colj[j] < a.Nseg) ? bias[colj[j]] : 0.f;
-      }
-#pragma unroll
-      for (int i = 0; i < TM; ++i) {
-#pragma unroll
-        for (int e = 0; e < 16; ++e) {
-          int64_t row = m0 + wm * 32 * TM + 32 * i + (e & 3) + 8 * (e >> 2) + crow;
-          if (row >= Mrun) continue;
-          if (one) row = sids[row];
-          else {
-            const int64_t n = row / a.gather_S;
-            row = (int64_t)sids[n] * a.gather_S + (row - n * a.gather_S);
-          }
-#pragma unroll
-          for (int j = 0; j < TN; ++j) {
-            if (colj[j] >= a.Nseg) continue;
-            const int64_t coff = (int64_t)seg * a.Nseg + colj[j];
-            float v = acc[i][j][e];
-            if (!split) {
-              if (a.rowscale) v = fmaf(a.rowscale[row], a.rowscale_vec[colj[j]], v);
-              v = apply_act(v + bvj[j], a.act);
-              if (a.aux_mode) {
-                const float x = a.aux[row * a.ldaux + coff];
-                v *= (a.aux_mode == 1) ? (1.f - x * x) : (x > 0.f ? 1.f : 0.f);
-              }
-              if (a.accumulate) v += Cout[row * a.ldc + coff];
-            }
-            Cout[row * a.ldc + coff] = v;
-          }
-        }
-      }
-      return;
-    }
-  }
-#pragma unroll
-  for (int j = 0; j < TN; ++j) {
-    const int col = n0 + wn * 32 * TN + 32 * j + ccol;
-    if (col >= a.Nseg) continue;
-    const float bv = (bias && !split) ? bias[col] : 0.f;
-    const int64_t coff = (int64_t)seg * a.Nseg + col;
-#pragma unroll
-    for (int i = 0; i < TM; ++i) {
-#pragma unroll
-      for (int e = 0; e < 16; ++e) {
-        int64_t row = m0 + wm * 32 * TM + 32 * i + (e & 3) + 8 * (e >> 2) + crow;
-        if (row < Mrun) {
-          float v = acc[i][j][e];
-          if (!split) {
-            if (a.rowscale) v = fmaf(a.rowscale[row], a.rowscale_vec[col], v);
-            v = apply_act(v + bv, a.act);
-            if (a.aux_mode) {
-              const float x = a.aux[row * a.ldaux + coff];
-              v *= (a.aux_mode == 1) ? (1.f - x * x) : (x > 0.f ? 1.f : 0.f);
-            }
-            if (a.accumulate) v += Cout[row * a.ldc + coff];
-          }
-          if (BUF && a.nt_store) __builtin_nontemporal_store(v, &Cout[row * a.ldc + coff]);
-          else Cout[row * a.ldc + coff] = v;
-        }
-      }
-    }
-  }
+#define XNRS_GEMM_BID blockIdx.x
+#define XNRS_GEMM_NWG gridDim.x
+#define XNRS_GEMM_LDS_TILES(A, B)                            \
+  __shared__ __attribute__((aligned(16))) float A[NBUF][A_SZ]; \
+  __shared__ __attribute__((aligned(16))) float B[NBUF][B_SZ];
+#include "gemm_f32_body.h"
+#undef XNRS_GEMM_BID
+#undef XNRS_GEMM_NWG
+#undef XNRS_GEMM_LDS_TILES
+}
+
+template <int T, int BK>
+constexpr int gemm_f32_lds_floats() {
+  return 2 * 64 * T * (BK == 16 ? BK : BK + 4);
+}
+
+template <int TM, int TN, bool A_COL, bool B_KN, bool VEC, int PIPE, int BK, bool BUF = false, int MINW = 2, bool GATH = false,
+          int KG = 2, bool RDOT = false, bool MDEV = false, bool LIVE = false>
+__device__ __forceinline__ void gemm_f32_body(const GemmArgs& a, int m_tiles, const int n_tiles_seg, const int gn, const int bid_in,
+                                              const int nwg_in, float* As0, float* Bs0) {
+  static_assert(!A_COL && !B_KN, "forward layout (the LDS tile sizes of gemm_f32_lds_floats)");
+#define XNRS_GEMM_BID bid_in
+#define XNRS_GEMM_NWG nwg_in
+#define XNRS_GEMM_LDS_TILES(A, B)                                                                                   \
+  static_assert(NBUF * A_SZ == gemm_f32_lds_floats<TM, BK>() && NBUF * B_SZ == gemm_f32_lds_floats<TN, BK>(), "LDS"); \
+  float(*const A)[A_SZ] = reinterpret_cast<float(*)[A_SZ]>(As0);                                                    \
+  float(*const B)[B_SZ] = reinterpret_cast<float(*)[B_SZ]>(Bs0);
+#include "gemm_f32_body.h"
+#undef XNRS_GEMM_BID
+#undef XNRS_GEMM_NWG
+#undef XNRS_GEMM_LDS_TILES
+}
+
+__global__ __launch_bounds__(256, 4) void gemm_qkv_one_launch_kernel(const GemmArgs kv, const GemmArgs q, int kv_m_tiles,
+                                                                     int kv_n_tiles_seg, int kv_gn, int q_m_tiles, int q_n_tiles,
+                                                                     int q_gn) {
+  __shared__ __attribute__((aligned(16))) float As[gemm_f32_lds_floats<2, 16>()];
+  __shared__ __attribute__((aligned(16))) float Bs[gemm_f32_lds_floats<2, 16>()];
+  static_assert(sizeof(As) + sizeof(Bs) <= 32768, "four workgroups per CU");
+  const int64_t ln = __builtin_amdgcn_readfirstlane((int)load_dev_scalar(kv.live_n));
+  const int64_t md0 = load_dev_scalar(q.m_dev);
+  const int64_t md = ((int64_t)__builtin_amdgcn_readfirstlane((int)(md0 >> 32)) << 32) | (uint32_t)__builtin_amdgcn_readfirstlane((int)md0);
+  const QkvOneLaunchWork w = qkv_one_launch_map((int64_t)blockIdx.x, ln, md, kv_m_tiles, kv_n_tiles_seg * kv.nseg, q.M, 128, q_n_tiles);
+  if (w.section < 0) return;
+  if (w.section == 0)
+    gemm_f32_body<2, 2, false, false, true, 5, 16, true, 4, false, 2, false, false, true>(kv, kv_m_tiles, kv_n_tiles_seg, kv_gn, w.index, 0,
+                                                                                        As, Bs);
+  else
+    gemm_f32_body<2, 1, false, false, true, 5, 16, true, 4, true, 2, false, true, false>(q, q_m_tiles, q_n_tiles, q_gn, w.index, 0, As, Bs);
 }
 
 __global__ __launch_bounds__(256) void transpose_kernel(const float* W, float* Wt, int rows, int cols) {
@@ -820,6 +334,9 @@
   k.additive_fused = (int)num("XNRS_ADDITIVE_FUSED", 1);
   k.af_fbuf = num("XNRS_AF_FBUF", 1) == 2 ? 2 : 1;
   k.mha_skip_masked = num("XNRS_MHA_SKIP_MASKED", 1) != 0;
+  {
+    k.gemm_qkv_one_launch = num("XNRS_GEMM_QKV_ONE_LAUNCH", 1) != 0;
+  }
   k.gemm_live_tiles = num("XNRS_GEMM_LIVE_TILES", 1) != 0;
   k.gemm_live_tiles_min_rows = num("XNRS_GEMM_LIVE_TILES_MIN_ROWS", 16384);
   k.gemm_live_rows = num("XNRS_GEMM_LIVE_ROWS", 1) != 0;
@@ -908,4 +425,50 @@
   return e;
 }
 
-}
+static std::atomic<int64_t> g_qkv_launches{0};
+void qkv_launches_add(int n) { g_qkv_launches.fetch_add(n, std::memory_order_relaxed); }
+int64_t qkv_launches_read(bool reset) {
+  return reset ? g_qkv_launches.exchange(0, std::memory_order_relaxed) : g_qkv_launches.load(std::memory_order_relaxed);
+}
+
+static bool qkv_section_ok(const GemmArgs& a, bool* gath) {
+  auto al16 = [](const void* p) { return (reinterpret_cast<uintptr_t>(p) & 15) == 0; };
+  if (a.a_col || a.b_kn || a.M <= 0 || a.Nseg <= 0 || a.nseg < 1 || a.K < 4 || a.K >= (1ll << 31) || a.K % 4 != 0) return false;
+  if (a.lda % 4 != 0 || a.ldw % 4 != 0 || !al16(a.A)) return false;
+  for (int s = 0; s < a.nseg; ++s)
+    if (!al16(a.W[s])) return false;
+  if ((a.slabs && a.nsplit > 1) || a.rowdot_out || a.rowscale || a.colsum || a.k_dev || a.C2) return false;
+  if (!knobs().gemm_buf || (int64_t)a.Nseg * a.ldw * 4 > (int64_t)BUF_OOB) return false;
+  *gath = a.gather_ids || a.M * a.lda * 4 > (int64_t)BUF_OOB;
+  return true;
+}
+
+bool gemm_qkv_one_launch_ok(const GemmArgs& kv, const GemmArgs& q) {
+  if (!knobs().gemm_qkv_one_launch || gemm_mode() != 0 || knobs().gemm_tile >= 0) return false;
+  bool kv_gath = false, q_gath = false;
+  if (!qkv_section_ok(kv, &kv_gath) || !qkv_section_ok(q, &q_gath)) return false;
+  if (kv_gath || !kv.live_tiles || !kv.live_n || kv.m_dev || kv.c_scatter) return false;
+  if (!q_gath || !q.gather_ids || q.gather_S != 1 || !q.c_scatter || !q.m_dev || q.live_tiles || q.nseg != 1) return false;
+  const int64_t grid = qkv_one_launch_grid((int)((kv.M + 127) / 128), (kv.Nseg + 127) / 128 * kv.nseg, q.M, 128, (q.Nseg + 63) / 64);
+  return (kv.M + 127) / 128 <= 0x7fffffffLL && grid <= 0x7fffffffLL;
+}
+
+hipError_t launch_gemm_qkv_one(const GemmArgs& kv_in, const GemmArgs& q_in, hipStream_t stream) {
+  if (!gemm_qkv_one_launch_ok(kv_in, q_in)) return hipErrorInvalidValue;
+  GemmArgs kv = kv_in, q = q_in;
+  for (GemmArgs* a : {&kv, &q}) {
+    if (a->act == 2 && knobs().fast_tanh) a->act = ACT_TANH_FAST;
+    a->k_per_split = a->K;
+    a->nt_store = (!a->accumulate && !a->c_scatter && a->M * a->ldc * 4 >= (64ll << 20)) ? 1 : 0;
+  }
+  const int kv_m_tiles = (int)((kv.M + 127) / 128), kv_n_tiles_seg = (kv.Nseg + 127) / 128;
+  const int q_m_tiles = (int)((q.M + 127) / 128), q_n_tiles = (q.Nseg + 63) / 64;
+  const int kv_gn = gemm_group_tiles(kv_n_tiles_seg * kv.nseg, 128, kv.K, false);
+  const int q_gn = gemm_group_tiles(q_n_tiles, 64, q.K, false);
+  const dim3 g((unsigned)qkv_one_launch_grid(kv_m_tiles, kv_n_tiles_seg * kv.nseg, q.M, 128, q_n_tiles));
+  hipLaunchKernelGGL(gemm_qkv_one_launch_kernel, g, dim3(256), 0, stream, kv, q, kv_m_tiles, kv_n_tiles_seg, kv_gn, q_m_tiles, q_n_tiles,
+                     q_gn);
+  return hipGetLastError();
+}
+
+}
diff --git a/xnrs_amd/csrc/gemm_f32_body.h b/xnrs_amd/csrc/gemm_f32_body.h
--- /dev/null
+++ b/xnrs_amd/csrc/gemm_f32_body.h
@@ -0,0 +1,534 @@
+  static_assert(!MDEV || (!A_COL && !B_KN), "device row counts: forward layout only");
+  static_assert(!LIVE || (BUF && !MDEV), "live row tiles: buffer-load forward kernels, host row count");
+  static_assert(!BUF || (!A_COL && !B_KN && VEC), "buffer loads are implemented for the forward layout");
+  static_assert(!RDOT || PIPE == 5, "the fused row dots ride on the interleaved pipeline (its MFMA call is the swapped one)");
+  static_assert(!GATH || BUF, "the gathered-A variant keeps buffer loads for B");
+  constexpr int BM = 64 * TM, BN = 64 * TN;
+  constexpr bool SWZ = BK == 16;
+  constexpr int LDK = SWZ ? BK : BK + 4;
+  constexpr int CHK = BK / 4;
+  constexpr int RPP = 256 / CHK;
+  constexpr int AR = BM / RPP, BR = BN / RPP;
+  constexpr int LDA = A_COL ? (BM + 4) : LDK;
+  constexpr int LDB = B_KN ? (BN + 4) : LDK;
+  constexpr int A_SZ = A_COL ? BK * LDA : BM * LDA;
+  constexpr int B_SZ = B_KN ? BK * LDB : BN * LDB;
+  constexpr int NBUF = 2;
+  XNRS_GEMM_LDS_TILES(As, Bs)
+
+  int64_t Mrun = a.M;
+  int nwg = XNRS_GEMM_NWG;
+  if constexpr (MDEV) {
+    const int64_t md = load_dev_scalar(a.m_dev);
+    Mrun = ((int64_t)__builtin_amdgcn_readfirstlane((int)(md >> 32)) << 32) | (uint32_t)__builtin_amdgcn_readfirstlane((int)md);
+    if (Mrun > a.M) Mrun = a.M;
+    m_tiles = (int)((Mrun + BM - 1) / BM);
+    nwg = m_tiles * n_tiles_seg * a.nseg;
+    if ((int)XNRS_GEMM_BID >= nwg) return;
+  }
+  if constexpr (LIVE) {
+    const int nl = __builtin_amdgcn_readfirstlane((int)load_dev_scalar(a.live_n));
+    m_tiles = nl < m_tiles ? (nl > 0 ? nl : 0) : m_tiles;
+    nwg = m_tiles * n_tiles_seg * a.nseg;
+    if ((int)XNRS_GEMM_BID >= nwg) return;
+  }
+  const int bid = XNRS_GEMM_BID;
+  const int xcd = bid & 7;
+  const int q = nwg >> 3, r = nwg & 7;
+  const int wgid = (xcd < r ? xcd * (q + 1) : r * (q + 1) + (xcd - r) * q) + (bid >> 3);
+  const int n_tiles = n_tiles_seg * a.nseg;
+  const int grp = wgid / (gn * m_tiles);
+  const int rem = wgid - grp * gn * m_tiles;
+  const int gw = (n_tiles - grp * gn < gn) ? n_tiles - grp * gn : gn;
+  const int mt = rem / gw;
+  const int nt = grp * gn + (rem - mt * gw);
+  const int seg = nt / n_tiles_seg;
+  const int nts = nt - seg * n_tiles_seg;
+  int64_t m0 = (int64_t)mt * BM;
+  if constexpr (LIVE) m0 = (int64_t)__builtin_amdgcn_readfirstlane(a.live_tiles[mt]) * BM;
+  const int n0 = nts * BN;
+
+  int64_t kps = a.k_per_split;
+  int Ktot = (int)a.K;
+  if constexpr (A_COL && B_KN) {
+    if (a.k_dev) {
+      const int kd = __builtin_amdgcn_readfirstlane((int)load_dev_scalar(a.k_dev));
+      Ktot = kd < Ktot ? (kd > 0 ? kd : 0) : Ktot;
+      kps = (((int64_t)Ktot + gridDim.y - 1) / gridDim.y + KALIGN - 1) / KALIGN * KALIGN;
+      if (kps < KALIGN) kps = KALIGN;
+    }
+  }
+  const int kbeg = (int)((int64_t)blockIdx.y * kps);
+  const int kend = (int)((kbeg + kps < Ktot) ? kbeg + kps : Ktot);
+
+  const float* __restrict__ W = a.W[seg];
+  const float* __restrict__ bias = a.bias[seg];
+
+  const int tid = threadIdx.x;
+  const int lane = tid & 63;
+  const int wave = tid >> 6;
+  const int wm = wave >> 1, wn = wave & 1;
+
+  const int lc = tid % CHK, lr = tid / CHK;
+  constexpr int CHA = BM / 4, KRA = 256 / CHA;
+  constexpr int CHB = BN / 4, KRB = 256 / CHB;
+  const int cA = tid % CHA, kA = tid / CHA;
+  const int cB = tid % CHB, kB = tid / CHB;
+
+  const float* pa[AR];
+  const float* pb[BR];
+  unsigned a_ok = 0, b_ok = 0;
+  unsigned offA0 = 0, offB0 = 0;
+  unsigned offBv[BR];
+  int dA = 0, dB = 0;
+  __amdgpu_buffer_rsrc_t rsA, rsB;
+  if constexpr (BUF) {
+    if constexpr (!GATH) rsA = __builtin_amdgcn_make_buffer_rsrc(const_cast<float*>(a.A), 0, (int)(Mrun * a.lda * 4), 0x00020000);
+    rsB = __builtin_amdgcn_make_buffer_rsrc(const_cast<float*>(W), 0, (int)((int64_t)a.Nseg * a.ldw * 4), 0x00020000);
+    if constexpr (GATH) {
+#pragma unroll
+      for (int i = 0; i < AR; ++i) {
+        const int64_t gr = m0 + lr + RPP * i;
+        int64_t src = gr < Mrun ? gr : Mrun - 1;
+        if (a.gather_ids) {
+          const int64_t n = src / a.gather_S;
+          src = (int64_t)a.gather_ids[n] * a.gather_S + (src - n * a.gather_S);
+        }
+        pa[i] = a.A + src * a.lda + 4 * lc;
+      }
+    } else {
+      const int64_t gr = m0 + lr;
+      offA0 = gr < Mrun ? (unsigned)((gr * a.lda + 4 * lc) * 4) : BUF_OOB;
+      dA = (int)(RPP * a.lda * 4);
+    }
+    const int col = n0 + lr;
+    offB0 = col < a.Nseg ? (unsigned)(((int64_t)col * a.ldw + 4 * lc) * 4) : BUF_OOB;
+    dB = (int)(RPP * a.ldw * 4);
+    if constexpr (GATH) {
+#pragma unroll
+      for (int i = 0; i < BR; ++i) offBv[i] = offB0 + (unsigned)(i * dB);
+    }
+  } else if (!A_COL) {
+#pragma unroll
+    for (int i = 0; i < AR; ++i) {
+      int64_t gr = m0 + lr + RPP * i;
+      if (gr < Mrun) a_ok |= 1u << i;
+      else gr = Mrun - 1;
+      int64_t src = gr;
+      if (a.gather_ids) {
+        const int64_t n = gr / a.gather_S;
+        src = (int64_t)a.gather_ids[n] * a.gather_S + (gr - n * a.gather_S);
+      }
+      pa[i] = a.A + src * a.lda;
+    }
+  } else {
+    if (m0 + 4 * cA < Mrun) a_ok = 1;
+  }
+  if (!B_KN) {
+#pragma unroll
+    for (int i = 0; i < BR; ++i) {
+      int col = n0 + lr + RPP * i;
+      if (col < a.Nseg) b_ok |= 1u << i;
+      else col = a.Nseg - 1;
+      pb[i] = W + (int64_t)col * a.ldw;
+    }
+  } else {
+    if (n0 + 4 * cB < a.Nseg) b_ok = 1;
+  }
+
+  f32x4 ra[1][AR], rb[1][BR];
+  const f32x4 zero4 = {0.f, 0.f, 0.f, 0.f};
+  auto gload = [&](auto P, int k0, int only = -1) {
+    constexpr int p = decltype(P)::value;
+    if constexpr (BUF) {
+      const unsigned sel = (k0 + 4 * lc < kend) ? 0u : BUF_OOB;
+      const int soff = (int)(k0 * 4);
+      int ka = k0;
+      if constexpr (GATH) {
+        const int klim = kend - 4 - 4 * lc;
+        ka = ka < klim ? ka : klim;
+      }
+#pragma unroll
+      for (int i = 0; i < AR; ++i)
+        if (only < 0 || only == i) {
+          if constexpr (GATH) ra[p][i] = *reinterpret_cast<const f32x4*>(pa[i] + ka);
+          else ra[p][i] = __builtin_bit_cast(f32x4, __builtin_amdgcn_raw_buffer_load_b128(rsA, (int)(offA0 | sel), soff + i * dA, 0));
+        }
+#pragma unroll
+      for (int i = 0; i < BR; ++i)
+        if (only < 0 || only == AR + i) {
+          if constexpr (GATH) rb[p][i] = __builtin_bit_cast(f32x4, __builtin_amdgcn_raw_buffer_load_b128(rsB, (int)(offBv[i] | sel), soff, 0));
+          else rb[p][i] = __builtin_bit_cast(f32x4, __builtin_amdgcn_raw_buffer_load_b128(rsB, (int)(offB0 | sel), soff + i * dB, 0));
+        }
+      return;
+    }
+    if (!A_COL) {
+      const int64_t k = k0 + 4 * lc;
+      const bool kok = k < kend;
+#pragma unroll
+      for (int i = 0; i < AR; ++i) {
+        if (only >= 0 && only != i) continue;
+        if (VEC) {
+          ra[p][i] = *reinterpret_cast<const f32x4*>((kok && ((a_ok >> i) & 1u)) ? pa[i] + k : g_zero_line);
+        } else {
+          f32x4 v = zero4;
+          if ((a_ok >> i) & 1u) {
+#pragma unroll
+            for (int e = 0; e < 4; ++e)
+              if (k + e < kend) v[e] = pa[i][k + e];
+          }
+          ra[p][i] = v;
+        }
+      }
+    } else {
+      const int64_t mi = m0 + 4 * cA;
+#pragma unroll
+      for (int i = 0; i < AR; ++i) {
+        if (only >= 0 && only != i) continue;
+        const int k = k0 + kA + KRA * i;
+        const bool kok = k < kend;
+        int srck = kok ? k : kbeg;
+        if constexpr (KG == 1) {
+          srck = a.gather_ids[srck];
+        } else if constexpr (KG == 2) {
+          if (a.gather_ids) {
+            if (a.gather_S == 1) srck = a.gather_ids[srck];
+            else {
+              const int n = srck / a.gather_S;
+              srck = a.gather_ids[n] * a.gather_S + (srck - n * a.gather_S);
+            }
+          }
+        }
+        const float* ptr = a.A + (int64_t)srck * a.lda;
+        if (VEC) {
+          ra[p][i] = *reinterpret_cast<const f32x4*>((kok && a_ok) ? ptr + mi : g_zero_line);
+        } else {
+          f32x4 v = zero4;
+          if (kok) {
+#pragma unroll
+            for (int e = 0; e < 4; ++e)
+              if (mi + e < Mrun) v[e] = ptr[mi + e];
+          }
+          ra[p][i] = v;
+        }
+      }
+    }
+    if (!B_KN) {
+      const int64_t k = k0 + 4 * lc;
+      const bool kok = k < kend;
+#pragma unroll
+      for (int i = 0; i < BR; ++i) {
+        if (only >= 0 && only != AR + i) continue;
+        if (VEC) {
+          rb[p][i] = *reinterpret_cast<const f32x4*>((kok && ((b_ok >> i) & 1u)) ? pb[i] + k : g_zero_line);
+        } else {
+          f32x4 v = zero4;
+          if ((b_ok >> i) & 1u) {
+#pragma unroll
+            for (int e = 0; e < 4; ++e)
+              if (k + e < kend) v[e] = pb[i][k + e];
+          }
+          rb[p][i] = v;
+        }
+      }
+    } else {
+      const int ni = n0 + 4 * cB;
+#pragma unroll
+      for (int i = 0; i < BR; ++i) {
+        if (only >= 0 && only != AR + i) continue;
+        const int k = k0 + kB + KRB * i;
+        const bool kok = k < kend;
+        int src = kok ? k : kbeg;
+        if constexpr (KG == 1) {
+          src = a.b_gather_ids[src];
+        } else if constexpr (KG == 2) {
+          if (a.b_gather_ids) {
+            if (a.b_gather_S == 1) src = a.b_gather_ids[src];
+            else {
+              const int n = src / a.b_gather_S;
+              src = a.b_gather_ids[n] * a.b_gather_S + (src - n * a.b_gather_S);
+            }
+          }
+        }
+        const float* ptr = W + (int64_t)src * a.ldw;
+        if (VEC) {
+          rb[p][i] = *reinterpret_cast<const f32x4*>((kok && b_ok) ? ptr + ni : g_zero_line);
+        } else {
+          f32x4 v = zero4;
+          if (kok) {
+#pragma unroll
+            for (int e = 0; e < 4; ++e)
+              if (ni + e < a.Nseg) v[e] = ptr[ni + e];
+          }
+          rb[p][i] = v;
+        }
+      }
+    }
+  };
+  auto kswz = [](int row, int c) { return SWZ ? (c ^ ((row >> 2) & 3)) : c; };
+  const bool do_cs = A_COL && a.colsum != nullptr && nt == 0;
+  f32x4 cs = {0.f, 0.f, 0.f, 0.f};
+  auto sstore = [&](auto P, int buf, int only = -1, bool fresh = true) {
+    constexpr int p = decltype(P)::value;
+#pragma unroll
+    for (int i = 0; i < AR; ++i) {
+      if (only >= 0 && only != i) continue;
+      if (!A_COL) *reinterpret_cast<f32x4*>(&As[buf][(lr + RPP * i) * LDA + 4 * kswz(lr + RPP * i, lc)]) = ra[p][i];
+      else {
+        *reinterpret_cast<f32x4*>(&As[buf][(kA + KRA * i) * LDA + 4 * cA]) = ra[p][i];
+        if (do_cs && fresh) cs += ra[p][i];
+      }
+    }
+#pragma unroll
+    for (int i = 0; i < BR; ++i) {
+      if (only >= 0 && only != AR + i) continue;
+      if (!B_KN) *reinterpret_cast<f32x4*>(&Bs[buf][(lr + RPP * i) * LDB + 4 * kswz(lr + RPP * i, lc)]) = rb[p][i];
+      else *reinterpret_cast<f32x4*>(&Bs[buf][(kB + KRB * i) * LDB + 4 * cB]) = rb[p][i];
+    }
+  };
+
+  f32x16 acc[TM][TN];
+#pragma unroll
+  for (int i = 0; i < TM; ++i)
+#pragma unroll
+    for (int j = 0; j < TN; ++j)
+#pragma unroll
+      for (int e = 0; e < 16; ++e) acc[i][j][e] = 0.f;
+
+  const int frow = lane & 31;
+  const int fk = (lane >> 5) * 4;
+  const int a_row0 = wm * 32 * TM + frow;
+  const int b_row0 = wn * 32 * TN + frow;
+
+  auto compute = [&](int buf, auto KQ0, auto KQ1) {
+#pragma unroll
+    for (int kq = decltype(KQ0)::value; kq < decltype(KQ1)::value; ++kq) {
+      f32x4 fa[TM], fb[TN];
+#pragma unroll
+      for (int i = 0; i < TM; ++i) {
+        if (!A_COL) {
+          fa[i] = *reinterpret_cast<const f32x4*>(&As[buf][(a_row0 + 32 * i) * LDA + 4 * kswz(a_row0 + 32 * i, kq * 2 + (fk >> 2))]);
+        } else {
+#pragma unroll
+          for (int e = 0; e < 4; ++e) fa[i][e] = As[buf][(kq * 8 + fk + e) * LDA + a_row0 + 32 * i];
+        }
+      }
+#pragma unroll
+      for (int j = 0; j < TN; ++j) {
+        if (!B_KN) {
+          fb[j] = *reinterpret_cast<const f32x4*>(&Bs[buf][(b_row0 + 32 * j) * LDB + 4 * kswz(b_row0 + 32 * j, kq * 2 + (fk >> 2))]);
+        } else {
+#pragma unroll
+          for (int e = 0; e < 4; ++e) fb[j][e] = Bs[buf][(kq * 8 + fk + e) * LDB + b_row0 + 32 * j];
+        }
+      }
+#pragma unroll
+      for (int e = 0; e < 4; ++e)
+#pragma unroll
+        for (int i = 0; i < TM; ++i)
+#pragma unroll
+          for (int j = 0; j < TN; ++j)
+            acc[i][j] = __builtin_amdgcn_mfma_f32_32x32x2f32(fa[i][e], fb[j][e], acc[i][j], 0, 0, 0);
+    }
+  };
+  using I0 = std::integral_constant<int, 0>;
+  using I4 = std::integral_constant<int, BK / 8>;
+
+  const int nk = (kend - kbeg + BK - 1) / BK;
+  auto ktile = [&](int t) { return kbeg + t * BK; };
+  if constexpr (PIPE == 1) {
+    if (nk > 0) {
+      gload(I0{}, ktile(0));
+      sstore(I0{}, 0);
+    }
+    __syncthreads();
+    for (int t = 0; t < nk; ++t) {
+      const int buf = t & 1;
+      if (t + 1 < nk) gload(I0{}, ktile(t + 1));
+      compute(buf, I0{}, I4{});
+      if (t + 1 < nk) sstore(I0{}, buf ^ 1);
+      __syncthreads();
+    }
+  } else if constexpr (PIPE == 5) {
+    constexpr int NKQ = BK / 8;
+    constexpr int NSLOT = NKQ * 4;
+    constexpr int NCH = AR + BR;
+    static_assert(NCH + 2 <= NSLOT, "not enough slots for the tile stores/loads");
+    f32x4 fa[2][TM], fb[2][TN];
+    auto ldfrag = [&](int st, int buf, int kq) {
+#pragma unroll
+      for (int i = 0; i < TM; ++i) {
+        if (!A_COL) {
+          fa[st][i] = *reinterpret_cast<const f32x4*>(&As[buf][(a_row0 + 32 * i) * LDA + 4 * kswz(a_row0 + 32 * i, kq * 2 + (fk >> 2))]);
+        } else {
+#pragma unroll
+          for (int e = 0; e < 4; ++e) fa[st][i][e] = As[buf][(kq * 8 + fk + e) * LDA + a_row0 + 32 * i];
+        }
+      }
+#pragma unroll
+      for (int j = 0; j < TN; ++j) {
+        if (!B_KN) {
+          fb[st][j] = *reinterpret_cast<const f32x4*>(&Bs[buf][(b_row0 + 32 * j) * LDB + 4 * kswz(b_row0 + 32 * j, kq * 2 + (fk >> 2))]);
+        } else {
+#pragma unroll
+          for (int e = 0; e < 4; ++e) fb[st][j][e] = Bs[buf][(kq * 8 + fk + e) * LDB + b_row0 + 32 * j];
+        }
+      }
+    };
+    const int last = nk - 1;
+    if (nk > 0) {
+      gload(I0{}, ktile(0));
+      sstore(I0{}, 0);
+      gload(I0{}, ktile(1 < last ? 1 : last));
+    }
+    __syncthreads();
+    for (int t = 0; t < nk; ++t) {
+      const int buf = t & 1;
+      const int kn = ktile(t + 2 < last ? t + 2 : last);
+      ldfrag(0, buf, 0);
+#pragma unroll
+      for (int kq = 0; kq < NKQ; ++kq) {
+#pragma unroll
+        for (int e = 0; e < 4; ++e) {
+          const int slot = kq * 4 + e;
+#pragma unroll
+          for (int i = 0; i < TM; ++i)
+#pragma unroll
+            for (int j = 0; j < TN; ++j)
+              if constexpr (RDOT)
+                acc[i][j] = __builtin_amdgcn_mfma_f32_32x32x2f32(fb[kq & 1][j][e], fa[kq & 1][i][e], acc[i][j], 0, 0, 0);
+              else
+                acc[i][j] = __builtin_amdgcn_mfma_f32_32x32x2f32(fa[kq & 1][i][e], fb[kq & 1][j][e], acc[i][j], 0, 0, 0);
+          if (e == 1 && kq + 1 < NKQ) ldfrag((kq + 1) & 1, buf, kq + 1);
+          if (slot >= 1 && slot < 1 + NCH) sstore(I0{}, buf ^ 1, slot - 1, t < last);
+          if (slot >= 2 && slot < 2 + NCH) gload(I0{}, kn, slot - 2);
+          __builtin_amdgcn_sched_barrier(0);
+        }
+      }
+      __syncthreads();
+    }
+  }
+
+  if constexpr (A_COL) {
+    if (a.colsum != nullptr && nt == 0) {
+      f32x4* red = reinterpret_cast<f32x4*>(&As[0][0]);
+      red[kA * CHA + cA] = cs;
+      __syncthreads();
+      if (kA == 0) {
+        f32x4 v = red[cA];
+#pragma unroll
+        for (int r = 1; r < KRA; ++r) v += red[r * CHA + cA];
+        float* dst = a.colsum + (int64_t)blockIdx.y * Mrun + m0 + 4 * cA;
+#pragma unroll
+        for (int e = 0; e < 4; ++e)
+          if (m0 + 4 * cA + e < Mrun) dst[e] = v[e];
+      }
+    }
+  }
+
+  const int ccol = lane & 31;
+  const int crow = 4 * (lane >> 5);
+  const bool split = gridDim.y > 1;
+  float* Cout = split ? a.slabs + (int64_t)blockIdx.y * a.slab_stride : a.C;
+  if constexpr (RDOT) {
+    float2* s_bw = reinterpret_cast<float2*>(&As[0][0]);
+    static_assert(sizeof(float2) * BN <= sizeof(float) * A_SZ * NBUF, "bias / weight staging fits the A tile buffers");
+    for (int c = tid; c < BN; c += 256) {
+      const int col = n0 + c;
+      const bool cok = col < a.Nseg;
+      s_bw[c] = make_float2((bias && cok) ? bias[col] : 0.f, cok ? a.rowdot_w[col] : 0.f);
+    }
+    __syncthreads();
+    const int half = lane >> 5;
+    auto dots = [&](auto FAST) {
+#pragma unroll
+      for (int j = 0; j < TN; ++j) {
+        const int cb = wn * 32 * TN + 32 * j;
+#pragma unroll
+        for (int i = 0; i < TM; ++i) {
+          const float sc = rowdot_block_t_lds<decltype(FAST)::value>(acc[i][j], s_bw + cb, half);
+          int64_t row = m0 + wm * 32 * TM + 32 * i + (lane & 31);
+          if (lane < 32 && row < Mrun && n0 + cb < a.Nseg) {
+            if constexpr (GATH && MDEV) {
+              if (a.c_scatter) row = (a.c_scatter_ids ? a.c_scatter_ids : a.gather_ids)[row];
+            }
+            a.rowdot_out[row * a.ldrd + ((n0 + cb) >> 5)] = sc;
+          }
+        }
+      }
+    };
+    if (a.act == ACT_TANH_FAST) dots(std::true_type{});
+    else dots(std::false_type{});
+    return;
+  }
+  if constexpr (!A_COL) {
+    if (a.c_scatter) {
+      const int32_t* __restrict__ sids = a.c_scatter_ids ? a.c_scatter_ids : a.gather_ids;
+      const bool one = a.gather_S == 1;
+      float bvj[TN];
+      int colj[TN];
+#pragma unroll
+      for (int j = 0; j < TN; ++j) {
+        colj[j] = n0 + wn * 32 * TN + 32 * j + ccol;
+        bvj[j] = (bias && !split && colj[j] < a.Nseg) ? bias[colj[j]] : 0.f;
+      }
+#pragma unroll
+      for (int i = 0; i < TM; ++i) {
+#pragma unroll
+        for (int e = 0; e < 16; ++e) {
+          int64_t row = m0 + wm * 32 * TM + 32 * i + (e & 3) + 8 * (e >> 2) + crow;
+          if (row >= Mrun) continue;
+          if (one) row = sids[row];
+          else {
+            const int64_t n = row / a.gather_S;
+            row = (int64_t)sids[n] * a.gather_S + (row - n * a.gather_S);
+          }
+#pragma unroll
+          for (int j = 0; j < TN; ++j) {
+            if (colj[j] >= a.Nseg) continue;
+            const int64_t coff = (int64_t)seg * a.Nseg + colj[j];
+            float v = acc[i][j][e];
+            if (!split) {
+              if (a.rowscale) v = fmaf(a.rowscale[row], a.rowscale_vec[colj[j]], v);
+              v = apply_act(v + bvj[j], a.act);
+              if (a.aux_mode) {
+                const float x = a.aux[row * a.ldaux + coff];
+                v *= (a.aux_mode == 1) ? (1.f - x * x) : (x > 0.f ? 1.f : 0.f);
+              }
+              if (a.accumulate) v += Cout[row * a.ldc + coff];
+            }
+            Cout[row * a.ldc + coff] = v;
+          }
+        }
+      }
+      return;
+    }
+  }
+#pragma unroll
+  for (int j = 0; j < TN; ++j) {
+    const int col = n0 + wn * 32 * TN + 32 * j + ccol;
+    if (col >= a.Nseg) continue;
+    const float bv = (bias && !split) ? bias[col] : 0.f;
+    const int64_t coff = (int64_t)seg * a.Nseg + col;
+#pragma unroll
+    for (int i = 0; i < TM; ++i) {
+#pragma unroll
+      for (int e = 0; e < 16; ++e) {
+        int64_t row = m0 + wm * 32 * TM + 32 * i + (e & 3) + 8 * (e >> 2) + crow;
+        if (row < Mrun) {
+          float v = acc[i][j][e];
+          if (!split) {
+            if (a.rowscale) v = fmaf(a.rowscale[row], a.rowscale_vec[col], v);
+            v = apply_act(v + bv, a.act);
+            if (a.aux_mode) {
+              const float x = a.aux[row * a.ldaux + coff];
+              v *= (a.aux_mode == 1) ? (1.f - x * x) : (x > 0.f ? 1.f : 0.f);
+            }
+            if (a.accumulate) v += Cout[row * a.ldc + coff];
+          }
+          if (BUF && a.nt_store) __builtin_nontemporal_store(v, &Cout[row * a.ldc + coff]);
+          else Cout[row * a.ldc + coff] = v;
+        }
+      }
+    }
+  }
diff --git a/xnrs_amd/csrc/kernels.h b/xnrs_amd/csrc/kernels.h
--- a/xnrs_amd/csrc/kernels.h
+++ b/xnrs_amd/csrc/kernels.h
@@ -35,6 +35,7 @@
   long long gemm_live_tiles_min_rows = 16384;
   bool gemm_live_rows = true;
   long long gemm_live_rows_min_rows = 16384;
+  bool gemm_qkv_one_launch = true;
   bool mha_skip_masked = true;
   int gru_layout = 0;
 };
@@ -98,6 +99,26 @@
 int gemm_group_tiles(int n_tiles, int bn, int64_t K, bool plain);
 size_t gemm_splitk_workspace_bytes(int64_t M, int64_t N, int64_t K);
 hipError_t launch_gemm_f32(const GemmArgs& a, hipStream_t stream, int* nsplit_used = nullptr);
+struct QkvOneLaunchWork {
+  int section;
+  int index;
+};
+__host__ __device__ inline QkvOneLaunchWork qkv_one_launch_map(int64_t block, int64_t live_n, int64_t m_dev, int kv_m_tiles,
+                                                               int kv_n_tiles, int64_t q_rows, int q_bm, int q_n_tiles) {
+  const int64_t lt = live_n < kv_m_tiles ? (live_n > 0 ? live_n : 0) : kv_m_tiles;
+  const int64_t kv_wgs = lt * kv_n_tiles, kv_pad = (kv_wgs + 7) & ~(int64_t)7;
+  if (block < kv_pad) return block >= 0 && block < kv_wgs ? QkvOneLaunchWork{0, (int)block} : QkvOneLaunchWork{-1, 0};
+  const int64_t rows = m_dev < q_rows ? (m_dev > 0 ? m_dev : 0) : q_rows;
+  const int64_t q_wgs = ((rows + q_bm - 1) / q_bm) * q_n_tiles;
+  return block - kv_pad < q_wgs ? QkvOneLaunchWork{1, (int)(block - kv_pad)} : QkvOneLaunchWork{-1, 0};
+}
+inline int64_t qkv_one_launch_grid(int kv_m_tiles, int kv_n_tiles, int64_t q_rows, int q_bm, int q_n_tiles) {
+  return (((int64_t)kv_m_tiles * kv_n_tiles + 7) & ~(int64_t)7) + ((q_rows + q_bm - 1) / q_bm) * q_n_tiles;
+}
+bool gemm_qkv_one_launch_ok(const GemmArgs& kv, const GemmArgs& q);
+hipError_t launch_gemm_qkv_one(const GemmArgs& kv, const GemmArgs& q, hipStream_t stream);
+void qkv_launches_add(int n);
+int64_t qkv_launches_read(bool reset);
 bool gemm_dw_eligible(const GemmArgs& a);
 bool gemm_dw_big_tile(const GemmArgs& a);
 hipError_t launch_gemm_dw(const GemmArgs& a, int nsplit, hipStream_t stream);
```

New measurement: 21240 impressions/s (median of 6 runs). +3.0%, better.
